# PaddlePaddle/Anakin

Hardware: AMD Instinct MI355X
Metric: ResNet50 INT8 images/sec + p50 latency @ batch 1/8, 1×MI355X (higher is better)
Workload: dtype int8

## Files before the change

### anakin_amd/csrc/api_chain.hip

```cpp
#include "api_internal.h"

enum : unsigned { CK_1X1 = 1, CK_3X3 = 2, CK_HEAD = 4, CK_PAIR = 8, CK_LED = CK_3X3 | CK_HEAD, CK_ANY = 15 };
static unsigned chain_kind(const saber_hip_chain* ch) { return !ch->c3 ? CK_1X1 : (ch->b2 ? CK_PAIR : (ch->b ? CK_3X3 : CK_HEAD)); }
static const struct { int c1; unsigned kinds; ChainForm f; } chain_forms[] = {
    {64, CK_ANY,            {4, 4, 4, 1, 1, CS_BASE, false}},
    {64, CK_ANY,            {2, 2, 4, 1, 1, CS_BASE, false}},
    {128, CK_1X1 | CK_LED,  {2, 2, 4, 1, 1, CS_BASE, false}},
    {128, CK_1X1 | CK_LED,  {1, 1, 4, 1, 1, CS_BASE, false}},
    {128, CK_1X1 | CK_LED,  {6, 2, 8, 1, 1, CS_W8, false}},
    {128, CK_1X1 | CK_LED,  {5, 1, 8, 1, 1, CS_W8, false}},
    {256, CK_1X1 | CK_LED,  {1, 1, 4, 1, 1, CS_BASE, false}},
    {256, CK_1X1,           {9, 1, 4, 2, 1, CS_SPLIT, false}},
    {256, CK_1X1,           {11, 1, 8, 2, 1, CS_SPLIT8, false}},
    {256, CK_LED,           {3, 1, 8, 1, 1, CS_W8, false}},
    {256, CK_3X3,           {7, 1, 8, 1, 2, CS_COOP2, true}},
    {256, CK_3X3,           {15, 2, 8, 1, 4, CS_COOP4, true}},
    {512, CK_1X1,           {1, 1, 4, 1, 1, CS_BASE, false}},
    {512, CK_1X1,           {9, 1, 4, 2, 1, CS_SPLIT, false}},
};
static void for_each_chain_form(const saber_hip_chain* ch, const std::function<void(const ChainForm&)>& fn) {
    for (const auto& r : chain_forms)
        if (r.c1 == ch->c1 && (r.kinds & chain_kind(ch))) fn(r.f);
}
static ChainForm chain_form_where(const saber_hip_chain* ch, const std::function<bool(const ChainForm& row, const ChainForm& found)>& take) {
// ... 45 lines not shown
    const int kw = K / nw, groups = kw / (16 * mfg), ksn = C / 64;
    for (int g = 0; g < groups; ++g)
        for (int ksi = 0; ksi < ksn; ++ksi)
            for (int mf = 0; mf < mfg; ++mf) {
                const int ks = (ks0 + ksi) % ksn;
                for (int lane = 0; lane < 64; ++lane) {
                    const int rho = lane & 15, kq = lane >> 4;
                    const int ch = kbase + wave * kw + g * 16 * mfg + (rho >> 2) * 4 * mfg + mf * 4 + (rho & 3);
                    const int8_t* src = w + (size_t)ch * C + ks * 64 + kq * 16;
                    out.insert(out.end(), (const uint8_t*)src, (const uint8_t*)src + 16);
                }
            }
}
static void pack_chain_weights3(const int8_t* w, int C, int wave, std::vector<uint8_t>& out, int nw = 4, int kbase = 0, int kcount = 0) {
    const int kw = (kcount ? kcount : C) / nw, mf0 = kw / 16, ksn = C / 64;
    for (int tap = 0; tap < 9; ++tap)
        for (int ks = 0; ks < ksn; ++ks)
            for (int mf = 0; mf < mf0; ++mf)
                for (int lane = 0; lane < 64; ++lane) {
                    const int rho = lane & 15, kq = lane >> 4;
                    const int ch = kbase + wave * kw + (rho >> 2) * 4 * mf0 + mf * 4 + (rho & 3);
                    for (int t = 0; t < 16; ++t) {
                        const int c = ks * 64 + kq * 16 + t;
                        out.push_back((uint8_t)w[((size_t)ch * C + c) * 9 + tap]);
                    }
                }
}
static void pack_frag1(const int8_t* w, int C, int ch_base, int mfg, int mf, int ks, std::vector<uint8_t>& out) {
    for (int lane = 0; lane < 64; ++lane) {
        const int rho = lane & 15, kq = lane >> 4;
        const int8_t* src = w + (size_t)(ch_base + (rho >> 2) * 4 * mfg + mf * 4 + (rho & 3)) * C + ks * 64 + kq * 16;
        out.insert(out.end(), (const uint8_t*)src, (const uint8_t*)src + 16);
    }
}
static void pack_frag3(const int8_t* w, int C, int ch_base, int tap, int ks, std::vector<uint8_t>& out) {
    for (int lane = 0; lane < 64; ++lane) {
        const int rho = lane & 15, kq = lane >> 4;
        for (int t = 0; t < 16; ++t) out.push_back((uint8_t)w[((size_t)(ch_base + rho) * C + ks * 64 + kq * 16 + t) * 9 + tap]);
    }
}
static void pack_coop4_stream(const saber_hip_conv* c3, const saber_hip_conv* a, const saber_hip_conv* b, std::vector<uint8_t>& out) {
    const int C = 256, K1 = 1024;
    for (int q = 0; q < 4; ++q)
        for (int w = 0; w < 8; ++w) {
            const int nt = w & 3, kh = w >> 2;
            for (int tap = 0; tap < 9; ++tap)
                for (int kl = 0; kl < 2; ++kl) pack_frag3(c3->wq_oihw.data(), C, q * 64 + nt * 16, tap, kh * 2 + kl, out);
            for (int i = 0; i < 4; ++i)
                for (int mf = 0; mf < 2; ++mf) pack_frag1(a->wq_oihw.data(), C, q * 256 + w * 32, 2, mf, (q + i) & 3, out);
            for (int jj = 0; b && jj < 8; ++jj) {
                const int j = jj < 2 ? kh * 2 + jj : 4 + kh * 6 + (jj - 2);
                pack_frag1(b->wq_oihw.data(), K1, q * 64 + nt * 16, 1, 0, (q * 4 + j) & 15, out);
            }
        }
}
static void pack_stage1_c128_stream(const saber_hip_conv* c3, const saber_hip_conv* a, const saber_hip_conv* b, std::vector<uint8_t>& out) {
    const int C = 128, K1 = 512;
    for (int w = 0; w < 8; ++w) {
        for (int tap = 0; tap < 9; ++tap)
            for (int ks = 0; ks < 2; ++ks) pack_frag3(c3->wq_oihw.data(), C, w * 16, tap, ks, out);
        for (int ks = 0; ks < 2; ++ks)
            for (int mf = 0; mf < 4; ++mf) pack_frag1(a->wq_oihw.data(), C, w * 64, 4, mf, ks, out);
        for (int ks = 0; ks < 8; ++ks) pack_frag1(b->wq_oihw.data(), K1, w * 16, 1, 0, ks, out);
    }
}
int saber_hip_conv2d_stem_pair_create(saber_hip_conv_t* stem, const saber_hip_conv_t* a, const saber_hip_conv_t* b, saber_hip_stem_pair_t** out) {
    if (!stem || !a || !b || !out) return fail(SABER_HIP_INVALID_VALUE, "null argument");
    const saber_hip_conv_desc& ds = stem->d;
    if (!stem->pool_fused || !stem->weights_set || ds.k != 64 || (ds.out_dtype != SABER_HIP_U8 && ds.out_dtype != SABER_HIP_S8))
        return fail(SABER_HIP_INVALID_VALUE, "stem pair: the head must be the fused stem conv + max pooling with 64 output channels (8-bit)");
    auto plain1x1 = [&](const saber_hip_conv* o) {
        const saber_hip_conv_desc& d = o->d;
        return o->is_i8 && o->weights_set && o->algo == ALGO_IGEMM_I8 && o->epi == EPI_I8_CONV && d.res_mode == SABER_HIP_RES_NONE &&
               !o->pair_k2 && !o->pool_fused && !o->pool2 && !o->pre_quant && !o->pre_pad && d.kh == 1 && d.kw == 1 && d.stride_h == 1 &&
               d.stride_w == 1 && d.pad_h == 0 && d.pad_w == 0 && d.group == 1 && d.c == 64 && o->c_eff == 64 && d.k % 32 == 0 &&
               d.in_layout == SABER_HIP_NHWC && d.out_layout == SABER_HIP_NHWC && d.act_negative_slope == 0.f &&
               (d.out_dtype == SABER_HIP_S8 || d.out_dtype == SABER_HIP_U8) && d.n == ds.n && d.h == stem->pool_oh && d.w == stem->pool_ow &&
               (o->x_dtype == DT_U8) == (ds.out_dtype == SABER_HIP_U8) && (int)o->wq_oihw.size() == d.k * 64;
    };
    if (!plain1x1(a) || !plain1x1(b) || a->d.k + b->d.k > 320)
        return fail(SABER_HIP_INVALID_VALUE, "stem pair: two plain 1x1 / stride-1 INT8 convs (64 -> k, k % 32 == 0, k_a + k_b <= 320, 8-bit NHWC outputs) "
                                              "on the pooled tensor");
    auto* sp = new saber_hip_stem_pair();
    sp->stem = stem; sp->a = a; sp->b = b;
    const int K1 = a->d.k, Kt = K1 + b->d.k;
    std::vector<int8_t> wcat((size_t)Kt * 64);
    std::memcpy(wcat.data(), a->wq_oihw.data(), (size_t)K1 * 64);
    std::memcpy(wcat.data() + (size_t)K1 * 64, b->wq_oihw.data(), (size_t)b->d.k * 64);
    std::vector<uint8_t> w, pa, pb, prm(256 * 16, 0);
    w.reserve((size_t)Kt * 64);
    for (int g = 0; g < Kt / 32; ++g)
        for (int mf = 0; mf < 2; ++mf) pack_frag1(wcat.data(), 64, g * 32, 2, mf, 0, w);
    pack_chain_params(a, (size_t)K1 / 4 * 3, pa);
    pack_chain_params(b, (size_t)b->d.k / 4 * 3, pb);
    std::memcpy(prm.data(), pa.data(), pa.size());
    std::memcpy(prm.data() + pa.size(), pb.data(), pb.size());
    hipError_t e = sp->d_w.upload(w);
    if (e == hipSuccess) e = sp->d_prm.upload(prm);
    if (e != hipSuccess) {
        delete sp;
        return hip_fail(e, "stem pair: device copies");
    }
    *out = sp;
    return SABER_HIP_OK;
}
void saber_hip_conv2d_stem_pair_destroy(saber_hip_stem_pair_t* sp) { delete sp; }
int saber_hip_conv2d_stem_pair_run(saber_hip_stem_pair_t* sp, const void* x, void* y_pool, void* y_a, void* y_b, void* workspace,
                                   saber_hip_stream_t stream) {
    if (g_capture) return capture_unsupported("saber_hip_conv2d_stem_pair_run (an executor-level object: saber_hip_net_optimize forms it itself)");
    if (!sp || !x || !y_a || !y_b) return fail(SABER_HIP_INVALID_VALUE, "null argument");
    saber_hip_conv* op = sp->stem;
    if (op->ws_bytes && !workspace) return fail(SABER_HIP_INVALID_VALUE, "workspace required");
    saber_mi355x::StemPairKArgs ka;
    const int rc = stem_pool_args(op, x, y_pool, workspace, (hipStream_t)stream, &ka.c);
    if (rc) return rc;
    ka.t.w = sp->d_w.p; ka.t.prm = sp->d_prm.p; ka.t.y1 = y_a; ka.t.y2 = y_b;
    ka.t.K1 = sp->a->d.k; ka.t.K2 = sp->b->d.k;
    ka.t.relu1 = sp->a->d.act == SABER_HIP_ACT_RELU; ka.t.relu2 = sp->b->d.act == SABER_HIP_ACT_RELU;
    ka.t.u8_1 = sp->a->d.out_dtype == SABER_HIP_U8; ka.t.u8_2 = sp->b->d.out_dtype == SABER_HIP_U8;
    HIP_TRY(saber_mi355x::launch_conv_stem_pool_pair(op->pre_quant ? 1 : 0, ka, (hipStream_t)stream));
    return SABER_HIP_OK;
}
saber_hip_chain::~saber_hip_chain() {
    if (h_coop_err) (void)hipHostFree(h_coop_err);
    delete stage1;
}
static unsigned div_magic(int d) { return d >= 2 ? (unsigned)((0x100000000ull + (unsigned)d - 1) / (unsigned)d) : 0u; }
static int stage_build(saber_hip_chain* const* chains, int n, bool per_image, saber_hip_chain* tail, saber_hip_chain_stage** out) {
    if (!chains || n <= 0 || n > saber_mi355x::STAGE4_LONG || !out) return fail(SABER_HIP_INVALID_VALUE, "stage: 1..24 chains");
    if (tail) {
        if (!chains[0] || chains[0]->c1 != 256 || tail->c1 != 256) return fail(SABER_HIP_INVALID_VALUE, "stage: a tail goes with a C = 256 stage only");
        if (n < 2 || !per_image || n + 1 > saber_mi355x::STAGE4_LONG) return fail(SABER_HIP_INVALID_VALUE, "stage: a tail needs 2..23 blocks, an image per XCD");
        if (!tail->c3 || tail->b || tail->b2 || tail->c3->d.stride_h != 2 || tail->c3->d.stride_w != 2)
            return fail(SABER_HIP_INVALID_VALUE, "stage: the tail must be a conv3x3 / stride 2 + conv1x1 chain without a second 1x1 conv");
        if (tail->a->d.res_stride != 2) return fail(SABER_HIP_INVALID_VALUE, "stage: the tail's shortcut must be sub-sampled by 2");
    }
    if (n > 1 && !per_image) return fail(SABER_HIP_INVALID_VALUE, "stage: several blocks need an image per XCD");
    if (n < 2 && chains[0] && chains[0]->c1 == 128) return fail(SABER_HIP_INVALID_VALUE, "stage: at C = 128 a stage is at least two blocks");
    const saber_hip_chain* c0 = chains[0];
    std::vector<saber_mi355x::StageBlk> blk;
    for (int k = 0; k < n; ++k) {
        const saber_hip_chain* ch = chains[k];
        const uint8_t* stream = !ch ? nullptr : (ch->c1 == 256 ? ch->d_stream[CS_COOP4].p : (ch->c1 == 128 ? ch->d_stream_stage1.p : nullptr));
        if (!ch || ch->c1 != c0->c1 || !ch->c3 || !ch->b || !stream || ch->c3->d.stride_h != 1)
            return fail(SABER_HIP_INVALID_VALUE, "stage: every block must be a conv3x3 (stride 1) + conv1x1 + conv1x1 chain at C = 256 (or all at C = 128)");
        const saber_hip_conv_desc& da = ch->a->d;
        if (da.n != c0->a->d.n || da.h != c0->a->d.h || da.w != c0->a->d.w) return fail(SABER_HIP_INVALID_VALUE, "stage: blocks of one tensor shape");
        if (k && ((ch->c3->x_dtype == DT_U8) != (chains[k - 1]->b->d.out_dtype == SABER_HIP_U8)))
            return fail(SABER_HIP_INVALID_VALUE, "stage: a block's 3x3 conv reads what the previous block's last conv writes");
        saber_mi355x::StageBlk B;
        std::memset(&B, 0, sizeof B);
        B.wstream = stream; B.prm0 = ch->d_prm0.p; B.prm1 = ch->d_prm1.p; B.prm2 = ch->d_prm2.p;
        B.coeff_conv = da.coeff_conv; B.scale_conv = ch->a->out_scale; B.coeff_res = da.coeff_res; B.scale_res = da.scale_res;
        B.in0_u8 = ch->c3->x_dtype == DT_U8; B.relu0 = ch->c3->d.act == SABER_HIP_ACT_RELU;
        B.in_u8 = ch->a->x_dtype == DT_U8; B.relu1 = da.act == SABER_HIP_ACT_RELU; B.res_relu = da.res_act == SABER_HIP_ACT_RELU;
        B.relu2 = ch->b->d.act == SABER_HIP_ACT_RELU; B.out_u8_2 = ch->b->d.out_dtype == SABER_HIP_U8;
        blk.push_back(B);
    }
    const saber_hip_conv_desc& d0 = c0->a->d;
    if (tail) {
        const saber_hip_conv_desc &d3 = tail->c3->d, &da = tail->a->d;
        if (d3.n != d0.n || d3.h != d0.h || d3.w != d0.w || da.res_h != d0.h || da.res_w != d0.w)
            return fail(SABER_HIP_INVALID_VALUE, "stage: the tail's 3x3 conv and shortcut read tensors of the blocks' shape");
        if ((tail->c3->x_dtype == DT_U8) != (chains[n - 1]->b->d.out_dtype == SABER_HIP_U8))
            return fail(SABER_HIP_INVALID_VALUE, "stage: the tail's 3x3 conv reads what the last block's last conv writes");
    }
    saber_hip_chain_stage* st = new saber_hip_chain_stage();
    st->chains.assign(chains, chains + n);
    st->c1 = c0->c1;
    st->n = d0.n; st->h = d0.h; st->w = d0.w;
    st->tiles_x = (d0.w + 15) / 16;
    st->tiles_per_img = st->tiles_x * ((d0.h + 1) / 2);
    st->per_image = per_image;
    const int wg_per_tile = st->c1 == 256 ? 4 : 1;
    const bool fits = d0.n <= 8 && st->tiles_per_img * wg_per_tile <= 32 &&
                      (st->c1 == 256 ? st->tiles_x == 1 : (st->tiles_x == 1 || st->tiles_x == 2 || st->tiles_x == 4));
    if ((per_image && !fits) || (st->c1 == 128 && !per_image)) {
        delete st;
        return fail(SABER_HIP_INVALID_VALUE, "stage: an image per XCD needs batch <= 8 and <= 32 workgroups per image (C = 256: width <= 16, <= 8 tiles "
                    "of 2 x 16 pixels; C = 128: width <= 64, <= 32 tiles)");
    }
    const size_t tiles = (size_t)d0.n * st->tiles_per_img;
    hipError_t e = hipSuccess;
    if (tail) {
        std::vector<uint8_t> ts;
        pack_coop4_stream(tail->c3, tail->a, nullptr, ts);
        e = st->d_tail_stream.upload(ts);
        const saber_hip_conv_desc& da = tail->a->d;
        saber_mi355x::StageBlk B;
        std::memset(&B, 0, sizeof B);
        B.wstream = st->d_tail_stream.p; B.prm0 = tail->d_prm0.p; B.prm1 = tail->d_prm1.p; B.prm2 = tail->d_prm0.p;
        B.coeff_conv = da.coeff_conv; B.scale_conv = tail->a->out_scale; B.coeff_res = da.coeff_res; B.scale_res = da.scale_res;
        B.in0_u8 = tail->c3->x_dtype == DT_U8; B.relu0 = tail->c3->d.act == SABER_HIP_ACT_RELU;
        B.in_u8 = tail->a->x_dtype == DT_U8; B.relu1 = da.act == SABER_HIP_ACT_RELU; B.res_relu = da.res_act == SABER_HIP_ACT_RELU;
        blk.push_back(B);
        st->tail = tail;
    }
    if (e == hipSuccess) e = st->d_blk.upload(blk);
    if (e == hipSuccess && st->c1 == 256) e = st->d_grp_ctr.alloc_zero(tiles * 32);
    if (e == hipSuccess) e = st->d_img_ctr.alloc_zero((size_t)d0.n * (st->tiles_per_img + 1) * 16);
    if (e == hipSuccess) e = st->d_xcc.alloc_zero(tiles * 32);
    if (e == hipSuccess && st->c1 == 256) e = st->d_xch.alloc_zero(tiles * 32 * 256);
    if (e == hipSuccess) e = hipHostMalloc((void**)&st->h_err, sizeof(unsigned), hipHostMallocMapped);
    if (e != hipSuccess) {
        delete st;
        return hip_fail(e, "stage: device buffers");
    }
    *st->h_err = 0u;
    *out = st;
    return SABER_HIP_OK;
}
template <int MAXB>
static int stage_launch(saber_hip_chain_stage* st, const void* x, const void* res, void* const* y1, void* const* y2, void* y_tail, hipStream_t s) {
    saber_mi355x::Stage4KArgs<MAXB> k;
    std::memset(&k, 0, sizeof k);
    k.x = x; k.res = res; k.zero = zero_page();
    if (!k.zero) return fail(SABER_HIP_RUNTIME_ERROR, "stage: zero page");
    k.blk = st->d_blk.p; k.grp_ctr = st->d_grp_ctr.p; k.img_ctr = st->d_img_ctr.p; k.xch = st->d_xch.p; k.xcc = st->d_xcc.p; k.err = st->h_err;
    k.nblk = (int)st->chains.size(); k.N = st->n; k.H = st->h; k.W = st->w;
    k.tiles_x = st->tiles_x; k.tiles_per_img = st->tiles_per_img;
    k.mg_tiles_x = div_magic(st->tiles_x); k.mg_tpi = div_magic(st->tiles_per_img); k.mg_wpi = div_magic(st->tiles_per_img * 4);
    k.per_image = st->per_image;
    for (int i = 0; i < k.nblk; ++i) { k.y1[i] = y1[i]; k.y2[i] = y2[i]; }
    if (y_tail) k.y1[k.nblk] = y_tail;
    HIP_TRY(st->c1 == 256 ? saber_mi355x::launch_conv_stage4(k, y_tail != nullptr, s) : saber_mi355x::launch_conv_stage1_c128(k, s));
    return SABER_HIP_OK;
}
int stage_run(saber_hip_chain_stage* st, const void* x, const void* res, void* const* y1, void* const* y2, hipStream_t s, void* y_tail) {
    if (y_tail && !st->tail) return fail(SABER_HIP_INVALID_VALUE, "stage: created without a tail");
    if (*(volatile unsigned*)st->h_err) {
        *(volatile unsigned*)st->h_err = 0u;
        return fail(SABER_HIP_RUNTIME_ERROR, "cooperative stage: an earlier launch's workgroups did not share an XCD or timed out at a barrier "
                    "(its outputs are not valid)");
    }
    return (int)st->chains.size() + (y_tail ? 1 : 0) <= saber_mi355x::STAGE4_SHORT ? stage_launch<saber_mi355x::STAGE4_SHORT>(st, x, res, y1, y2, y_tail, s)
                                                                                   : stage_launch<saber_mi355x::STAGE4_LONG>(st, x, res, y1, y2, y_tail, s);
}
int saber_hip_conv2d_stage_create(saber_hip_chain_t* const* chains, int n, saber_hip_chain_stage_t** out) {
    if (!xcd_round_robin()) return fail(SABER_HIP_UNIMPL, "stage: this device does not place workgroup b on XCD b % 8");
    return stage_build(chains, n, true, nullptr, out);
}
int saber_hip_conv2d_stage_create_tail(saber_hip_chain_t* const* chains, int n, saber_hip_chain_t* tail, saber_hip_chain_stage_t** out) {
    if (!tail) return fail(SABER_HIP_INVALID_VALUE, "null argument");
    if (!xcd_round_robin()) return fail(SABER_HIP_UNIMPL, "stage: this device does not place workgroup b on XCD b % 8");
    return stage_build(chains, n, true, tail, out);
}
void saber_hip_conv2d_stage_destroy(saber_hip_chain_stage_t* st) { delete st; }
int saber_hip_conv2d_stage_run(saber_hip_chain_stage_t* st, const void* x, const void* res, void* const* y1, void* const* y2, saber_hip_stream_t stream) {
    if (g_capture) return capture_unsupported("saber_hip_conv2d_stage_run (saber_hip_net_optimize forms stages itself)");
    if (!st || !x || !res || !y1 || !y2) return fail(SABER_HIP_INVALID_VALUE, "null argument");
    for (size_t i = 0; i < st->chains.size(); ++i)
        if (!y1[i] || !y2[i]) return fail(SABER_HIP_INVALID_VALUE, "stage: an output pointer per block");
    return stage_run(st, x, res, y1, y2, (hipStream_t)stream);
}
int saber_hip_conv2d_stage_run_tail(saber_hip_chain_stage_t* st, const void* x, const void* res, void* const* y1, void* const* y2, void* y_tail,
                                    saber_hip_stream_t stream) {
    if (g_capture) return capture_unsupported("saber_hip_conv2d_stage_run_tail (saber_hip_net_optimize forms stages itself)");
    if (!st || !x || !res || !y1 || !y2 || !y_tail) return fail(SABER_HIP_INVALID_VALUE, "null argument");
    for (size_t i = 0; i < st->chains.size(); ++i)
        if (!y1[i] || !y2[i]) return fail(SABER_HIP_INVALID_VALUE, "stage: an output pointer per block");
    return stage_run(st, x, res, y1, y2, (hipStream_t)stream, y_tail);
}
static void pack_chain_stream(const saber_hip_chain* ch, ChainStream layout, std::vector<uint8_t>& out) {
    const saber_hip_conv *c3 = ch->c3, *a = ch->a, *b = ch->b;
    const int c = ch->c1, k1 = ch->k1, k2 = ch->k2, c2 = b ? b->d.c : 0, k2w = k2 / 2;
    const int nw = layout == CS_BASE || layout == CS_SPLIT ? 4 : 8;
    const int8_t *w3 = c3 ? c3->wq_oihw.data() : nullptr, *wa = a->wq_oihw.data(), *wb = b ? b->wq_oihw.data() : nullptr;
    std::vector<int8_t> wcat;
    if (ch->b2) {
        wcat.assign(b->wq_oihw.begin(), b->wq_oihw.end());
        wcat.insert(wcat.end(), ch->b2->wq_oihw.begin(), ch->b2->wq_oihw.end());
        wb = wcat.data();
    }
    auto mfg = [&](int k) { return ch->b2 ? 2 : std::min(4, k / nw / 16); };
    switch (layout) {
    case CS_BASE: case CS_W8:
        for (int w = 0; w < nw; ++w) {
            if (c3) pack_chain_weights3(w3, c, w, out, nw);
            pack_chain_weights(wa, k1, c, 4, w, out, 0, nw);
            if (b) pack_chain_weights(wb, k2, c2, mfg(k2), w, out, 0, nw);
        }
        break;
    case CS_SPLIT: case CS_SPLIT8:
        for (int half = 0; half < 2; ++half)
            for (int w = 0; w < nw; ++w) {
                pack_chain_weights(wa, k1, c, 4, w, out, 0, nw);
                pack_chain_weights(wb, k2w, c2, mfg(k2w), w, out, half * k2w, nw);
            }
        break;
    case CS_COOP2:
        for (int half = 0; half < 2; ++half)
            for (int w = 0; w < nw; ++w) {
                pack_chain_weights3(w3, c, w, out, nw, half * (c / 2), c / 2);
                pack_chain_weights(wa, k1 / 2, c, 4, w, out, half * (k1 / 2), nw, half * (c / 128));
                pack_chain_weights(wb, k2w, c2, 1, w, out, half * k2w, nw, half * (c2 / 128));
            }
        break;
    default: pack_coop4_stream(c3, a, b, out);
    }
}
static int chain_build(saber_hip_conv* c3, saber_hip_conv* a, saber_hip_conv* b, saber_hip_chain_t** out, saber_hip_conv* b2 = nullptr) {
    if (!a || !out || (!b && !c3) || (b2 && (!b || !c3))) return fail(SABER_HIP_INVALID_VALUE, "null argument");
    const bool pair2 = b2 != nullptr;
    const bool strided = c3 && (!b || pair2) && c3->d.stride_h == 2 && c3->d.stride_w == 2;
    if (pair2 && !strided) return fail(SABER_HIP_INVALID_VALUE, "chain: a sibling pair follows the strided head (conv3x3 / stride 2 + conv1x1 + eltwise) only");
    if (!chain_1x1(a, strided) || (b && !chain_1x1(b)) || (b2 && !chain_1x1(b2)))
        return fail(SABER_HIP_INVALID_VALUE, "chain: both ops must be plain 1x1 stride-1 INT8 NHWC convs with weights set");
    if (strided != (a->d.res_stride > 1) || (strided && a->d.res_stride != 2))
        return fail(SABER_HIP_INVALID_VALUE, "chain: a stride-2 head goes with a shortcut sub-sampled by 2 (and only with one)");
    const saber_hip_conv_desc& da = a->d;
    if (da.res_mode != SABER_HIP_RES_ELTWISE || da.out_dtype != SABER_HIP_S8 || (da.res_has_dtype && da.res_dtype != SABER_HIP_S8))
        return fail(SABER_HIP_INVALID_VALUE, "chain: the first conv must carry the fused eltwise epilogue with s8 residual and output");
    if (b) {
        const saber_hip_conv_desc& db = b->d;
// ... 168 lines not shown
```

### anakin_amd/csrc/api_internal.h

```cpp
#pragma once
#include "../../include/saber_hip.h"
#include "kernels.h"

#include <cmath>
#include <cstdio>
#include <algorithm>
#include <cstdlib>
#include <cstring>
#include <functional>
#include <memory>
#include <mutex>
#include <string>
#include <utility>
#include <type_traits>
#include <vector>

using namespace saber_mi355x;

namespace saber_api {

extern thread_local std::string g_err;
inline int fail(int code, const std::string& msg) {
    g_err = msg;
    return code;
// ... 142 lines not shown
    unsigned* h_part_err = nullptr;
    DevBuf<uint8_t> d_w3;
    DevBuf<float> d_bias, d_scale;
    DevBuf<int> d_comp;
    DevBuf<unsigned> d_sm_ctr;
    bool has_bias = false, has_comp = false;
    std::string algo_name;
    int pair_k1 = 0, pair_k2 = 0, pair_relu2 = 0, pair_dtype2 = 0;
    const saber_hip_conv* pair_src_a = nullptr;
    const saber_hip_conv* pair_src_b = nullptr;
};

struct saber_hip_stem_pair {
    saber_hip_conv* stem = nullptr;
    const saber_hip_conv* a = nullptr;
    const saber_hip_conv* b = nullptr;
    DevBuf<uint8_t> d_w, d_prm;
};

enum ChainStream { CS_BASE, CS_SPLIT, CS_SPLIT8, CS_W8, CS_COOP2, CS_COOP4, CS_COUNT };
struct ChainForm {
    int code = 0;
    int rows = 0;
    int waves = 4;
    int split = 1;
    int coop = 1;
    ChainStream stream = CS_BASE;
    bool placement = false;
};

struct saber_hip_chain {
    saber_hip_conv* c3 = nullptr;
    saber_hip_conv* a = nullptr;
    saber_hip_conv* b = nullptr;
    saber_hip_conv* b2 = nullptr;
    int c1 = 0, k1 = 0, k2 = 0;
    ChainForm form;
    DevBuf<uint8_t> d_stream[CS_COUNT];
    DevBuf<uint8_t> d_prm0, d_prm1, d_prm2;
    DevBuf<uint8_t> d_coop_xch;
    DevBuf<uint8_t> d_stream_stage1;
    DevBuf<unsigned long long> d_coop_ctr;
    DevBuf<unsigned> d_coop_xcc;
    unsigned* h_coop_err = nullptr;
    int coop_tiles = 0;
    struct saber_hip_chain_stage* stage1 = nullptr;
    ~saber_hip_chain();
};

struct saber_hip_chain_stage {
    std::vector<saber_hip_chain*> chains;
    saber_hip_chain* tail = nullptr;
    DevBuf<uint8_t> d_tail_stream;
    DevBuf<saber_mi355x::StageBlk> d_blk;
    DevBuf<unsigned long long> d_grp_ctr, d_img_ctr;
    DevBuf<uint8_t> d_xch;
    DevBuf<unsigned> d_xcc;
    unsigned* h_err = nullptr;
    int c1 = 0, n = 0, h = 0, w = 0, tiles_x = 0, tiles_per_img = 0;
    bool per_image = false;
    ~saber_hip_chain_stage() {
        if (h_err) (void)hipHostFree(h_err);
    }
};

struct saber_hip_sep {
    saber_hip_conv* dw = nullptr;
    saber_hip_conv* pw = nullptr;
    int form = 0;
    DevBuf<uint8_t> d_wdw, d_wpw, d_prm;
    DevBuf<float> d_dw_bias, d_dw_scale;
    std::string name;
};

struct saber_hip_fc {
    saber_hip_fc_desc d;
    saber_hip_conv* conv = nullptr;
    bool pre_quant = false;
    float in_scale = 1.f;
};

namespace saber_api {
struct EventPair {
    hipEvent_t e0 = nullptr, e1 = nullptr;
    hipError_t init() {
        hipError_t e = hipEventCreate(&e0);
        return e != hipSuccess ? e : hipEventCreate(&e1);
    }
    ~EventPair() {
        if (e0) (void)hipEventDestroy(e0);
        if (e1) (void)hipEventDestroy(e1);
    }
};
struct ColdBench {
    size_t kBytes = (size_t)64 << 20;
    void* buf = nullptr;
    std::vector<hipEvent_t> ev;
    int reps = 0;
    hipError_t init(int r, size_t bytes = 0) {
        if (bytes) kBytes = std::min<size_t>(std::max<size_t>(bytes, (size_t)64 << 20), (size_t)512 << 20) & ~(size_t)0xfffff;
        reps = r < 3 ? 3 : (r > 32 ? 32 : r);
        hipError_t e = hipMalloc(&buf, kBytes + 256);
        if (e != hipSuccess) return e;
        e = hipMemset(buf, 1, kBytes + 256);
        if (e != hipSuccess) return e;
        ev.assign(2 * (size_t)reps, nullptr);
// ... 17 lines not shown
        if (hipEventSynchronize(ev[2 * reps - 1]) != hipSuccess) return -1.f;
        std::vector<float> t(reps);
        for (int r = 0; r < reps; ++r)
            if (hipEventElapsedTime(&t[r], ev[2 * r], ev[2 * r + 1]) != hipSuccess) return -1.f;
        std::sort(t.begin(), t.end());
        return t[reps / 2] * 1000.f;
    }
};

extern thread_local ColdBench* g_cold;
int time_enqueued(hipStream_t s, const std::function<int()>& fn, int warm_iters, float* t);
extern thread_local std::vector<unsigned long long>* g_used_kernels;
constexpr float g_reuse_tol = 0.03f;
struct ColdScope {
    ColdBench local;
    bool owner = false;
    hipError_t enter(int reps, size_t flush_bytes = 0) {
        const char* w = std::getenv("SABER_HIP_AUTOTUNE_WARM");
        if (w && w[0] == '1') return hipSuccess;
        if (g_cold) return hipSuccess;
        hipError_t e = local.init(reps, flush_bytes);
        if (e != hipSuccess) return e;
        g_cold = &local;
        owner = true;
        return hipSuccess;
    }
    ~ColdScope() {
        if (owner) g_cold = nullptr;
    }
};

}

namespace saber_api {
enum OpKind { OP_CONV, OP_CONV_PAIR, OP_FC, OP_QUANT, OP_DEQUANT, OP_TRANSPOSE_IN, OP_ELT_I8, OP_ELT_F32, OP_POOL_I8, OP_POOL_F32, OP_POOL_F32_I8, OP_FC_Q, OP_SOFTMAX, OP_RELU_F32, OP_ACT_F32 };
struct NetOp {
    OpKind kind;
    std::string name;
    saber_hip_conv* conv = nullptr;
    saber_hip_fc* fc = nullptr;
    int in = -1, in2 = -1, out = -1, out2 = -1;
    saber_hip_chain* chain = nullptr;
    int chain_out = -1;
    bool use_chain = false, skip = false;
    saber_hip_chain* chain3 = nullptr;
    int chain3_res = -1, chain3_y1 = -1, chain3_y2 = -1;
    int chain3_y3 = -1;
    bool use_chain3 = false;
    saber_hip_chain_stage* stage = nullptr;
    int stage_n = 0;
    bool use_stage = false;
    bool use_tail = false;
    int tail_of = -1, tail_mode = 0;
    saber_hip_stem_pair* stem_pair = nullptr;
    int stem_y1 = -1, stem_y2 = -1;
    saber_hip_sep* sep = nullptr;
    int sep_out = -1;
    bool use_sep = false;
    int lane = 0;
    bool record = false;
    int p[16] = {0};
    float f[6] = {0};
    size_t count = 0;
};
}

struct saber_hip_net {
    std::vector<size_t> tensor_bytes;
    std::vector<size_t> tensor_off;
    std::vector<void*> tensor_ext;
    std::vector<std::pair<const void*, int>> captured_ptr;
    void* ptr(int id) const {
        if (id < 0) return nullptr;
        if ((size_t)id < tensor_ext.size() && tensor_ext[id]) return tensor_ext[id];
        return (void*)(arena + tensor_off[id]);
    }
    std::vector<NetOp> ops;
    char* arena = nullptr;
    size_t arena_bytes = 0, ws_off = 0, ws_bytes = 0;
    hipGraph_t graph = nullptr;
    hipGraphExec_t exec = nullptr;
    bool finalized = false;
    bool compacted = false;
    bool shared_device = false;
    bool reproducible_fp32 = false;
    bool inplace_external = false;
    int coop_fallbacks = 0;
    hipStream_t side = nullptr;
    hipEvent_t ev_start = nullptr, ev_join = nullptr;
    std::vector<hipEvent_t> ev_op;
    std::vector<int> writer;
    bool lanes_ready = false, has_side = false;
    std::vector<saber_hip_conv*> owned;
    std::vector<saber_hip_chain*> owned_chains;
    std::vector<saber_hip_chain_stage*> owned_stages;
    std::vector<saber_hip_stem_pair*> owned_stem_pairs;
    std::vector<saber_hip_sep*> owned_seps;
};

namespace saber_api {
struct Capture;
extern thread_local Capture* g_capture;
int capture_conv(saber_hip_conv* op, const void* x, void* y, const void* res);
int capture_fc(saber_hip_fc* fc, const void* x, float* y, bool quantised_input);
int capture_unsupported(const char* what);
int capture_stream_op(OpKind kind, const char* name, const int* p, int np, const float* f, int nf, size_t count, const void* in,
                      size_t in_bytes, const void* in2, size_t in2_bytes, void* out, size_t out_bytes, void* out2, size_t out2_bytes);
}

bool sel_valid(const saber_hip_conv* op, const saber_api::ConvSel& s);
int sel_set(saber_hip_conv* op, const saber_api::ConvSel& s);
void sel_release_unused(saber_hip_conv* op);
void sel_name(saber_hip_conv* op);
unsigned long long sel_kernel_key(const saber_hip_conv* op, const saber_api::ConvSel& s);
int sel_launch(saber_hip_conv* op, saber_mi355x::ConvKArgs& a, hipStream_t s);
void for_each_candidate(const saber_hip_conv* op, const saber_api::ConvSel* best, const std::function<void(const saber_api::ConvSel&)>& fn);
bool dw_ok(const saber_hip_conv* op);
bool group_ok(const saber_hip_conv* op);
bool stem_ok(const saber_hip_conv* op);
bool fc_small_ok(const saber_hip_conv* op);
bool b3_tile_ok(const saber_hip_conv* op, int tile, int ks);
int dw_static_form(const saber_hip_conv* op);
int group_static_form(const saber_hip_conv* op);
constexpr long DW_STRIP_MIN_LANES = 150000;
std::string stem_pair_name(const saber_api::NetOp& o);
void conv_fill_args(const saber_hip_conv* op, saber_mi355x::ConvKArgs& a, const void* x, void* y, const void* res);
int stem_pool_args(const saber_hip_conv* op, const void* x, void* y, void* workspace, hipStream_t s, saber_mi355x::ConvKArgs* a);
bool xcd_round_robin();
int split_prepare(saber_hip_conv* op);
bool img_conv_ok(const saber_hip_conv* op);
int img_conv_prepare(saber_hip_conv* op);
int pw_prepare(saber_hip_conv* op);
bool pw_eligible(const saber_hip_conv* op);
int img_conv_run(saber_hip_conv* op, const void* x, void* y, const void* res, void* y_pool, hipStream_t stream);
void img_conv_release(saber_hip_conv* op);
int net_launch(saber_hip_net* net, const NetOp& o, hipStream_t s);
bool fc_softmax_ok(const saber_hip_fc* fc, bool quantised_input = false);
int fc_run_softmax(saber_hip_fc* fc, const void* x, float* y, float* prob, void* workspace, hipStream_t s, bool quantised_input);
int fc_softmax_prepare(saber_hip_fc* fc);
void net_set_chain_mode(saber_hip_net* net, int ia, int mode);
int net_chain_mode(const saber_hip_net* net, int ia);
void net_set_stage(saber_hip_net* net, int i0, bool on);
void net_set_tail(saber_hip_net* net, int i0, bool on);
ChainForm chain_form(const saber_hip_chain* ch, int code);
bool chain_form_valid(const saber_hip_chain* ch, int code);
ChainForm chain_form_default(const saber_hip_chain* ch);
ChainForm chain_form_plain(const saber_hip_chain* ch);
std::string chain_form_name(const saber_hip_chain* ch);
void for_each_chain_candidate(const saber_hip_chain* ch, bool shared_device, const std::function<void(const ChainForm&)>& fn);
bool conv_sep_ok(const saber_hip_conv* dw, const saber_hip_conv* pw, std::string* why);
bool sep_form_valid(const saber_hip_sep* sp, int code);
void for_each_sep_form(const saber_hip_sep* sp, const std::function<void(int code)>& fn);
int sep_static_form(const saber_hip_sep* sp);
void net_set_sep(saber_hip_net* net, int i, int code);
int stage_run(saber_hip_chain_stage* st, const void* x, const void* res, void* const* y1, void* const* y2, hipStream_t s, void* y_tail = nullptr);
```

### anakin_amd/csrc/api_net.hip

```cpp
#include "api_internal.h"

#include <atomic>
static std::atomic<int> g_coop_fallbacks_total{0};

int net_launch(saber_hip_net* net, const NetOp& o, hipStream_t s) {
    auto T = [&](int id) -> void* { return net->ptr(id); };
    void* ws = net->arena + net->ws_off;
    switch (o.kind) {
    case OP_CONV:
        if (o.skip) return SABER_HIP_OK;
        if (o.stage && o.use_stage) {
            void* y1[saber_mi355x::STAGE4_LONG];
            void* y2[saber_mi355x::STAGE4_LONG];
            const NetOp* ops = &o;
            for (int k = 0; k < o.stage_n; ++k) {
                y1[k] = T(ops[3 * k].chain3_y1);
                y2[k] = T(ops[3 * k].chain3_y2);
            }
            const int rc = stage_run(o.stage, T(o.in), T(o.chain3_res), y1, y2, s, o.use_tail ? T(ops[3 * o.stage_n].chain3_y1) : nullptr);
            if (rc == SABER_HIP_RUNTIME_ERROR) {
                ++net->coop_fallbacks;
                ++g_coop_fallbacks_total;
                net_set_stage(net, (int)(&o - net->ops.data()), false);
                if (net->exec) {
                    (void)hipGraphExecDestroy(net->exec);
                    (void)hipGraphDestroy(net->graph);
                    net->exec = nullptr;
                    net->graph = nullptr;
                }
            }
            return rc;
        }
        if (o.stem_pair) return saber_hip_conv2d_stem_pair_run(o.stem_pair, T(o.in), nullptr, T(o.stem_y1), T(o.stem_y2), ws, s);
        if (o.chain3 && o.use_chain3) {
            const int rc = saber_hip_conv2d_chain_run3(o.chain3, T(o.in), T(o.chain3_res), T(o.chain3_y1), T(o.chain3_y2), T(o.chain3_y3), s);
            if (rc == SABER_HIP_RUNTIME_ERROR) {
                ++net->coop_fallbacks;
                ++g_coop_fallbacks_total;
            }
            return rc;
        }
        if (o.chain && o.use_chain) return saber_hip_conv2d_chain_run(o.chain, T(o.in), T(o.in2), T(o.out), T(o.chain_out), s);
        if (o.sep && o.use_sep) return saber_hip_conv2d_sep_run(o.sep, T(o.in), nullptr, T(o.sep_out), s);
        if (o.conv->gpool) return saber_hip_conv2d_run_gpool(o.conv, T(o.in), T(o.out), T(o.in2), T(o.out2), s);
        return saber_hip_conv2d_run(o.conv, T(o.in), T(o.out), T(o.in2), ws, s);
    case OP_CONV_PAIR:
        if (o.skip) return SABER_HIP_OK;
        return saber_hip_conv2d_run_pair(o.conv, T(o.in), T(o.out), T(o.out2), s);
    case OP_FC:
        if (o.out2 >= 0) return fc_run_softmax(o.fc, T(o.in), (float*)T(o.out), (float*)T(o.out2), ws, s, false);
        return saber_hip_fc_run(o.fc, T(o.in), (float*)T(o.out), ws, s);
    case OP_QUANT:
        return saber_hip_quantize_nchw_to_nhwc(o.p[0], o.p[1], o.p[2], o.p[3], o.p[4], o.p[5], o.f[0],
                                               (const float*)T(o.in), T(o.out), s);
    case OP_DEQUANT:
        return saber_hip_dequantize_nhwc_to_nchw(o.p[0], o.p[1], o.p[2], o.p[3], o.p[4], o.f[0], T(o.in),
                                                 (float*)T(o.out), s);
    case OP_TRANSPOSE_IN:
        return saber_hip_transpose_nchw_to_nhwc_f32(o.p[0], o.p[1], o.p[2], o.p[3], o.p[4], (const float*)T(o.in),
                                                    (float*)T(o.out), s);
    case OP_ELT_I8:
        return saber_hip_eltwise_sum_i8(o.count, (const int8_t*)T(o.in), (const int8_t*)T(o.in2), o.f[0], o.f[1],
                                        o.f[2], o.f[3], o.p[0], (int8_t*)T(o.out), s);
    case OP_ELT_F32:
        return saber_hip_eltwise_sum_f32(o.count, (const float*)T(o.in), (const float*)T(o.in2), o.f[0], o.f[1],
                                         o.p[0], (float*)T(o.out), s);
    case OP_POOL_I8:
        return saber_hip_pool2d_i8_nhwc(o.p[0], o.p[1], o.p[2], o.p[3], o.p[4], o.p[5], o.p[6], o.p[7], o.p[8],
                                        o.p[9], o.p[10], o.p[11], o.p[12], o.p[13], o.p[14], T(o.in), T(o.out), s);
    case OP_POOL_F32:
        return saber_hip_pool2d_f32(o.p[0], o.p[1], o.p[2], o.p[3], o.p[4], o.p[5], o.p[6], o.p[7], o.p[8], o.p[9],
                                    o.p[10], o.p[11], o.p[12], o.p[13], (const float*)T(o.in), (float*)T(o.out), s);
// ... 163 lines not shown
int saber_hip_net_add_activation_f32(saber_hip_net_t* net, int active, size_t count, float negative_slope, float coef, int in_id, int out_id) {
    NetOp o;
    o.kind = OP_ACT_F32; o.in = in_id; o.out = out_id; o.count = count; o.name = "activation_f32";
    o.p[0] = active; o.f[0] = negative_slope; o.f[1] = coef;
    return push(net, std::move(o));
}
int saber_hip_net_add_softmax(saber_hip_net_t* net, int rows, int cols, int in_id, int out_id) {
    NetOp o;
    o.kind = OP_SOFTMAX; o.in = in_id; o.out = out_id; o.name = "softmax_f32";
    o.p[0] = rows; o.p[1] = cols;
    return push(net, std::move(o));
}

int saber_hip_net_finalize(saber_hip_net_t* net) {
    if (net->finalized) return SABER_HIP_OK;
    size_t off = 0;
    net->tensor_off.resize(net->tensor_bytes.size());
    for (size_t i = 0; i < net->tensor_bytes.size(); ++i) {
        net->tensor_off[i] = off;
        if (net->tensor_ext[i]) continue;
        off += (net->tensor_bytes[i] + 255) / 256 * 256;
    }
    net->ws_off = off;
    off += (net->ws_bytes + 255) / 256 * 256;
    net->arena_bytes = off ? off : 256;
    HIP_TRY(hipMalloc((void**)&net->arena, net->arena_bytes));
    HIP_TRY(hipMemset(net->arena, 0, net->arena_bytes));
    HIP_TRY(hipStreamSynchronize(nullptr));
    net->finalized = true;
    return SABER_HIP_OK;
}
int saber_hip_net_compact_arena(saber_hip_net_t* net, const int* keep, int n_keep) {
    if (!net || !net->finalized) return fail(SABER_HIP_INVALID_VALUE, "compact_arena: net not finalized");
    const int nt = (int)net->tensor_bytes.size(), nops = (int)net->ops.size();
    for (const NetOp& o : net->ops)
        if (o.lane) return SABER_HIP_OK;
    std::vector<int> first(nt, nops), last(nt, -1), writes(nt, 0), reads(nt, 0);
    std::vector<char> pinned(nt, 0);
    for (int i = 0; i < n_keep; ++i)
        if (keep && keep[i] >= 0 && keep[i] < nt) pinned[keep[i]] = 1;
    std::vector<int> g_lo(nops), g_hi(nops);
    for (int i = 0; i < nops; ++i) g_lo[i] = g_hi[i] = i;
    auto span = [&](int i, int n) {
        const int hi = std::min(nops - 1, i + n - 1);
        int lo = i;
        for (int j = i; j <= hi; ++j) lo = std::min(lo, g_lo[j]);
        int h2 = hi;
        for (int j = i; j <= hi; ++j) h2 = std::max(h2, g_hi[j]);
        for (int j = lo; j <= h2; ++j) { g_lo[j] = std::min(g_lo[j], lo); g_hi[j] = std::max(g_hi[j], h2); }
    };
    for (int i = 0; i < nops; ++i) {
        const NetOp& o = net->ops[i];
        if (o.stage) span(i, 3 * o.stage_n + (o.stage->tail ? 2 : 0));
        if (o.chain3) span(i, 3);
        if (o.chain) span(i, 2);
        if (o.stem_pair) span(i, 2);
        if (o.sep) span(i, 2);
        if ((o.kind == OP_FC || o.kind == OP_FC_Q) && o.out2 >= 0) span(i, 2);
        if (i + 1 < nops && net->ops[i + 1].skip) span(i, 2);
    }
    for (int i = 0; i < nops; ++i) {
        const NetOp& o = net->ops[i];
        const int rd[] = {o.in, o.in2, o.chain3_res};
        const int wr[] = {o.out, o.out2, o.chain_out, o.chain3_y1, o.chain3_y2, o.chain3_y3, o.stem_y1, o.stem_y2, o.sep_out};
        auto touch = [&](int t) {
            if (t < 0 || t >= nt) return;
            first[t] = std::min(first[t], g_lo[i]);
            last[t] = std::max(last[t], g_hi[i]);
        };
        for (int t : rd) { touch(t); if (t >= 0 && t < nt) ++reads[t]; }
        for (int t : wr) { touch(t); if (t >= 0 && t < nt) ++writes[t]; }
    }
    for (int t = 0; t < nt; ++t)
        if (net->tensor_ext[t] || !writes[t] || !reads[t] || last[t] < 0) pinned[t] = 1;
    for (int t = 0; t < nt; ++t)
        if (pinned[t]) { first[t] = -1; last[t] = nops; }
    std::vector<int> order;
    for (int t = 0; t < nt; ++t)
        if (!net->tensor_ext[t]) order.push_back(t);
    auto slot = [&](int t) { return (net->tensor_bytes[t] + 255) / 256 * 256; };
    std::stable_sort(order.begin(), order.end(), [&](int a, int b) { return slot(a) > slot(b); });
    std::vector<size_t> off(nt, 0);
    std::vector<int> placed;
    size_t top = 0;
    for (int t : order) {
        const size_t sz = slot(t);
        if (!sz) { off[t] = 0; continue; }
        std::vector<std::pair<size_t, size_t>> busy;
        for (int u : placed)
            if (first[u] <= last[t] && first[t] <= last[u]) busy.push_back({off[u], off[u] + slot(u)});
        std::sort(busy.begin(), busy.end());
        size_t at = 0;
        for (const auto& b : busy) {
            if (at + sz <= b.first) break;
            at = std::max(at, b.second);
        }
        off[t] = at;
        top = std::max(top, at + sz);
        placed.push_back(t);
    }
    const size_t ws_off = top, total = std::max<size_t>(256, top + (net->ws_bytes + 255) / 256 * 256);
    if (total >= net->arena_bytes) return SABER_HIP_OK;
    char* fresh = nullptr;
    HIP_TRY(hipMalloc((void**)&fresh, total));
    HIP_TRY(hipMemset(fresh, 0, total));
    HIP_TRY(hipDeviceSynchronize());
// ... 247 lines not shown
            float ms = 0;
            HIP_TRY(hipEventElapsedTime(&ms, ev[prev[i]], ev[i + 1]));
            acc[i] += ms;
        }
    }
    for (size_t i = 0; i < n; ++i) out_us[i] = (float)(acc[i] * 1000.0 / iters);
    return SABER_HIP_OK;
}
int saber_hip_net_time_op_in_pass(saber_hip_net_t* net, saber_hip_stream_t stream, int index, int iters, float* out_us) {
    if (!net || !net->finalized || iters <= 0 || !out_us || index < 0 || index >= (int)net->ops.size())
        return fail(SABER_HIP_INVALID_VALUE, "bad argument");
    hipStream_t s = (hipStream_t)stream;
    EventPair evp;
    HIP_TRY(evp.init());
    double acc = 0.0;
    for (int it = 0; it < iters + 1; ++it) {
        for (size_t i = 0; i < net->ops.size(); ++i) {
            if ((int)i == index) HIP_TRY(hipEventRecord(evp.e0, s));
            int rc = net_launch(net, net->ops[i], s);
            if (rc) return rc;
            if ((int)i == index) HIP_TRY(hipEventRecord(evp.e1, s));
        }
        HIP_TRY(hipStreamSynchronize(s));
        float ms = 0;
        HIP_TRY(hipEventElapsedTime(&ms, evp.e0, evp.e1));
        if (it) acc += ms;
    }
    *out_us = (float)(acc * 1000.0 / iters);
    return SABER_HIP_OK;
}
int saber_hip_net_time_ops(saber_hip_net_t* net, saber_hip_stream_t stream, int iters, float* out_us) {
    hipStream_t s = (hipStream_t)stream;
    EventPair evp;
    HIP_TRY(evp.init());
    hipEvent_t e0 = evp.e0, e1 = evp.e1;
    for (size_t i = 0; i < net->ops.size(); ++i) {
        int rc = net_launch(net, net->ops[i], s);
        if (rc) return rc;
        HIP_TRY(hipEventRecord(e0, s));
        for (int it = 0; it < iters; ++it) net_launch(net, net->ops[i], s);
        HIP_TRY(hipEventRecord(e1, s));
        HIP_TRY(hipEventSynchronize(e1));
        float ms = 0;
        HIP_TRY(hipEventElapsedTime(&ms, e0, e1));
        out_us[i] = ms * 1000.f / iters;
    }
    return SABER_HIP_OK;
}
int saber_hip_net_tensor_unwritten(const saber_hip_net_t* net, int id) {
    if (id < 0 || id >= (int)net->tensor_bytes.size()) return 0;
    if (net->tensor_bytes[id] == 0) return 1;
    for (const NetOp& o : net->ops)
        if (((o.chain3 && o.use_chain3) || o.stem_pair || (o.sep && o.use_sep)) && o.out == id) return 1;
    return 0;
}
static void net_drop_graph(saber_hip_net* net) {
    if (!net->exec) return;
    (void)hipGraphExecDestroy(net->exec);
    (void)hipGraphDestroy(net->graph);
    net->exec = nullptr;
    net->graph = nullptr;
}
int saber_hip_net_status(saber_hip_net_t* net) {
    if (!net || !net->finalized) return fail(SABER_HIP_INVALID_VALUE, "net not finalized");
    int bad = 0;
    for (size_t i = 0; i < net->ops.size(); ++i) {
        NetOp& o = net->ops[i];
        if (o.stage && o.stage->h_err && *(volatile unsigned*)o.stage->h_err) {
            *(volatile unsigned*)o.stage->h_err = 0u;
            if (o.use_stage) net_set_stage(net, (int)i, false);
            ++bad;
        }
        saber_hip_chain* ch = o.chain3;
        if (ch) {
            unsigned* words[2] = {ch->h_coop_err, ch->stage1 ? ch->stage1->h_err : nullptr};
            for (unsigned* w : words)
                if (w && *(volatile unsigned*)w) {
                    *(volatile unsigned*)w = 0u;
                    if (ch->form.placement) ch->form = chain_form_plain(ch);
                    ++bad;
                }
        }
    }
    if (!bad) return SABER_HIP_OK;
    net->coop_fallbacks += bad;
    g_coop_fallbacks_total += bad;
    net_drop_graph(net);
    return fail(SABER_HIP_RUNTIME_ERROR, "a cooperative launch of the last pass did not complete (workgroups on different XCDs, or a hand-off "
                "timed out: another kernel held the CUs); its outputs are not valid - those sites now launch block by block: run the pass again");
}
int saber_hip_net_inject_coop_error(saber_hip_net_t* net) {
    if (!net) return fail(SABER_HIP_INVALID_VALUE, "null argument");
    for (NetOp& o : net->ops)
        if (o.stage && o.use_stage && o.stage->h_err) { *(volatile unsigned*)o.stage->h_err = 1u; return SABER_HIP_OK; }
    for (NetOp& o : net->ops) {
        if (o.stage && o.stage->h_err) { *(volatile unsigned*)o.stage->h_err = 1u; return SABER_HIP_OK; }
        if (o.chain3 && o.chain3->h_coop_err) { *(volatile unsigned*)o.chain3->h_coop_err = 1u; return SABER_HIP_OK; }
    }
    return fail(SABER_HIP_INVALID_VALUE, "the net has no cooperative launch site");
}
int saber_hip_net_num_launches(const saber_hip_net_t* net) {
    int n = 0;
    for (const NetOp& o : net->ops) n += o.skip ? 0 : 1;
    return n;
}
void saber_hip_net_destroy(saber_hip_net_t* net) {
// ... 18 lines not shown
```

### anakin_amd/csrc/api_net_autotune.hip

```cpp
#include "api_internal.h"

static saber_hip_conv* net_op_conv(saber_hip_net* net, int index) {
    if (index < 0 || index >= (int)net->ops.size()) return nullptr;
    NetOp& o = net->ops[index];
    if (o.kind == OP_CONV || o.kind == OP_CONV_PAIR) return o.conv;
    if (o.kind == OP_FC || o.kind == OP_FC_Q) return o.fc ? o.fc->conv : nullptr;
    return nullptr;
}
int saber_hip_net_get_choice(saber_hip_net_t* net, int index) {
    saber_hip_conv* c = net_op_conv(net, index);
    int choice = (c && !c->pool_fused && (c->algo <= ALGO_IGEMM_F32 || dw_ok(c) || group_ok(c))) ? saber_hip_conv2d_get_tile(c) : 0;
    if (c && net->ops[index].chain) choice |= (1 << 28) | ((net->ops[index].use_chain ? net->ops[index].chain->form.code : 0) << 24);
    const bool in_tail = c && net->ops[index].tail_of >= 0 && net->ops[net->ops[index].tail_of].use_tail;
    const bool led = net->ops[index].chain3 && (in_tail ? net->ops[index].tail_mode == 2 : net->ops[index].use_chain3);
    if (c && net->ops[index].chain3) choice |= (1 << 29) | ((led ? net->ops[index].chain3->form.code : 0) << 24);
    if (c && net->ops[index].sep) choice |= (3 << 28) | ((net->ops[index].use_sep ? net->ops[index].sep->form : 0) << 24);
    if (c && net->ops[index].stage && net->ops[index].use_stage) choice |= 1 << 30;
    if (c && net->ops[index].stage && net->ops[index].use_tail) choice |= (int)0x80000000u;
    return choice;
}
int saber_hip_net_stage_blocks(const saber_hip_net_t* net, int index) {
    if (!net || index < 0 || index >= (int)net->ops.size()) return 0;
    return net->ops[index].stage ? net->ops[index].stage_n : 0;
}
int saber_hip_net_set_choice(saber_hip_net_t* net, int index, int choice) {
    saber_hip_conv* c = net_op_conv(net, index);
    if (!c || !choice || c->pool_fused || (c->algo > ALGO_IGEMM_F32 && !dw_ok(c) && !group_ok(c))) return SABER_HIP_OK;
    if (net->reproducible_fp32 && !c->is_i8) return SABER_HIP_OK;
    if (net->ops[index].kind == OP_CONV_PAIR && index > 0 && net->ops[index - 1].stem_pair) return SABER_HIP_OK;
    const int chain_bits = (choice >> 24) & 63;
    const bool stage_on = ((choice >> 30) & 1) && !net->shared_device;
    const bool tail_on = stage_on && (((unsigned)choice >> 31) & 1u);
    choice &= 0xffffff;
    if (net->shared_device && ((choice >> 16) & 0xff) == 11) choice &= ~(0xf << 12);
    NetOp& o = net->ops[index];
    saber_hip_chain* ch = index + 1 >= (int)net->ops.size() ? nullptr : ((o.chain3 && (chain_bits & 32)) ? o.chain3 : ((o.chain && (chain_bits & 16)) ? o.chain : nullptr));
    int tn = chain_bits & 15;
    if (ch && net->shared_device && chain_form(ch, tn).placement) tn = chain_form_plain(ch).code;
    if (ch && tn && !chain_form_valid(ch, tn)) return saber_hip_conv2d_chain_set_tile(ch, tn);
    const bool sep_bits = o.sep && (chain_bits & 48) == 48;
    if (sep_bits && tn && !sep_form_valid(o.sep, tn)) return saber_hip_conv2d_sep_set_tile(o.sep, tn);
    int rc = choice ? saber_hip_conv2d_set_tile(c, choice) : SABER_HIP_OK;
    if (rc) return rc;
    const bool in_tail = o.tail_of >= 0 && net->ops[o.tail_of].use_tail;
    if (in_tail) net_set_tail(net, o.tail_of, false);
    o.name = std::string(o.kind == OP_FC || o.kind == OP_FC_Q ? "fc:" : "conv:") + c->algo_name;
    if ((o.kind == OP_FC || o.kind == OP_FC_Q) && o.out2 >= 0) o.name += fc_softmax_ok(o.fc, o.kind == OP_FC_Q) ? "+softmax" : " | softmax_f32";
    if (ch && tn) (void)saber_hip_conv2d_chain_set_tile(ch, tn);
    const bool in_stage = o.chain3 && o.skip && !o.stage;
    if (ch && ch == o.chain3) net_set_chain_mode(net, index + 1, (tn || in_stage) ? 2 : net_chain_mode(net, index + 1) == 2 ? 1 : net_chain_mode(net, index + 1));
    else if (ch) net_set_chain_mode(net, index, net_chain_mode(net, index) == 2 ? 2 : (tn ? 1 : 0));
    if (o.stage) net_set_stage(net, index, stage_on);
    if (o.stage) net_set_tail(net, index, tail_on);
    if (in_tail) net_set_tail(net, o.tail_of, true);
    if (o.skip) o.name = (o.chain3 && o.use_chain3) ? "conv:(in the stage launch)" : "conv:(in the chain launch)";
    if (o.skip && index > 0 && net->ops[index - 1].tail_of >= 0 && net->ops[net->ops[index - 1].tail_of].use_tail) o.name = "conv:(in the stage launch)";
    if (o.skip && o.kind == OP_CONV_PAIR) o.name = (index > 0 && net->ops[index - 1].stem_pair) ? "conv:(in the stem launch)" : "conv:(in the chain launch)";
    if (o.stem_pair) o.name = stem_pair_name(o);
    if (o.sep) net_set_sep(net, index, sep_bits ? tn : (o.use_sep ? o.sep->form : 0));
    if (o.skip && index > 0 && net->ops[index - 1].sep && net->ops[index - 1].use_sep) o.name = "conv:(in the separable launch)";
    if (net->exec) {
        (void)hipGraphExecDestroy(net->exec);
        (void)hipGraphDestroy(net->graph);
        net->exec = nullptr;
        net->graph = nullptr;
    }
    return SABER_HIP_OK;
}

static int net_consolidate_kernels(saber_hip_net* net, hipStream_t s) {
    if (net->has_side) return SABER_HIP_OK;
    if (const char* e = std::getenv("SABER_HIP_NO_CONSOLIDATE"))
        if (e[0] == '1') return SABER_HIP_OK;
    struct Site { int op; unsigned long long key; ConvSel choice; };
    auto conv_of = [&](const NetOp& o) -> saber_hip_conv* {
        if (o.skip || (o.chain && o.use_chain) || (o.chain3 && o.use_chain3) || (o.stage && o.use_stage) || (o.sep && o.use_sep)) return nullptr;
        if (o.kind != OP_CONV && o.kind != OP_CONV_PAIR) return nullptr;
        if (net->reproducible_fp32 && o.conv && !o.conv->is_i8) return nullptr;
        return (o.conv && !o.conv->pool_fused && o.conv->algo <= ALGO_IGEMM_F32) ? o.conv : nullptr;
    };
    auto collect = [&]() {
        std::vector<Site> v;
        for (int i = 0; i < (int)net->ops.size(); ++i)
            if (saber_hip_conv* c = conv_of(net->ops[i])) v.push_back({i, sel_kernel_key(c, c->sel), c->sel});
        return v;
    };
    EventPair ev;
    HIP_TRY(ev.init());
    auto forward_ms = [&](float* ms) -> int {
        int rc = 0;
        for (int i = 0; i < 3 && !rc; ++i) rc = saber_hip_net_run(net, s);
        if (rc) return rc;
        HIP_TRY(hipEventRecord(ev.e0, s));
        for (int i = 0; i < 30 && !rc; ++i) rc = saber_hip_net_run(net, s);
        HIP_TRY(hipEventRecord(ev.e1, s));
        HIP_TRY(hipEventSynchronize(ev.e1));
        HIP_TRY(hipEventElapsedTime(ms, ev.e0, ev.e1));
        return rc;
    };
    std::vector<Site> sites = collect();
    for (size_t si = 0; si < sites.size(); ++si) {
        const Site cur = sites[si];
        if ((cur.key >> 8 & 0xff) != 5) continue;
        int uses = 0;
        for (const Site& t : sites) uses += t.key == cur.key;
        if (uses != 1) continue;
        saber_hip_conv* c = conv_of(net->ops[cur.op]);
        std::vector<Site> alts;
        for (const Site& t : sites) {
            if (t.op == cur.op || (t.key & 0xff) != (cur.key & 0xff) || (t.key >> 8 & 0xff) != 5 || t.key == cur.key) continue;
// ... 68 lines not shown
        int rc = saber_hip_conv2d_autotune(c, xin, T(o.out), T(o.in2), net->arena + net->ws_off, stream, iters);
        if (rc) return rc;
        o.name = std::string(o.kind == OP_CONV ? "conv:" : "fc:") + c->algo_name;
        if ((o.kind == OP_FC || o.kind == OP_FC_Q) && o.out2 >= 0) o.name += fc_softmax_ok(o.fc, o.kind == OP_FC_Q) ? "+softmax" : " | softmax_f32";
        if (o.stem_pair) o.name = stem_pair_name(o);
    }
    const char* log_env = std::getenv("SABER_HIP_AUTOTUNE_LOG");
    const bool log_cands = g_cold && log_env && log_env[0] == '1';
    auto log_cand = [&](const saber_hip_conv* c, const std::string& name, float t) {
        if (log_cands) std::fprintf(stderr, "autotune [%dx%dx%d c%d k%d %dx%d] %-40s %8.2f us\n", c->d.n, c->d.h, c->d.w, c->d.c, c->d.k, c->d.kh, c->d.kw, name.c_str(), t);
    };
    for (size_t i = 0; i < net->ops.size(); ++i)
        if (net->ops[i].stage) net_set_stage(net, (int)i, false);
    for (size_t i = 0; i < net->ops.size(); ++i) {
        NetOp& A = net->ops[i];
        const int ia = (int)i;
        NetOp* H = (ia > 0 && net->ops[ia - 1].chain3) ? &net->ops[ia - 1] : nullptr;
        if (!A.chain && !H) continue;
        const int first = H ? ia - 1 : ia;
        const int last = (A.chain || (H && H->chain3->b2)) ? ia + 1 : ia;
        hipStream_t s = (hipStream_t)stream;
        auto run_all = [&]() -> int {
            int rc = 0;
            for (int k = first; k <= last; ++k) rc |= net_launch(net, net->ops[k], s);
            return rc;
        };
        auto timed = [&](float* t) { return time_enqueued(s, run_all, 20, t); };
        float best = 0.f;
        int best_mode = 0, best_tn = 0;
        net_set_chain_mode(net, ia, 0);
        int rc = timed(&best);
        if (rc) return rc;
        log_cand(A.conv, "separate", best);
        for (int mode = A.chain ? 1 : 2; mode <= (H ? 2 : 1); ++mode) {
            saber_hip_chain* ch = mode == 2 ? H->chain3 : A.chain;
            for_each_chain_candidate(ch, net->shared_device, [&](const ChainForm& f) {
                float ms = -1.f;
                if (saber_hip_conv2d_chain_set_tile(ch, f.code) != SABER_HIP_OK) return;
                net_set_chain_mode(net, ia, mode);
                const int rt = timed(&ms);
                log_cand(A.conv, (mode == 2 ? H->name : A.name).substr(5), ms);
                if (rt == SABER_HIP_OK && ms < best) { best = ms; best_mode = mode; best_tn = f.code; }
            });
        }
        if (best_mode) (void)saber_hip_conv2d_chain_set_tile(best_mode == 2 ? H->chain3 : A.chain, best_tn);
        net_set_chain_mode(net, ia, best_mode);
        rc = run_all();
        if (rc) return rc;
    }
    for (size_t i = 0; i < net->ops.size(); ++i) {
        NetOp& H0 = net->ops[i];
        if (!H0.stage || net->shared_device) continue;
        const bool has_tail = H0.stage->tail != nullptr;
        const int first = (int)i, last = first + 3 * H0.stage_n - 1 + (has_tail ? 2 : 0);
        hipStream_t s = (hipStream_t)stream;
        auto run_all = [&]() -> int {
            int rc = 0;
            for (int k = first; k <= last; ++k) rc |= net_launch(net, net->ops[k], s);
            return rc;
        };
        auto timed = [&](float* t) { return time_enqueued(s, run_all, 20, t); };
        std::vector<int> modes(H0.stage_n), tns(H0.stage_n);
        for (int k = 0; k < H0.stage_n; ++k) {
            modes[k] = net_chain_mode(net, first + 3 * k + 1);
            tns[k] = net->ops[first + 3 * k].chain3->form.code;
        }
        float sep = 0.f, one = 0.f;
        int rc = timed(&sep);
        if (rc) return rc;
        log_cand(H0.conv, "separate", sep);
        net_set_stage(net, first, true);
        net_set_tail(net, first, false);
        bool ok = timed(&one) == SABER_HIP_OK && hipStreamSynchronize(s) == hipSuccess && !*(volatile unsigned*)H0.stage->h_err;
        log_cand(H0.conv, H0.name.substr(5), ok ? one : -1.f);
        if (ok && has_tail) {
            float wt = 0.f;
            net_set_tail(net, first, true);
            const bool ok_t = timed(&wt) == SABER_HIP_OK && hipStreamSynchronize(s) == hipSuccess && !*(volatile unsigned*)H0.stage->h_err;
            log_cand(H0.conv, H0.name.substr(5), ok_t ? wt : -1.f);
            if (*(volatile unsigned*)H0.stage->h_err) ok = false;
            else if (ok_t && wt < one) one = wt;
            else net_set_tail(net, first, false);
        }
        if (!ok || one >= sep) {
            *(volatile unsigned*)H0.stage->h_err = 0u;
            net_set_stage(net, first, false);
            for (int k = 0; k < H0.stage_n; ++k) {
                (void)saber_hip_conv2d_chain_set_tile(net->ops[first + 3 * k].chain3, tns[k]);
                net_set_chain_mode(net, first + 3 * k + 1, modes[k]);
            }
        }
        rc = run_all();
        if (rc) return rc;
    }
    for (size_t i = 0; i + 1 < net->ops.size(); ++i) {
        NetOp& D = net->ops[i];
        if (!D.sep) continue;
        hipStream_t s = (hipStream_t)stream;
        auto run_all = [&]() -> int { return net_launch(net, net->ops[i], s) | net_launch(net, net->ops[i + 1], s); };
        auto timed = [&](float* t) { return time_enqueued(s, run_all, 20, t); };
        float best = 0.f;
        int best_code = 0;
        net_set_sep(net, (int)i, 0);
        int rc = timed(&best);
        if (rc) return rc;
        log_cand(D.conv, "separate", best);
        for_each_sep_form(D.sep, [&](int code) {
            float us = -1.f;
            net_set_sep(net, (int)i, code);
            const int rt = timed(&us);
            log_cand(D.conv, D.name.substr(5), us);
            if (rt == SABER_HIP_OK && us < best) { best = us; best_code = code; }
        });
        net_set_sep(net, (int)i, best_code);
        rc = run_all();
        if (rc) return rc;
    }
    return g_cold ? net_consolidate_kernels(net, (hipStream_t)stream) : SABER_HIP_OK;
}
```

### anakin_amd/csrc/api_net_optimize.hip

```cpp
#include "api_internal.h"

static void net_name_chain(NetOp& A, NetOp& B) {
    if (A.skip) {
        A.name = B.name = "conv:(in the chain launch)";
    } else if (A.use_chain) {
        A.name = "conv:" + chain_form_name(A.chain);
        B.name = "conv:(in the chain launch)";
    } else {
        A.name = std::string("conv:") + A.conv->algo_name;
        B.name = std::string("conv:") + B.conv->algo_name;
    }
}
static std::string stage_name(const NetOp& H0) {
    return "conv:stage_c" + std::to_string(H0.stage->c1) + "_" + std::to_string(H0.stage_n) + "x[conv3x3+chain1x1]_2x16" + (H0.stage->c1 == 256 ? "_coop4" : "") +
           (H0.use_tail ? "+[conv3x3/2+conv1x1]" : "");
}
void net_set_chain_mode(saber_hip_net* net, int ia, int mode) {
    NetOp& A = net->ops[ia];
    NetOp* H = (ia > 0 && net->ops[ia - 1].chain3) ? &net->ops[ia - 1] : nullptr;
    if (mode == 2 && !H) mode = 1;
    if (mode == 1 && !A.chain) mode = 0;
    NetOp* B = A.chain ? &net->ops[ia + 1] : nullptr;
    A.use_chain = mode == 1 || (mode == 2 && H->chain3->b && !H->chain3->b2);
    if (B) B->skip = mode == 1 || (mode == 2 && H->chain3->b);
    A.skip = mode == 2;
    if (H && H->chain3->b2) {
        NetOp& P = net->ops[ia + 1];
        P.skip = mode == 2;
        P.name = mode == 2 ? "conv:(in the chain launch)" : std::string("conv:") + P.conv->algo_name;
    }
    if (H) {
        H->use_chain3 = mode == 2;
        H->name = "conv:" + (mode == 2 ? chain_form_name(H->chain3) : std::string(H->conv->algo_name));
    }
    if (B) net_name_chain(A, *B);
    else A.name = A.skip ? "conv:(in the chain launch)" : std::string("conv:") + A.conv->algo_name;
    if (H && H->stage && H->use_stage) H->name = stage_name(*H);
    else if (H && H->skip) H->name = "conv:(in the stage launch)";
}
std::string stem_pair_name(const NetOp& o) {
    return std::string("conv:") + o.conv->algo_name + "+pair1x1_" + std::to_string(o.stem_pair->a->d.k) + "+" + std::to_string(o.stem_pair->b->d.k);
}
void net_set_tail(saber_hip_net* net, int i0, bool on) {
    NetOp& H0 = net->ops[i0];
    if (!H0.stage || !H0.stage->tail) return;
    const int it = i0 + 3 * H0.stage_n;
    NetOp& Ht = net->ops[it];
    on = on && H0.use_stage;
    if (on == H0.use_tail) return;
    if (on) Ht.tail_mode = net_chain_mode(net, it + 1);
    H0.use_tail = on;
    Ht.skip = on;
    net_set_chain_mode(net, it + 1, on ? 2 : Ht.tail_mode);
    if (on) net->ops[it + 1].name = "conv:(in the stage launch)";
    if (H0.use_stage) H0.name = stage_name(H0);
}
void net_set_stage(saber_hip_net* net, int i0, bool on) {
    NetOp& H0 = net->ops[i0];
    if (!H0.stage) return;
    if (!on) net_set_tail(net, i0, false);
    for (int k = 0; k < H0.stage_n; ++k) {
        if (on || H0.use_stage) net_set_chain_mode(net, i0 + 3 * k + 1, 2);
        NetOp& Hk = net->ops[i0 + 3 * k];
        if (k) {
            Hk.skip = on;
            if (on) Hk.name = "conv:(in the stage launch)";
        }
    }
    H0.use_stage = on;
    if (on) net_set_tail(net, i0, true);
    if (on) H0.name = stage_name(H0);
}
int net_chain_mode(const saber_hip_net* net, int ia) {
    const NetOp& A = net->ops[ia];
    return A.skip ? 2 : (A.use_chain ? 1 : 0);
}
void net_set_sep(saber_hip_net* net, int i, int code) {
    NetOp& D = net->ops[i];
    if (!D.sep || i + 1 >= (int)net->ops.size()) return;
    NetOp& P = net->ops[i + 1];
    if (code && saber_hip_conv2d_sep_set_tile(D.sep, code) != SABER_HIP_OK) code = 0;
    D.use_sep = code != 0;
    P.skip = D.use_sep;
    D.name = std::string("conv:") + (D.use_sep ? saber_hip_conv2d_sep_algo(D.sep) : D.conv->algo_name.c_str());
    P.name = D.use_sep ? std::string("conv:(in the separable launch)") : std::string("conv:") + P.conv->algo_name;
}
static int clone_conv_i8(const saber_hip_conv* src, const saber_hip_conv_desc& d, saber_hip_conv** out) {
    int rc = saber_hip_conv2d_create(&d, out);
    if (rc) return rc;
    rc = saber_hip_conv2d_set_weights(*out, src->wq_oihw.data(), SABER_HIP_S8, src->w_scale.data(),
                                      src->has_bias ? src->bias_host.data() : nullptr, src->in_scale, src->out_scale);
    if (rc) {
        saber_hip_conv2d_destroy(*out);
        *out = nullptr;
    }
    return rc;
}

int saber_hip_net_optimize(saber_hip_net_t* net, int flags) {
    if (!net) return fail(SABER_HIP_INVALID_VALUE, "null argument");
    if (net->finalized) return fail(SABER_HIP_INVALID_VALUE, "optimize must run before finalize");
    if (flags & 2048) {
        net->shared_device = true;
        flags &= ~256;
    }
    if (net->shared_device) flags &= ~256;
    if (flags & SABER_HIP_NET_REPRODUCIBLE_FP32) net->reproducible_fp32 = true;
    std::vector<NetOp>& ops = net->ops;
    const int nt = (int)net->tensor_bytes.size();
    std::vector<char> dead(ops.size(), 0);
    int removed = 0;
    auto consumers = [&](int t) {
// ... 279 lines not shown
            Hd.chain3_res = A.in2; Hd.chain3_y1 = A.out; Hd.chain3_y2 = B.out;
            const bool was = A.use_chain;
            net_set_chain_mode(net, (int)i + 1, ch->c1 <= 128 ? 2 : (was ? 1 : 0));
            if (Hd.use_chain3) removed += was ? 1 : 2;
        }
        for (size_t i = 0; i + 1 < ops.size(); ++i) {
            NetOp& Hd = ops[i];
            NetOp& A = ops[i + 1];
            if (A.chain || A.skip || A.kind != OP_CONV || !A.conv || A.conv->d.res_mode != SABER_HIP_RES_ELTWISE || A.in2 < 0 || A.lane ||
                Hd.kind != OP_CONV || !Hd.conv || Hd.chain3 || Hd.chain || Hd.skip || Hd.lane || Hd.in2 >= 0 || A.in != Hd.out)
                continue;
            int readers = 0;
            for (const NetOp& o : ops) readers += (o.in == Hd.out) + (o.in2 == Hd.out);
            if (readers != 1) continue;
            saber_hip_chain* ch = nullptr;
            NetOp* P = (flags & 1024) && i + 2 < ops.size() ? &ops[i + 2] : nullptr;
            if (P && (P->kind != OP_CONV_PAIR || P->lane || P->skip || P->in != A.out || !P->conv || !P->conv->pair_src_a || !P->conv->pair_src_b)) P = nullptr;
            if (P) {
                int rd = 0;
                for (const NetOp& o : ops) rd += (o.in == A.out) + (o.in2 == A.out);
                if (rd != 1 || saber_hip_conv2d_chain_create3_pair(Hd.conv, A.conv, const_cast<saber_hip_conv*>(P->conv->pair_src_a),
                                                                   const_cast<saber_hip_conv*>(P->conv->pair_src_b), &ch) != SABER_HIP_OK)
                    P = nullptr;
            }
            if (!P && saber_hip_conv2d_chain_create3(Hd.conv, A.conv, nullptr, &ch) != SABER_HIP_OK) continue;
            net->owned_chains.push_back(ch);
            Hd.chain3 = ch;
            Hd.chain3_res = A.in2; Hd.chain3_y1 = A.out; Hd.chain3_y2 = P ? P->out : -1; Hd.chain3_y3 = P ? P->out2 : -1;
            net_set_chain_mode(net, (int)i + 1, ch->c1 <= 128 ? 2 : 0);
            if (Hd.use_chain3) removed += P ? 2 : 1;
        }
    }
    if ((flags & 256) && (flags & 32) && !two_lanes) {
        for (size_t i = 0; i + 2 < ops.size();) {
            auto block_ok = [&](size_t j) {
                return j + 2 < ops.size() && ops[j].chain3 && ops[j].chain3->b && !ops[j].stage && ops[j].chain3_y2 >= 0 &&
                       ((ops[j].chain3->c1 == 256 && ops[j].chain3->stage1) || (ops[j].chain3->c1 == 128 && ops[j].chain3->d_stream_stage1.p));
            };
            if (!block_ok(i)) { ++i; continue; }
            std::vector<saber_hip_chain*> run{ops[i].chain3};
            while ((int)run.size() < saber_mi355x::STAGE4_LONG) {
                const size_t p = i + 3 * (run.size() - 1), j = p + 3;
                if (!block_ok(j) || ops[j].chain3->c1 != run[0]->c1 || ops[j].in != ops[p].chain3_y2 || ops[j].chain3_res != ops[p].chain3_y1) break;
                run.push_back(ops[j].chain3);
            }
            if (run.size() >= 2) {
                saber_hip_chain_stage* st = nullptr;
                const size_t pl = i + 3 * (run.size() - 1), jt = pl + 3;
                saber_hip_chain* tail = nullptr;
                if (jt + 1 < ops.size() && run[0]->c1 == 256 && ops[jt].chain3 && !ops[jt].chain3->b && !ops[jt].chain3->b2 && !ops[jt].stage &&
                    ops[jt].chain3->c1 == 256 && ops[jt].chain3->c3->d.stride_h == 2 && ops[jt].in == ops[pl].chain3_y2 &&
                    ops[jt].chain3_res == ops[pl].chain3_y1 && ops[jt].chain3_y1 >= 0)
                    tail = ops[jt].chain3;
                if (tail && saber_hip_conv2d_stage_create_tail(run.data(), (int)run.size(), tail, &st) != SABER_HIP_OK) tail = nullptr;
                if (tail || saber_hip_conv2d_stage_create(run.data(), (int)run.size(), &st) == SABER_HIP_OK) {
                    net->owned_stages.push_back(st);
                    ops[i].stage = st;
                    ops[i].stage_n = (int)run.size();
                    if (tail) ops[jt].tail_of = (int)i;
                    int before = 0;
                    for (size_t k = 0; k < run.size(); ++k) before += 3 - (ops[i + 3 * k].skip + ops[i + 3 * k + 1].skip + ops[i + 3 * k + 2].skip);
                    if (tail) before += 2 - (ops[jt].skip + ops[jt + 1].skip);
                    const bool on = run[0]->a->d.n >= 4 && run[0]->c1 == 256;
                    net_set_stage(net, (int)i, on);
                    if (on) removed += before - 1;
                }
            }
            i += 3 * run.size();
        }
    }
    if (flags & 4096) {
        for (size_t i = 0; i + 1 < ops.size(); ++i) {
            NetOp& F = ops[i];
            if (dead[i] || (F.kind != OP_FC && F.kind != OP_FC_Q) || !F.fc || F.out2 >= 0 || F.lane) continue;
            size_t j = i + 1;
            while (j < ops.size() && dead[j]) ++j;
            if (j >= ops.size()) break;
            NetOp& S = ops[j];
            if (S.kind != OP_SOFTMAX || S.in != F.out || S.skip || S.lane || S.p[0] != F.fc->d.m || S.p[1] != F.fc->d.n) continue;
            if (F.kind == OP_FC && F.fc->pre_quant) continue;
            if (!fc_softmax_ok(F.fc, F.kind == OP_FC_Q) || fc_softmax_prepare(F.fc) != SABER_HIP_OK) continue;
            F.out2 = S.out;
            F.name = std::string("fc:") + F.fc->conv->algo_name + "+softmax";
            S.skip = true;
            S.name = "softmax_f32 (in the fc launch)";
            ++removed;
        }
    }
    if (net->shared_device) {
        for (NetOp& o : ops) {
            saber_hip_conv* c = (o.kind == OP_FC || o.kind == OP_FC_Q) ? (o.fc ? o.fc->conv : nullptr) : o.conv;
            if (c) {
                c->no_placement = true;
                if (c->sel.fam == FAM_B3 && c->sel.ksplit) (void)sel_set(c, sel_b3(c->sel, c->sel.tile, c->sel.ks, 0));
            }
            for (saber_hip_chain* ch : {o.chain, o.chain3})
                if (ch && ch->form.placement) ch->form = chain_form_plain(ch);
        }
    }
    net->ws_bytes = 0;
    for (const NetOp& o : ops) {
        size_t w = 0;
        if ((o.kind == OP_CONV) && o.conv) w = o.conv->ws_bytes;
        if (o.kind == OP_FC && o.fc) w = saber_hip_fc_workspace_bytes(o.fc);
        if (w > net->ws_bytes) net->ws_bytes = w;
    }
    return removed;
}
```

### anakin_amd/csrc/conv_stage_coop.hip

```cpp
#include "coop_sync.h"

namespace saber_mi355x {

template <int MAXB, bool TAIL>
__global__ __launch_bounds__(512) void conv_stage4_c256_kernel(const Stage4KArgs<MAXB> ka) {
    constexpr int C1 = 256, K1 = 1024, K2 = 256, NW = 8;
    constexpr int F0 = 18, F1 = 8, F2 = 8;
    constexpr int FB = F0 + F1 + F2, FT = F0 + F1;
    constexpr int K0Q = C1 / 4, K1Q = K1 / 4, K2Q = K2 / 4;
    constexpr int CH1 = C1 / 16, PCH = CH1 + 1, HW = 18, HP = 4 * HW;
    constexpr int HCH = (HP * PCH + 63) / 64 * 64;
    constexpr int CPRW = K1Q / 16;
    constexpr int P0C = (K0Q / 4 * 3 + 63) / 64 * 64, P1C = K1Q / 4 * 3, P2C = (K2Q / 4 * 3 + 63) / 64 * 64;
    constexpr int MPC = K0Q / 16 + 1;
    constexpr int YPC = (K1 - K1Q) / 16 + 1;
    constexpr int YCH = (32 * YPC + 63) / 64 * 64;
    static_assert(P1C % 64 == 0 && (32 * CPRW) == 64 * NW, "DMA granularity");
    __shared__ v4i halo[HCH];
    __shared__ v4i tile[32 * CPRW];
    __shared__ v4i ptile[YCH];
    __shared__ v4i mid_own[32 * MPC];
    __shared__ v4i red[4 * 2 * 64];
    __shared__ v4i prm0[P0C];
    __shared__ v4i prm1[P1C];
    __shared__ v4i prm2[P2C];
    __shared__ int dma_off[((HCH / 64 + NW - 1) / NW + (YCH / 64 + NW - 1) / NW) * 512];
    SABER_TL_DECL;
    SABER_TL(0);
    const int tid = threadIdx.x, lane = tid & 63;
    const int wave = __builtin_amdgcn_readfirstlane(tid >> 6);
    const int nt = wave & 3, kh = wave >> 2;
    const int frow = lane & 15, fq = lane >> 4;
    const int b = blockIdx.x;
    int n, rem, q;
    if (ka.per_image) {
        const int slot = b >> 3;
        const int il = ka.mg_wpi ? (int)__umulhi((unsigned)slot, ka.mg_wpi) : slot;
        const int widx = slot - il * ka.tiles_per_img * 4;
        n = il * 8 + (b & 7);
        rem = widx >> 2;
        q = widx & 3;
        if (n >= ka.N) return;
    } else {
        const int t = (b >> 5) * 8 + (b & 7);
        q = (b >> 3) & 3;
        if (t >= ka.N * ka.tiles_per_img) return;
        n = ka.mg_tpi ? (int)__umulhi((unsigned)t, ka.mg_tpi) : t;
        rem = t - n * ka.tiles_per_img;
    }
    const int t = n * ka.tiles_per_img + rem;
    const int ty = ka.mg_tiles_x ? (int)__umulhi((unsigned)rem, ka.mg_tiles_x) : rem;
    const int x0 = (rem - ty * ka.tiles_x) * 16, y0 = ty * 2;
    const int H = ka.H, W = ka.W;
    auto pix = [&](int m, bool& ok) -> int {
        int x = x0 + (m & 15), y = y0 + (m >> 4);
        ok = x < W && y < H;
        x = x < W ? x : W - 1;
        y = y < H ? y : H - 1;
        return (n * H + y) * W + x;
    };
    unsigned long long* const ctr = ka.grp_ctr + (size_t)t * 32;
    unsigned long long* const e_up = ka.img_ctr + ((size_t)n * (ka.tiles_per_img + 1) + ty) * 16;
    bool ok0, ok1, okt;
    const int p0 = pix(frow, ok0), p1 = pix(16 + frow, ok1);
    const int tpx = tid / CPRW, tc = (tid % CPRW) ^ (tpx & 15);
    const int pt = pix(tpx, okt);

    constexpr int HIT = (HCH / 64 + NW - 1) / NW, YIT = (YCH / 64 + NW - 1) / NW;
    int* const halo_off = dma_off + tid;
    int* const pt_off = dma_off + HIT * 512 + tid;
#pragma unroll
    for (int it = 0; it < HIT; ++it) {
        const int L = (wave + it * NW) * 64 + lane;
        const int hp = L / PCH, cc = L - hp * PCH;
        const int hy = hp / HW, hx = hp - hy * HW;
        const int gy = y0 - 1 + hy, gx = x0 - 1 + hx;
        const bool in = hp < HP && cc < CH1 && (unsigned)gy < (unsigned)H && (unsigned)gx < (unsigned)W;
        halo_off[it * 512] = in ? ((n * H + gy) * W + gx) * C1 + cc * 16 : -1;
    }
#pragma unroll
    for (int it = 0; it < YIT; ++it) {
        const int L = (wave + it * NW) * 64 + lane;
        const int px = L / YPC, j = L - px * YPC;
        bool okp;
        const int pp_ = pix(px & 31, okp);
        const int pc = j < q * 16 ? j : j + 16;
        pt_off[it * 512] = (px < 32 && j < YPC - 1) ? pp_ * K1 + pc * 16 : -1;
    }
    auto dma_halo = [&](const void* x, bool l2) {
        const char* xg = (const char*)x;
#pragma unroll
        for (int it = 0; it < HIT; ++it) {
            const int i = wave + it * NW;
            if (i >= HCH / 64) break;
            const int off = halo_off[it * 512];
            if (off < 0) lds_dma16(ka.zero, halo + i * 64);
            else if (l2) lds_dma16_l2(xg + off, halo + i * 64);
            else lds_dma16(xg + off, halo + i * 64);
        }
    };
    auto dma_prm = [&](const StageBlk& B) {
        if (wave < P0C / 64) lds_dma16((const v4i*)B.prm0 + q * (K0Q / 4 * 3) + wave * 64 + lane, prm0 + wave * 64);
        for (int i = wave; i < P1C / 64; i += NW) lds_dma16((const v4i*)B.prm1 + q * P1C + i * 64 + lane, prm1 + i * 64);
        if (wave < P2C / 64) lds_dma16((const v4i*)B.prm2 + q * (K2Q / 4 * 3) + wave * 64 + lane, prm2 + wave * 64);
    };
    auto stream_of = [&](const StageBlk& B, int nf) -> const v4i* {
        return (const v4i*)B.wstream + (size_t)(q * NW + wave) * (nf * 64) + lane;
    };
    const int nall = ka.nblk + (TAIL ? 1 : 0);

    dma_halo(ka.x, false);
    lds_dma16((const char*)ka.res + (size_t)pt * K1 + q * K1Q + tc * 16, tile + wave * 64);
    dma_prm(ka.blk[0]);
    asm volatile("" ::: "memory");
    v4i fr[F0 + 2];
    {
        const v4i* wsb = stream_of(ka.blk[0], FB);
#pragma unroll
        for (int r = 0; r < F0 + 2; ++r) {
            fr[r] = wsb[r * 64];
            asm volatile("" ::: "memory");
        }
    }
    wait_vm_older_than<F0 + 2>();
    __builtin_amdgcn_s_barrier();
    SABER_TL(1);

    StageBlk B = ka.blk[0];
    for (int k = 0; k < ka.nblk; ++k) {
        const v4i z = {0, 0, 0, 0};
        {
            const int xm0 = B.in0_u8 ? (int)0x80808080u : 0;
            const int c0 = nt * 16 + fq * 4;
            const v4i* pp = prm0 + (c0 / 4) * 3;
            v4i acc0 = kh ? z : pp[2], acc1 = acc0;
            const v4i* hb = halo + frow * PCH + fq + kh * 8;
#pragma unroll
            for (int s = 0; s < F0; ++s) {
                const int kl = s % 2, tap = s / 2;
                const int dy = tap / 3, dx = tap % 3;
                v4i b0 = hb[(dy * HW + dx) * PCH + kl * 4];
                v4i b1 = hb[((dy + 1) * HW + dx) * PCH + kl * 4];
                b0.x ^= xm0; b0.y ^= xm0; b0.z ^= xm0; b0.w ^= xm0;
                b1.x ^= xm0; b1.y ^= xm0; b1.z ^= xm0; b1.w ^= xm0;
                acc0 = mma_step(fr[s], b0, acc0);
                acc1 = mma_step(fr[s], b1, acc1);
            }
            if (kh) {
                red[(nt * 2 + 0) * 64 + lane] = acc0;
                red[(nt * 2 + 1) * 64 + lane] = acc1;
            }
            asm volatile("s_waitcnt lgkmcnt(0)" ::: "memory");
            __builtin_amdgcn_s_barrier();
            if (!kh) {
                const v4i r0 = red[(nt * 2 + 0) * 64 + lane], r1 = red[(nt * 2 + 1) * 64 + lane];
                acc0.x += r0.x; acc0.y += r0.y; acc0.z += r0.z; acc0.w += r0.w;
                acc1.x += r1.x; acc1.y += r1.y; acc1.z += r1.z; acc1.w += r1.w;
                const float lo0 = B.relu0 ? 0.f : -3.0e38f;
                const float off0 = B.in_u8 ? 0.f : 128.f;
                const unsigned xo0 = B.in_u8 ? 0u : 0x80808080u;
                const unsigned o0 = chain_out_pack(acc0, z, __builtin_bit_cast(v4f, pp[1]), __builtin_bit_cast(v4f, pp[0]), lo0, off0, xo0);
                const unsigned o1 = chain_out_pack(acc1, z, __builtin_bit_cast(v4f, pp[1]), __builtin_bit_cast(v4f, pp[0]), lo0, off0, xo0);
                char* xg = (char*)ka.xch + ((size_t)t * 32 + frow) * C1 + q * K0Q + c0;
                *(unsigned*)xg = o0;
                *(unsigned*)(xg + 16 * C1) = o1;
                *(unsigned*)((char*)mid_own + frow * (MPC * 16) + c0) = o0;
                *(unsigned*)((char*)mid_own + (16 + frow) * (MPC * 16) + c0) = o1;
            }
        }
        if (k == 0 && tid == 0) {
            unsigned xcc;
            asm volatile("s_getreg_b32 %0, hwreg(HW_REG_XCC_ID)" : "=s"(xcc));
            ka.xcc[t * 32 + q] = xcc & 7u;
            if (rem == 0 && q == 0) ka.xcc[t * 32 + 4] = (xcc & 7u) + 1u;
        }
        coop_arrive(ctr);
        v4i fs[F1 - 2 + F2];
        {
            const v4i* wsb = stream_of(B, FB);
// ... 431 lines not shown
                const int ch = (ks * 4 + fq) ^ frow;
                acc0 = mma_step(fs[F1 - 2 + ks], tile[frow * CPRW + ch], acc0);
                acc1 = mma_step(fs[F1 - 2 + ks], tile[(16 + frow) * CPRW + ch], acc1);
            }
            const float lo2 = B.relu2 ? 0.f : -3.0e38f;
            const float off2 = B.out_u8_2 ? 0.f : 128.f;
            const unsigned xm2 = B.out_u8_2 ? 0u : 0x80808080u;
            const unsigned o0 = chain_out_pack(acc0, z, __builtin_bit_cast(v4f, pp[1]), __builtin_bit_cast(v4f, pp[0]), lo2, off2, xm2);
            const unsigned o1 = chain_out_pack(acc1, z, __builtin_bit_cast(v4f, pp[1]), __builtin_bit_cast(v4f, pp[0]), lo2, off2, xm2);
            if (ok0) *(unsigned*)((char*)ka.y2[k] + (size_t)p0 * K2 + c2) = o0;
            if (ok1) *(unsigned*)((char*)ka.y2[k] + (size_t)p1 * K2 + c2) = o1;
        }
        SABER_TL(6);
        if (k + 1 < ka.nblk) {
            asm volatile("s_waitcnt vmcnt(0)" ::: "memory");
            __builtin_amdgcn_s_barrier();
            unsigned long long* const e_k = e_up + (k & 1);
            if (wave == 0 && lane == 0) {
                (void)__hip_atomic_fetch_add(e_k, 1ull, __ATOMIC_RELAXED, __HIP_MEMORY_SCOPE_WORKGROUP);
                (void)__hip_atomic_fetch_add(e_k + 16, 1ull, __ATOMIC_RELAXED, __HIP_MEMORY_SCOPE_WORKGROUP);
            }
            dma_prm(Bn);
            if (wave == 0) {
                const unsigned long long one = (unsigned long long)ka.tiles_x;
                coop_wait_mask2(e_k, (ty > 0 ? 2 * one : one) - 1, e_k + 16, (ty + 1 < tile_rows ? 2 * one : one) - 1, ka.err);
            }
            __builtin_amdgcn_s_barrier();
            dma_halo(ka.y2[k], true);
            wait_vm_older_than<0>();
            __builtin_amdgcn_s_barrier();
            B = Bn;
            SABER_TL(7);
        }
    }
    if (tid == 0 && ka.err) {
        const unsigned first = (unsigned)L2Reader(ka.xcc).load16((unsigned)(n * ka.tiles_per_img) * 128u + 16u).x;
        if (first && first != my_xcc) __hip_atomic_fetch_add(ka.err, 1u, __ATOMIC_RELAXED, __HIP_MEMORY_SCOPE_SYSTEM);
    }
    SABER_TL_FLUSH();
}

template <int MAXB>
static hipError_t launch_stage1(const Stage4KArgs<MAXB>& ka, hipStream_t s) {
    if (ka.nblk <= 1 || ka.nblk > MAXB || ka.N <= 0 || !ka.blk || !ka.xcc || !ka.per_image || !ka.img_ctr ||
        (ka.tiles_x != 1 && ka.tiles_x != 2 && ka.tiles_x != 4))
        return hipErrorInvalidValue;
    const dim3 grid((ka.N + 7) / 8 * ka.tiles_per_img * 8), block(512);
    hipLaunchKernelGGL(conv_stage1_c128_kernel<MAXB>, grid, block, 0, s, ka);
    return hipGetLastError();
}
hipError_t launch_conv_stage1_c128(const Stage4KArgs<STAGE4_SHORT>& a, hipStream_t s) { return launch_stage1(a, s); }
hipError_t launch_conv_stage1_c128(const Stage4KArgs<STAGE4_LONG>& a, hipStream_t s) { return launch_stage1(a, s); }
template <int MAXB>
static hipError_t launch_stage4(const Stage4KArgs<MAXB>& ka, bool tail, hipStream_t s) {
    if (tail && (ka.nblk < 2 || ka.nblk + 1 > MAXB || !ka.y1[ka.nblk])) return hipErrorInvalidValue;
    if (ka.nblk <= 0 || ka.nblk > MAXB || ka.N <= 0 || !ka.blk || !ka.grp_ctr || !ka.xch || !ka.xcc ||
        (ka.nblk > 1 && (!ka.per_image || !ka.img_ctr || ka.tiles_x != 1)))
        return hipErrorInvalidValue;
    const int tiles = ka.N * ka.tiles_per_img;
    const dim3 grid(ka.per_image ? (ka.N + 7) / 8 * ka.tiles_per_img * 4 * 8 : (tiles + 7) / 8 * 32), block(512);
    if (tail) hipLaunchKernelGGL((conv_stage4_c256_kernel<MAXB, true>), grid, block, 0, s, ka);
    else hipLaunchKernelGGL((conv_stage4_c256_kernel<MAXB, false>), grid, block, 0, s, ka);
    return hipGetLastError();
}
hipError_t launch_conv_stage4(const Stage4KArgs<STAGE4_SHORT>& a, bool tail, hipStream_t s) { return launch_stage4(a, tail, s); }
hipError_t launch_conv_stage4(const Stage4KArgs<STAGE4_LONG>& a, bool tail, hipStream_t s) { return launch_stage4(a, tail, s); }

}
```

### anakin_amd/csrc/kernels.h

```cpp
#pragma once
#include <hip/hip_runtime.h>
#include <stddef.h>
#include <stdint.h>

#ifdef SABER_TIMELINE
extern __device__ unsigned long long* saber_tl_buf;
#define SABER_TL_DECL unsigned long long tl_[16] = {0, 0, 0, 0, 0, 0, 0, 0, 0, 0, 0, 0, 0, 0, 0, 0}
#define SABER_TL(i) tl_[i] = wall_clock64()
#define SABER_TL_FLUSH()                                                                   \
    do {                                                                                   \
        if (threadIdx.x == 0 && saber_tl_buf)                                              \
            for (int i_ = 0; i_ < 16; ++i_) saber_tl_buf[(size_t)blockIdx.x * 16 + i_] = tl_[i_]; \
    } while (0)
#else
#define SABER_TL_DECL do { } while (0)
#define SABER_TL(i) do { } while (0)
#define SABER_TL_FLUSH() do { } while (0)
#endif

namespace saber_mi355x {

enum { DT_F32 = 0, DT_S8 = 1, DT_U8 = 2 };

enum {
// ... 80 lines not shown
    void* y2;
    int M, in_u8;
    int relu1, res_relu;
    float coeff_conv, scale_conv, coeff_res, scale_res;
    int relu2, out_u8_2;
    const void* prm0;
    const void* zero;
    int N, H, W;
    int tiles_x, tiles_per_img;
    unsigned mg_tiles_x, mg_tpi;
    int in0_u8, relu0;
    int s0, H0, W0;
    int res_sub, res_H, res_W;
    void* y2b;
    int k2_split, relu2b, out_u8_2b;
};
struct CoopKArgs {
    ChainKArgs c;
    unsigned long long* coop_ctr;
    void* coop_xch;
    unsigned* coop_xcc;
    unsigned* coop_err;
    int n_tiles;
};
bool conv1x1_chain_ok(int c1, int k1, int k2);
hipError_t launch_conv1x1_chain(const ChainKArgs& a, int c1, int k1, int k2, int rows, int waves, int split, int with3x3, hipStream_t s);
hipError_t launch_conv_chain_coop(const CoopKArgs& a, hipStream_t s);

struct StageBlk {
    const void* wstream;
    const void* prm0;
    const void* prm1;
    const void* prm2;
    float coeff_conv, scale_conv, coeff_res, scale_res;
    int in0_u8, relu0, in_u8, relu1, res_relu, relu2, out_u8_2, pad_;
};
template <int MAXB>
struct Stage4KArgs {
    const void* x;
    const void* res;
    const void* zero;
    const StageBlk* blk;
    unsigned long long* grp_ctr;
    unsigned long long* img_ctr;
    void* xch;
    unsigned* xcc;
    unsigned* err;
    int nblk, N, H, W;
    int tiles_x, tiles_per_img;
    unsigned mg_tiles_x, mg_tpi, mg_wpi;
    int per_image;
    void* y1[MAXB];
    void* y2[MAXB];
};
constexpr int STAGE4_SHORT = 8, STAGE4_LONG = 24;
hipError_t launch_conv_stage4(const Stage4KArgs<STAGE4_SHORT>& a, bool tail, hipStream_t s);
hipError_t launch_conv_stage4(const Stage4KArgs<STAGE4_LONG>& a, bool tail, hipStream_t s);
hipError_t launch_conv_stage1_c128(const Stage4KArgs<STAGE4_SHORT>& a, hipStream_t s);
hipError_t launch_conv_stage1_c128(const Stage4KArgs<STAGE4_LONG>& a, hipStream_t s);

struct StagePhase {
    int type;
    int cin, cout;
    int in_t, out_t, res_t;
    int in_u8, relu, out_u8;
    int elt, res_relu;
    float coeff_conv, scale_conv, coeff_res, scale_res;
    unsigned w_chunk, prm_chunk;
    int barrier;
    int reload;
    unsigned pch, mg_pch;
    int red_chunk;
    int pool_t;
    float pool_idiv;
};
static_assert(sizeof(StagePhase) == 96, "StagePhase layout");
struct StageKArgs {
    const StagePhase* phases;
    const void* weights;
    const void* prm;
    const void* zero;
    unsigned long long* sync;
    int n_phases, n_barriers;
    int n_img, H, W;
    unsigned long long* trace;
    void* t[STAGE_MAX_TENSORS];
};
bool stage_xcd_type(int tiles_per_cu, int ksteps_per_wave, int is3x3, int* type);
hipError_t launch_stage_xcd(const StageKArgs& a, size_t lds_bytes, hipStream_t s);
hipError_t launch_img_conv(const StageKArgs& a, size_t lds_bytes, hipStream_t s);

__device__ __forceinline__ void pin_hot_args(const ConvKArgs& a) {
    asm volatile("" ::"s"(a.x), "s"(a.w), "s"(a.zero), "s"(a.npx), "s"(a.nky), "s"(a.mg_npx), "s"(a.Kg_pad), "s"(a.M), "s"(a.OH),
                 "s"(a.OW), "s"(a.inv_ohw), "s"(a.inv_ow), "s"(a.H), "s"(a.W), "s"(a.C), "s"(a.stride_h), "s"(a.stride_w),
                 "s"(a.pad_h), "s"(a.pad_w), "s"(a.dil_h), "s"(a.dil_w), "s"(a.kh), "s"(a.kw), "s"(a.steps), "s"(a.in_u8));
}

enum { TILE_32x32 = 0, TILE_64x32 = 1, TILE_64x64 = 2, TILE_128x64 = 3, TILE_64x128 = 4, TILE_128x128 = 5,
       TILE_COUNT = 6,
       TILE_W8_64x64 = 6, TILE_W8_128x64 = 7, TILE_W8_128x128 = 8, TILE_W8_256x128 = 9, TILE_COUNT_B3 = 10 };
void tile_dims(int tile, int* bm_k, int* bn_pix);

hipError_t launch_conv_igemm(int mode, int tile, int ks, const ConvKArgs& a, hipStream_t s);
hipError_t launch_conv_igemm_dma(int mode, int tile, int ks, int wg, const ConvKArgs& a, hipStream_t s);
hipError_t launch_conv3x3_halo(int th, const ConvKArgs& a, hipStream_t s);
hipError_t launch_conv3x3_img(const ConvKArgs& a, int nw, int ib, int rb, hipStream_t s);
bool conv3x3_img_feasible(int C, int OW, int OH, int N, int nw, int ib, int rb);
bool conv3x3_b3h_variant(int variant, int* bmk, int* th, int* tm, int* threads);
bool conv1x1_pw_ok(int c, int k);
hipError_t launch_conv1x1_pw(const ConvKArgs& a, hipStream_t s);
// ... 99 lines not shown
```

### anakin_amd/lib.py

```python
import ctypes as C
import os

HERE = os.path.dirname(os.path.abspath(__file__))
LIB_PATH = os.environ.get("SABER_MI355X_LIB") or os.path.join(HERE, "libsaber_mi355x.so")

F32, S8, U8, S32 = 0, 1, 2, 3
NHWC, NCHW = 0, 1
ACT_NONE, ACT_RELU = 0, 1
POOL_MAX, POOL_AVG_INCL, POOL_AVG_EXCL = 0, 1, 2
RES_NONE, RES_SUM_INPLACE, RES_ELTWISE = 0, 1, 2
TILES = ["32x32", "64x32", "64x64", "128x64", "64x128", "128x128"]

SYMBOLS = [
    "saber_hip_last_error", "saber_hip_device_ok",
    "saber_hip_conv2d_create", "saber_hip_conv2d_set_weights", "saber_hip_conv2d_workspace_bytes",
    "saber_hip_conv2d_out_shape", "saber_hip_conv2d_run", "saber_hip_conv2d_destroy",
    "saber_hip_conv2d_get_quantized_weights", "saber_hip_conv2d_algo", "saber_hip_conv2d_set_tile",
    "saber_hip_conv2d_get_tile", "saber_hip_conv2d_autotune", "saber_hip_conv2d_set_pooling",
    "saber_hip_conv2d_create_pair", "saber_hip_conv2d_run_pair", "saber_hip_conv2d_autotune_pair",
    "saber_hip_net_add_conv_pair",
    "saber_hip_conv2d_chain_create", "saber_hip_conv2d_chain_create3", "saber_hip_conv2d_chain_create3_pair", "saber_hip_conv2d_chain_destroy", "saber_hip_conv2d_chain_run",
    "saber_hip_conv2d_chain_run3",
    "saber_hip_conv2d_chain_set_tile", "saber_hip_conv2d_chain_get_tile",
    "saber_hip_conv2d_stage_create", "saber_hip_conv2d_stage_destroy", "saber_hip_conv2d_stage_run", "saber_hip_conv2d_stage_create_tail", "saber_hip_conv2d_stage_run_tail",
    "saber_hip_conv2d_stem_pair_create", "saber_hip_conv2d_stem_pair_destroy", "saber_hip_conv2d_stem_pair_run",
    "saber_hip_conv2d_sep_create", "saber_hip_conv2d_sep_run", "saber_hip_conv2d_sep_set_tile", "saber_hip_conv2d_sep_get_tile",
    "saber_hip_conv2d_sep_algo", "saber_hip_conv2d_sep_destroy",
    "saber_hip_conv2d_set_global_pooling", "saber_hip_conv2d_run_gpool",
    "saber_hip_stage_create", "saber_hip_stage_num_tensors", "saber_hip_stage_run", "saber_hip_stage_status", "saber_hip_stage_trace", "saber_hip_stage_destroy",
    "saber_hip_fc_create", "saber_hip_fc_set_weights", "saber_hip_fc_workspace_bytes", "saber_hip_fc_run",
    "saber_hip_fc_destroy", "saber_hip_fc_algo", "saber_hip_fc_set_tile", "saber_hip_gemm_f32", "saber_hip_gemm_f32_release_plans",
    "saber_hip_gemm_i8_create", "saber_hip_gemm_i8_workspace_bytes", "saber_hip_gemm_i8_run", "saber_hip_gemm_i8_destroy",
    "saber_hip_quantize_nchw_to_nhwc", "saber_hip_dequantize_nhwc_to_nchw",
    "saber_hip_transpose_nchw_to_nhwc_f32", "saber_hip_transpose_nhwc_to_nchw_f32",
    "saber_hip_quantize_flat_s8", "saber_hip_eltwise_sum_i8", "saber_hip_eltwise_sum_f32", "saber_hip_relu_f32", "saber_hip_activation_f32", "saber_hip_prelu_f32",
    "saber_hip_pool_out_dim", "saber_hip_pool_out_dim2", "saber_hip_pool2d_i8_nhwc", "saber_hip_pool2d_f32", "saber_hip_pool2d_f32_from_i8", "saber_hip_pool2d_f32_from_i8_q", "saber_hip_fc_run_q", "saber_hip_fc_run_softmax", "saber_hip_softmax_f32",
    "saber_hip_net_add_pool_f32_from_i8_q", "saber_hip_net_add_fc_q", "saber_hip_net_optimize", "saber_hip_net_num_launches", "saber_hip_net_tensor_unwritten", "saber_hip_net_get_choice", "saber_hip_net_set_choice", "saber_hip_net_stage_blocks", "saber_hip_net_time_op_in_pass", "saber_hip_net_status", "saber_hip_net_inject_coop_error", "saber_hip_net_coop_fallbacks", "saber_hip_coop_fallbacks_total",
    "saber_hip_net_create", "saber_hip_net_add_tensor", "saber_hip_net_add_conv", "saber_hip_net_add_fc",
    "saber_hip_net_add_quantize", "saber_hip_net_add_dequantize", "saber_hip_net_add_transpose_in_f32", "saber_hip_net_add_eltwise_i8",
    "saber_hip_net_add_eltwise_f32", "saber_hip_net_add_pool_i8", "saber_hip_net_add_pool_f32",
    "saber_hip_net_add_pool_f32_from_i8", "saber_hip_net_add_softmax", "saber_hip_net_set_lane", "saber_hip_net_finalize", "saber_hip_net_tensor_ptr",
    "saber_hip_net_arena_bytes", "saber_hip_net_num_ops", "saber_hip_net_run", "saber_hip_net_run_op",
    "saber_hip_net_capture", "saber_hip_net_replay", "saber_hip_net_time_ops", "saber_hip_net_time_pass", "saber_hip_net_op_work", "saber_hip_net_op_name",
    "saber_hip_net_autotune", "saber_hip_net_destroy",
    "saber_hip_net_add_relu_f32", "saber_hip_net_add_activation_f32", "saber_hip_net_bind_tensor", "saber_hip_net_num_tensors", "saber_hip_net_tensor_bytes",
    "saber_hip_capture_begin", "saber_hip_capture_end", "saber_hip_capture_active", "saber_hip_net_tensor_of_ptr",
    "saber_hip_net_compact_arena", "saber_hip_net_arena_compacted", "saber_hip_serving_streams",
]


class StagePhase(C.Structure):
    _fields_ = [("conv", C.c_void_p), ("in_", C.c_int), ("out", C.c_int), ("res", C.c_int)]


class ConvDesc(C.Structure):
    _fields_ = [(n, C.c_int) for n in
                ("n", "h", "w", "c", "k", "kh", "kw", "pad_h", "pad_w", "stride_h", "stride_w", "dil_h", "dil_w",
                 "group", "in_dtype", "out_dtype", "in_layout", "out_layout", "act", "res_mode", "res_act")] + \
               [("sum_scale", C.c_float), ("coeff_conv", C.c_float), ("coeff_res", C.c_float),
                ("scale_res", C.c_float), ("int8_weights", C.c_int), ("act_negative_slope", C.c_float),
                ("res_has_dtype", C.c_int), ("res_dtype", C.c_int), ("res_stride", C.c_int), ("res_h", C.c_int),
                ("res_w", C.c_int)]


class FcDesc(C.Structure):
    _fields_ = [(n, C.c_int) for n in ("m", "n", "k", "in_dtype", "int8_weights", "w_is_kn")]


class SaberHipError(RuntimeError):
    pass


_lib = None


def load():
    global _lib
    if _lib is not None:
        return _lib
    try:
        import torch
    except ImportError:
        pass
    if not os.path.exists(LIB_PATH):
        raise SaberHipError(
            "anakin_amd/libsaber_mi355x.so is missing - build it with `python anakin_amd/build.py` "
            "(there is no CPU fallback for the MI355X Saber target)")
    lib = C.CDLL(LIB_PATH)
    P, I, F, Z = C.c_void_p, C.c_int, C.c_float, C.c_size_t
    lib.saber_hip_last_error.restype = C.c_char_p
    lib.saber_hip_conv2d_create.argtypes = [C.POINTER(ConvDesc), C.POINTER(P)]
    lib.saber_hip_conv2d_set_weights.argtypes = [P, P, I, P, P, F, F]
    lib.saber_hip_conv2d_workspace_bytes.argtypes = [P]
    lib.saber_hip_conv2d_workspace_bytes.restype = Z
    lib.saber_hip_conv2d_out_shape.argtypes = [P, C.POINTER(I), C.POINTER(I)]
    lib.saber_hip_conv2d_out_shape.restype = None
    lib.saber_hip_conv2d_run.argtypes = [P, P, P, P, P, P]
    lib.saber_hip_conv2d_destroy.argtypes = [P]
    lib.saber_hip_conv2d_destroy.restype = None
    lib.saber_hip_conv2d_get_quantized_weights.argtypes = [P, P, P]
    lib.saber_hip_conv2d_algo.argtypes = [P]
    lib.saber_hip_conv2d_algo.restype = C.c_char_p
    lib.saber_hip_conv2d_set_tile.argtypes = [P, I]
    lib.saber_hip_conv2d_get_tile.argtypes = [P]
    lib.saber_hip_conv2d_set_pooling.argtypes = [P] + [I] * 8
    lib.saber_hip_conv2d_autotune.argtypes = [P, P, P, P, P, P, I]
    lib.saber_hip_conv2d_create_pair.argtypes = [P, P, C.POINTER(P)]
    lib.saber_hip_conv2d_run_pair.argtypes = [P, P, P, P, P]
    lib.saber_hip_conv2d_autotune_pair.argtypes = [P, P, P, P, P, I]
    lib.saber_hip_net_add_conv_pair.argtypes = [P, P, I, I, I]
    lib.saber_hip_conv2d_chain_create.argtypes = [P, P, C.POINTER(P)]
    lib.saber_hip_conv2d_chain_create3.argtypes = [P, P, P, C.POINTER(P)]
    lib.saber_hip_net_tensor_unwritten.argtypes = [P, I]
    lib.saber_hip_net_num_launches.argtypes = [P]
    lib.saber_hip_conv2d_chain_destroy.argtypes = [P]
    lib.saber_hip_conv2d_chain_destroy.restype = None
    lib.saber_hip_conv2d_chain_run.argtypes = [P, P, P, P, P, P]
    lib.saber_hip_conv2d_chain_create3_pair.argtypes = [P, P, P, P, C.POINTER(P)]
    lib.saber_hip_conv2d_chain_run3.argtypes = [P, P, P, P, P, P, P]
    lib.saber_hip_conv2d_chain_set_tile.argtypes = [P, I]
    lib.saber_hip_conv2d_chain_get_tile.argtypes = [P]
    lib.saber_hip_conv2d_stage_create.argtypes = [C.POINTER(P), I, C.POINTER(P)]
    lib.saber_hip_conv2d_stage_destroy.argtypes = [P]
    lib.saber_hip_conv2d_stage_destroy.restype = None
    lib.saber_hip_conv2d_stage_run.argtypes = [P, P, P, C.POINTER(P), C.POINTER(P), P]
    lib.saber_hip_conv2d_stage_create_tail.argtypes = [C.POINTER(P), I, P, C.POINTER(P)]
    lib.saber_hip_conv2d_stage_run_tail.argtypes = [P, P, P, C.POINTER(P), C.POINTER(P), P, P]
    lib.saber_hip_conv2d_stem_pair_create.argtypes = [P, P, P, C.POINTER(P)]
    lib.saber_hip_conv2d_stem_pair_destroy.argtypes = [P]
    lib.saber_hip_conv2d_stem_pair_destroy.restype = None
    lib.saber_hip_conv2d_stem_pair_run.argtypes = [P, P, P, P, P, P, P]
    lib.saber_hip_conv2d_sep_create.argtypes = [P, P, C.POINTER(P)]
    lib.saber_hip_conv2d_sep_run.argtypes = [P, P, P, P, P]
    lib.saber_hip_conv2d_sep_set_tile.argtypes = [P, I]
    lib.saber_hip_conv2d_sep_get_tile.argtypes = [P]
    lib.saber_hip_conv2d_sep_algo.argtypes = [P]
    lib.saber_hip_conv2d_sep_algo.restype = C.c_char_p
    lib.saber_hip_conv2d_sep_destroy.argtypes = [P]
    lib.saber_hip_conv2d_sep_destroy.restype = None
    lib.saber_hip_conv2d_set_global_pooling.argtypes = [P]
    lib.saber_hip_conv2d_run_gpool.argtypes = [P, P, P, P, P, P]
    lib.saber_hip_stage_create.argtypes = [C.POINTER(StagePhase), I, C.POINTER(P)]
    lib.saber_hip_stage_num_tensors.argtypes = [P]
    lib.saber_hip_stage_run.argtypes = [P, C.POINTER(P), I, P]
    lib.saber_hip_stage_status.argtypes = [P]
    lib.saber_hip_stage_trace.argtypes = [P, P, C.c_size_t]
    lib.saber_hip_stage_destroy.argtypes = [P]
    lib.saber_hip_stage_destroy.restype = None
    lib.saber_hip_fc_create.argtypes = [C.POINTER(FcDesc), C.POINTER(P)]
    lib.saber_hip_fc_set_weights.argtypes = [P, P, I, P, P, F, F]
    lib.saber_hip_fc_workspace_bytes.argtypes = [P]
    lib.saber_hip_fc_workspace_bytes.restype = Z
    lib.saber_hip_fc_run.argtypes = [P, P, P, P, P]
    lib.saber_hip_fc_destroy.argtypes = [P]
    lib.saber_hip_net_optimize.argtypes = [P, I]
    lib.saber_hip_net_stage_blocks.argtypes = [P, I]
    lib.saber_hip_net_status.argtypes = [P]
    lib.saber_hip_net_inject_coop_error.argtypes = [P]
    lib.saber_hip_net_coop_fallbacks.argtypes = [P]
    lib.saber_hip_coop_fallbacks_total.argtypes = []
    lib.saber_hip_net_time_op_in_pass.argtypes = [P, P, I, I, C.POINTER(C.c_float)]
    lib.saber_hip_net_get_choice.argtypes = [P, I]
    lib.saber_hip_net_set_choice.argtypes = [P, I, I]
    lib.saber_hip_fc_algo.argtypes = [P]
    lib.saber_hip_fc_algo.restype = C.c_char_p
    lib.saber_hip_fc_set_tile.argtypes = [P, I]
    lib.saber_hip_fc_destroy.restype = None
    lib.saber_hip_gemm_f32.argtypes = [I, I, I, I, I, F, P, P, F, P, P]
    lib.saber_hip_gemm_f32_release_plans.argtypes = []
    lib.saber_hip_gemm_f32_release_plans.restype = I
    lib.saber_hip_gemm_i8_create.argtypes = [I, I, I, I, I, I, P, C.POINTER(P)]
    lib.saber_hip_gemm_i8_workspace_bytes.argtypes = [P]
    lib.saber_hip_gemm_i8_workspace_bytes.restype = Z
    lib.saber_hip_gemm_i8_run.argtypes = [P, P, P, P, P]
    lib.saber_hip_gemm_i8_destroy.argtypes = [P]
    lib.saber_hip_gemm_i8_destroy.restype = None
    lib.saber_hip_quantize_nchw_to_nhwc.argtypes = [I, I, I, I, I, I, F, P, P, P]
    lib.saber_hip_dequantize_nhwc_to_nchw.argtypes = [I, I, I, I, I, F, P, P, P]
    lib.saber_hip_transpose_nchw_to_nhwc_f32.argtypes = [I, I, I, I, I, P, P, P]
    lib.saber_hip_transpose_nhwc_to_nchw_f32.argtypes = [I, I, I, I, I, P, P, P]
    lib.saber_hip_quantize_flat_s8.argtypes = [Z, F, P, P, P]
    lib.saber_hip_eltwise_sum_i8.argtypes = [Z, P, P, F, F, F, F, I, P, P]
    lib.saber_hip_eltwise_sum_f32.argtypes = [Z, P, P, F, F, I, P, P]
    lib.saber_hip_pool_out_dim.argtypes = [I, I, I, I, I]
    lib.saber_hip_pool_out_dim2.argtypes = [I, I, I, I, I, I]
    lib.saber_hip_pool2d_i8_nhwc.argtypes = [I] * 15 + [P, P, P]
    lib.saber_hip_pool2d_f32.argtypes = [I] * 14 + [P, P, P]
    lib.saber_hip_pool2d_f32_from_i8.argtypes = [I] * 14 + [F, P, P, P]
    lib.saber_hip_pool2d_f32_from_i8_q.argtypes = [I] * 14 + [F, P, P, F, P, P]
    lib.saber_hip_fc_run_q.argtypes = [P, P, P, P]
    lib.saber_hip_net_add_pool_f32_from_i8_q.argtypes = [P] + [I] * 14 + [F, I, I, F, I]
    lib.saber_hip_net_add_fc_q.argtypes = [P, P, I, I]
    lib.saber_hip_softmax_f32.argtypes = [I, I, P, P, P]
    lib.saber_hip_relu_f32.argtypes = [Z, P, P, P]
    lib.saber_hip_activation_f32.argtypes = [I, Z, F, F, P, P, P]
    lib.saber_hip_prelu_f32.argtypes = [Z, I, I, I, P, P, P, P]
    lib.saber_hip_net_create.argtypes = [C.POINTER(P)]
    lib.saber_hip_net_add_tensor.argtypes = [P, Z]
    lib.saber_hip_net_add_conv.argtypes = [P, P, I, I, I]
    lib.saber_hip_net_add_fc.argtypes = [P, P, I, I]
    lib.saber_hip_net_add_quantize.argtypes = [P, I, I, I, I, I, I, F, I, I]
    lib.saber_hip_net_add_dequantize.argtypes = [P, I, I, I, I, I, F, I, I]
    lib.saber_hip_net_add_transpose_in_f32.argtypes = [P, I, I, I, I, I, I, I]
    lib.saber_hip_net_add_eltwise_i8.argtypes = [P, Z, F, F, F, F, I, I, I, I]
    lib.saber_hip_net_add_eltwise_f32.argtypes = [P, Z, F, F, I, I, I, I]
    lib.saber_hip_net_add_pool_i8.argtypes = [P] + [I] * 17
    lib.saber_hip_net_add_pool_f32.argtypes = [P] + [I] * 16
    lib.saber_hip_net_add_pool_f32_from_i8.argtypes = [P] + [I] * 14 + [F, I, I]
    lib.saber_hip_net_add_softmax.argtypes = [P, I, I, I, I]
# ... 67 lines not shown
```

### anakin_amd/saber.py

```python
import ctypes as C

import numpy as np
import torch

from . import lib as L

_TORCH_DT = {L.F32: torch.float32, L.S8: torch.int8, L.U8: torch.uint8}


def _stream():
    return C.c_void_p(torch.cuda.current_stream().cuda_stream)


def _p(t):
    return None if t is None else C.c_void_p(t.data_ptr())


def _np_ptr(a):
    return None if a is None else a.ctypes.data_as(C.c_void_p)


def dtype_code(t):
    return {torch.float32: L.F32, torch.int8: L.S8, torch.uint8: L.U8}[t.dtype]

# ... 219 lines not shown

ACTIVE_SIGMOID, ACTIVE_RELU, ACTIVE_TANH, ACTIVE_CLIPPED_RELU, ACTIVE_ELU, ACTIVE_STANH, ACTIVE_PRELU, ACTIVE_GELU, ACTIVE_SWISH = \
    1, 2, 3, 4, 5, 9, 10, 11, 12


def activation(active, x, y=None, negative_slope=0.0, coef=1.0):
    import torch
    if y is None:
        y = torch.empty_like(x)
    L.check(L.load().saber_hip_activation_f32(int(active), x.numel(), float(negative_slope), float(coef), _p(x), _p(y), _stream()))
    return y


def prelu(x, slope, channels, inner, channel_shared=False, y=None):
    import torch
    if y is None:
        y = torch.empty_like(x)
    L.check(L.load().saber_hip_prelu_f32(x.numel(), int(channels), int(inner), int(bool(channel_shared)), _p(slope), _p(x), _p(y), _stream()))
    return y


class SaberConvChain:

    def __init__(self, a, b, conv3x3=None, pair_b=None):
        self.a, self.b, self.c3, self.b2 = a, b, conv3x3, pair_b
        self.h = C.c_void_p()
        if pair_b is not None:
            L.check(L.load().saber_hip_conv2d_chain_create3_pair(conv3x3.h, a.h, b.h, pair_b.h, C.byref(self.h)))
        elif conv3x3 is None:
            L.check(L.load().saber_hip_conv2d_chain_create(a.h, b.h, C.byref(self.h)))
        else:
            L.check(L.load().saber_hip_conv2d_chain_create3(conv3x3.h, a.h, None if b is None else b.h, C.byref(self.h)))

    def dispatch(self, x, res, ya, yb=None, yc=None):
        L.check(L.load().saber_hip_conv2d_chain_run3(self.h, _p(x), _p(res), _p(ya), _p(yb), _p(yc), _stream()))
        return ya, yb

    def set_tile(self, tn):
        L.check(L.load().saber_hip_conv2d_chain_set_tile(self.h, tn))

    def tile(self):
        return L.load().saber_hip_conv2d_chain_get_tile(self.h)

    def __del__(self):
        try:
            if self.h:
                L.load().saber_hip_conv2d_chain_destroy(self.h)
        except Exception:
            pass


class SaberChainStage:

    def __init__(self, chains, tail=None):
        self.chains = list(chains)
        self.tail = tail
        arr = (C.c_void_p * len(chains))(*[c.h for c in chains])
        self.h = C.c_void_p()
        if tail is None:
            L.check(L.load().saber_hip_conv2d_stage_create(arr, len(chains), C.byref(self.h)))
        else:
            L.check(L.load().saber_hip_conv2d_stage_create_tail(arr, len(chains), tail.h, C.byref(self.h)))

    def dispatch(self, x, res, y1s, y2s, y_tail=None):
        n = len(self.chains)
        a = (C.c_void_p * n)(*[t.data_ptr() for t in y1s])
        b = (C.c_void_p * n)(*[t.data_ptr() for t in y2s])
        if y_tail is None:
            L.check(L.load().saber_hip_conv2d_stage_run(self.h, _p(x), _p(res), a, b, _stream()))
        else:
            L.check(L.load().saber_hip_conv2d_stage_run_tail(self.h, _p(x), _p(res), a, b, _p(y_tail), _stream()))

    def __del__(self):
        try:
            if self.h:
                L.load().saber_hip_conv2d_stage_destroy(self.h)
        except Exception:
            pass


class SaberStemPair:

    def __init__(self, stem, a, b):
        self.ops = (stem, a, b)
        self.h = C.c_void_p()
        L.check(L.load().saber_hip_conv2d_stem_pair_create(stem.h, a.h, b.h, C.byref(self.h)))

    def dispatch(self, x, y_a, y_b, y_pool=None):
        stem = self.ops[0]
        ws = stem.ws if hasattr(stem, "ws") else stem.conv.ws
        L.check(L.load().saber_hip_conv2d_stem_pair_run(self.h, _p(x), _p(y_pool), _p(y_a), _p(y_b), _p(ws), _stream()))

    def __del__(self):
        try:
            if self.h:
                L.load().saber_hip_conv2d_stem_pair_destroy(self.h)
        except Exception:
            pass


class SaberConvSep:

    def __init__(self, dw, pw):
        self.ops = (dw, pw)
        self.h = C.c_void_p()
        L.check(L.load().saber_hip_conv2d_sep_create(dw.h, pw.h, C.byref(self.h)))

    def dispatch(self, x, y_pw, y_dw=None):
        L.check(L.load().saber_hip_conv2d_sep_run(self.h, _p(x), _p(y_dw), _p(y_pw), _stream()))
        return y_pw

    def set_tile(self, code):
        L.check(L.load().saber_hip_conv2d_sep_set_tile(self.h, code))

    def tile(self):
        return L.load().saber_hip_conv2d_sep_get_tile(self.h)

    def algo(self):
        return L.load().saber_hip_conv2d_sep_algo(self.h).decode()

    def __del__(self):
        try:
            if self.h:
                L.load().saber_hip_conv2d_sep_destroy(self.h)
# ... 379 lines not shown
            cur.wait_stream(side)
        else:
            L.check(L.load().saber_hip_net_capture(self.h, _stream()))

    def replay(self):
        L.check(L.load().saber_hip_net_replay(self.h, _stream()))

    def autotune(self, iters=5):
        L.check(L.load().saber_hip_net_autotune(self.h, _stream(), iters))

    def choices(self):
        lib = L.load()
        return [int(lib.saber_hip_net_get_choice(self.h, i)) for i in range(self.num_ops())]

    def set_choices(self, choices):
        lib = L.load()
        assert len(choices) == self.num_ops()
        for i, c in enumerate(choices):
            L.check(lib.saber_hip_net_set_choice(self.h, i, int(c)))

    def status(self):
        L.check(L.load().saber_hip_net_status(self.h))

    def coop_fallbacks(self):
        return L.load().saber_hip_net_coop_fallbacks(self.h)

    def stages(self):
        lib = L.load()
        out = []
        for i in range(self.num_ops()):
            n = int(lib.saber_hip_net_stage_blocks(self.h, i))
            if n:
                out.append((i, n, bool(int(lib.saber_hip_net_get_choice(self.h, i)) >> 30 & 1)))
        return out

    def select_stages(self, on):
        ch = self.choices()
        for i, _, _ in self.stages():
            ch[i] = (ch[i] | (1 << 30)) if on else (ch[i] & ~(1 << 30))
        self.set_choices(ch)

    def tails(self):
        ch = self.choices()
        return [(i, n) for i, n, on in self.stages() if on and (ch[i] >> 31) & 1]

    def select_tails(self, on):
        ch = self.choices()
        for i, _, sel in self.stages():
            if sel:
                v = ((ch[i] | (1 << 31)) if on else (ch[i] & ~(1 << 31))) & 0xffffffff
                ch[i] = v - (1 << 32) if v >> 31 else v
        self.set_choices(ch)

    def time_ops(self, iters=20):
        out = (C.c_float * self.num_ops())()
        L.check(L.load().saber_hip_net_time_ops(self.h, _stream(), iters, out))
        return list(out)

    def time_op_in_pass(self, index, iters=20):
        out = C.c_float()
        L.check(L.load().saber_hip_net_time_op_in_pass(self.h, _stream(), int(index), int(iters), C.byref(out)))
        return float(out.value)

    def time_pass(self, iters=20):
        out = (C.c_float * self.num_ops())()
        L.check(L.load().saber_hip_net_time_pass(self.h, _stream(), iters, out))
        return list(out)

    def op_work(self, index):
        b, f = C.c_double(), C.c_double()
        L.check(L.load().saber_hip_net_op_work(self.h, int(index), C.byref(b), C.byref(f)))
        return b.value, f.value

    def arena_bytes(self):
        return L.load().saber_hip_net_arena_bytes(self.h)

    def compact(self, keep=()):
        ids = (C.c_int * max(1, len(keep)))(*[self.tensors[k][0] for k in keep])
        L.check(L.load().saber_hip_net_compact_arena(self.h, ids, len(keep)))
        return self.arena_bytes()

    def compacted(self):
        return bool(L.load().saber_hip_net_arena_compacted(self.h))

    def tensor_of_ptr(self, t):
        return int(L.load().saber_hip_net_tensor_of_ptr(self.h, t.data_ptr()))

    def bind(self, tid, t):
        self.keep.append(t)
        L.check(L.load().saber_hip_net_bind_tensor(self.h, int(tid), t.data_ptr()))

    def num_tensors(self):
        return int(L.load().saber_hip_net_num_tensors(self.h))


class Capture:

    def __init__(self, keep=()):
        self.net = None
        self._keep = list(keep)

    def __enter__(self):
        L.check(L.load().saber_hip_capture_begin())
        return self

    def __exit__(self, et, ev, tb):
# ... 24 lines not shown
```

### include/saber_hip.h

```cpp
#ifndef SABER_HIP_H
#define SABER_HIP_H

#include <stddef.h>
#include <stdint.h>

#ifdef __cplusplus
extern "C" {
#endif

typedef void* saber_hip_stream_t;

typedef enum {
    SABER_HIP_OK = 0,
    SABER_HIP_INVALID_VALUE = -2,
    SABER_HIP_UNIMPL = -3,
    SABER_HIP_OUT_OF_MEM = -4,
    SABER_HIP_RUNTIME_ERROR = -5
} saber_hip_status;

typedef enum { SABER_HIP_F32 = 0, SABER_HIP_S8 = 1, SABER_HIP_U8 = 2, SABER_HIP_S32 = 3 } saber_hip_dtype;
typedef enum { SABER_HIP_NHWC = 0, SABER_HIP_NCHW = 1 } saber_hip_layout;
typedef enum { SABER_HIP_ACT_NONE = 0, SABER_HIP_ACT_RELU = 1 } saber_hip_act;
typedef enum { SABER_HIP_POOL_MAX = 0, SABER_HIP_POOL_AVG_INCL = 1, SABER_HIP_POOL_AVG_EXCL = 2 } saber_hip_pool_type;

// ... 25 lines not shown
    int res_dtype;
    int res_stride;
    int res_h, res_w;
} saber_hip_conv_desc;

typedef struct saber_hip_conv saber_hip_conv_t;

int saber_hip_conv2d_create(const saber_hip_conv_desc* desc, saber_hip_conv_t** out);
int saber_hip_conv2d_set_weights(saber_hip_conv_t* op, const void* w, int w_dtype, const float* w_scale,
                                 const float* bias, float in_scale, float out_scale);
size_t saber_hip_conv2d_workspace_bytes(const saber_hip_conv_t* op);
void saber_hip_conv2d_out_shape(const saber_hip_conv_t* op, int* oh, int* ow);
int saber_hip_conv2d_run(saber_hip_conv_t* op, const void* x, void* y, const void* res, void* workspace,
                         saber_hip_stream_t stream);
void saber_hip_conv2d_destroy(saber_hip_conv_t* op);
int saber_hip_conv2d_set_pooling(saber_hip_conv_t* op, int pool_type, int kh, int kw, int stride_h, int stride_w,
                                 int pad_h, int pad_w, int floor_mode);
int saber_hip_conv2d_get_quantized_weights(const saber_hip_conv_t* op, int8_t* wq_oihw, float* w_scale);
const char* saber_hip_conv2d_algo(const saber_hip_conv_t* op);
int saber_hip_conv2d_set_tile(saber_hip_conv_t* op, int tile);
int saber_hip_conv2d_get_tile(const saber_hip_conv_t* op);
int saber_hip_conv2d_autotune(saber_hip_conv_t* op, const void* x, void* y, const void* res, void* workspace,
                              saber_hip_stream_t stream, int iters);

int saber_hip_conv2d_set_global_pooling(saber_hip_conv_t* op);
int saber_hip_conv2d_run_gpool(saber_hip_conv_t* op, const void* x, void* y, const void* res, void* y_pool,
                               saber_hip_stream_t stream);

int saber_hip_conv2d_create_pair(const saber_hip_conv_t* a, const saber_hip_conv_t* b, saber_hip_conv_t** out);
int saber_hip_conv2d_run_pair(saber_hip_conv_t* pair, const void* x, void* y_a, void* y_b, saber_hip_stream_t stream);
int saber_hip_conv2d_autotune_pair(saber_hip_conv_t* pair, const void* x, void* y_a, void* y_b,
                                   saber_hip_stream_t stream, int iters);

typedef struct saber_hip_chain saber_hip_chain_t;
int saber_hip_conv2d_chain_create(saber_hip_conv_t* a, saber_hip_conv_t* b, saber_hip_chain_t** out);
int saber_hip_conv2d_chain_create3(saber_hip_conv_t* conv3x3, saber_hip_conv_t* a, saber_hip_conv_t* b, saber_hip_chain_t** out);
int saber_hip_conv2d_chain_create3_pair(saber_hip_conv_t* conv3x3, saber_hip_conv_t* a, saber_hip_conv_t* pair_a, saber_hip_conv_t* pair_b,
                                        saber_hip_chain_t** out);
void saber_hip_conv2d_chain_destroy(saber_hip_chain_t* chain);
int saber_hip_conv2d_chain_run(saber_hip_chain_t* chain, const void* x, const void* res, void* y_a, void* y_b,
                               saber_hip_stream_t stream);
int saber_hip_conv2d_chain_run3(saber_hip_chain_t* chain, const void* x, const void* res, void* y_a, void* y_b, void* y_c,
                                saber_hip_stream_t stream);
int saber_hip_conv2d_chain_set_tile(saber_hip_chain_t* chain, int tn);
int saber_hip_conv2d_chain_get_tile(const saber_hip_chain_t* chain);

typedef struct saber_hip_chain_stage saber_hip_chain_stage_t;
int saber_hip_conv2d_stage_create(saber_hip_chain_t* const* chains, int n, saber_hip_chain_stage_t** out);
void saber_hip_conv2d_stage_destroy(saber_hip_chain_stage_t* stage);
int saber_hip_conv2d_stage_run(saber_hip_chain_stage_t* stage, const void* x, const void* res, void* const* y1, void* const* y2,
                               saber_hip_stream_t stream);
int saber_hip_conv2d_stage_create_tail(saber_hip_chain_t* const* chains, int n, saber_hip_chain_t* tail, saber_hip_chain_stage_t** out);
int saber_hip_conv2d_stage_run_tail(saber_hip_chain_stage_t* stage, const void* x, const void* res, void* const* y1, void* const* y2,
                                    void* y_tail, saber_hip_stream_t stream);

typedef struct saber_hip_stem_pair saber_hip_stem_pair_t;
int saber_hip_conv2d_stem_pair_create(saber_hip_conv_t* stem, const saber_hip_conv_t* a, const saber_hip_conv_t* b, saber_hip_stem_pair_t** out);
void saber_hip_conv2d_stem_pair_destroy(saber_hip_stem_pair_t* sp);
int saber_hip_conv2d_stem_pair_run(saber_hip_stem_pair_t* sp, const void* x, void* y_pool, void* y_a, void* y_b, void* workspace,
                                   saber_hip_stream_t stream);

typedef struct saber_hip_sep saber_hip_sep_t;
int saber_hip_conv2d_sep_create(saber_hip_conv_t* dw, saber_hip_conv_t* pw, saber_hip_sep_t** out);
int saber_hip_conv2d_sep_run(saber_hip_sep_t* sep, const void* x, void* y_dw , void* y_pw, saber_hip_stream_t stream);
int saber_hip_conv2d_sep_set_tile(saber_hip_sep_t* sep, int code);
int saber_hip_conv2d_sep_get_tile(const saber_hip_sep_t* sep);
const char* saber_hip_conv2d_sep_algo(const saber_hip_sep_t* sep);
void saber_hip_conv2d_sep_destroy(saber_hip_sep_t* sep);

typedef struct saber_hip_stage saber_hip_stage_t;
typedef struct {
    saber_hip_conv_t* conv;
    int in, out, res;
} saber_hip_stage_phase;
int saber_hip_stage_create(const saber_hip_stage_phase* phases, int n_phases, saber_hip_stage_t** out);
int saber_hip_stage_num_tensors(const saber_hip_stage_t* stage);
int saber_hip_stage_run(saber_hip_stage_t* stage, void* const* tensors, int n_tensors, saber_hip_stream_t stream);
int saber_hip_stage_status(saber_hip_stage_t* stage);
int saber_hip_stage_trace(saber_hip_stage_t* stage, unsigned long long* out, size_t cap);
void saber_hip_stage_destroy(saber_hip_stage_t* stage);

typedef struct {
    int m, n, k;
    int in_dtype;
    int int8_weights;
    int w_is_kn;
} saber_hip_fc_desc;
typedef struct saber_hip_fc saber_hip_fc_t;
int saber_hip_fc_create(const saber_hip_fc_desc* desc, saber_hip_fc_t** out);
int saber_hip_fc_set_weights(saber_hip_fc_t* op, const void* w, int w_dtype, const float* w_scale,
                             const float* bias, float in_scale, float out_scale);
size_t saber_hip_fc_workspace_bytes(const saber_hip_fc_t* op);
int saber_hip_fc_run(saber_hip_fc_t* op, const void* x, float* y, void* workspace, saber_hip_stream_t stream);
int saber_hip_fc_run_q(saber_hip_fc_t* op, const int8_t* xq, float* y, saber_hip_stream_t stream);
int saber_hip_fc_run_softmax(saber_hip_fc_t* op, const void* x, float* y, float* prob, void* workspace, saber_hip_stream_t stream);
const char* saber_hip_fc_algo(const saber_hip_fc_t* op);
int saber_hip_fc_set_tile(saber_hip_fc_t* op, int tile);
void saber_hip_fc_destroy(saber_hip_fc_t* op);

int saber_hip_gemm_f32(int trans_a, int trans_b, int m, int n, int k, float alpha, const float* a,
                       const float* b, float beta, float* c, saber_hip_stream_t stream);
int saber_hip_gemm_f32_release_plans(void);

typedef struct saber_hip_gemm_i8 saber_hip_gemm_i8_t;
int saber_hip_gemm_i8_create(int trans_a, int trans_b, int m, int n, int k, int a_dtype, const int8_t* b_host,
                             saber_hip_gemm_i8_t** out);
// ... 24 lines not shown
int saber_hip_pool_out_dim2(int in, int pad, int window, int stride, int floor_mode, int any_pad);
int saber_hip_pool2d_i8_nhwc(int n, int h, int w, int c, int oh, int ow, int kh, int kw, int stride_h,
                             int stride_w, int pad_h, int pad_w, int pool_type, int in_dtype, int out_dtype,
                             const void* x, void* y, saber_hip_stream_t stream);
int saber_hip_pool2d_f32(int n, int h, int w, int c, int oh, int ow, int kh, int kw, int stride_h,
                         int stride_w, int pad_h, int pad_w, int pool_type, int layout, const float* x,
                         float* y, saber_hip_stream_t stream);
int saber_hip_pool2d_f32_from_i8(int n, int h, int w, int c, int oh, int ow, int kh, int kw, int stride_h,
                                 int stride_w, int pad_h, int pad_w, int pool_type, int in_dtype, float scale,
                                 const void* x, float* y, saber_hip_stream_t stream);
int saber_hip_pool2d_f32_from_i8_q(int n, int h, int w, int c, int oh, int ow, int kh, int kw, int stride_h,
                                   int stride_w, int pad_h, int pad_w, int pool_type, int in_dtype, float scale,
                                   const void* x, float* y, float q_scale, int8_t* yq, saber_hip_stream_t stream);
int saber_hip_softmax_f32(int rows, int cols, const float* x, float* y, saber_hip_stream_t stream);

typedef struct saber_hip_net saber_hip_net_t;
int saber_hip_net_create(saber_hip_net_t** out);
int saber_hip_net_add_tensor(saber_hip_net_t* net, size_t bytes);
int saber_hip_net_add_conv(saber_hip_net_t* net, saber_hip_conv_t* op, int in_id, int out_id, int res_id);
int saber_hip_net_add_conv_pair(saber_hip_net_t* net, saber_hip_conv_t* pair, int in_id, int out_a_id, int out_b_id);
int saber_hip_net_add_fc(saber_hip_net_t* net, saber_hip_fc_t* op, int in_id, int out_id);
int saber_hip_net_add_quantize(saber_hip_net_t* net, int n, int c, int h, int w, int c_pad, int out_dtype,
                               float scale, int in_id, int out_id);
int saber_hip_net_add_dequantize(saber_hip_net_t* net, int n, int c, int h, int w, int in_dtype, float scale,
                                 int in_id, int out_id);
int saber_hip_net_add_transpose_in_f32(saber_hip_net_t* net, int n, int c, int h, int w, int c_pad, int in_id,
                                       int out_id);
int saber_hip_net_add_eltwise_i8(saber_hip_net_t* net, size_t count, float scale_a, float scale_b,
                                 float coeff_a, float coeff_b, int relu, int a_id, int b_id, int out_id);
int saber_hip_net_add_eltwise_f32(saber_hip_net_t* net, size_t count, float coeff_a, float coeff_b, int relu,
                                  int a_id, int b_id, int out_id);
int saber_hip_net_add_pool_i8(saber_hip_net_t* net, int n, int h, int w, int c, int oh, int ow, int kh, int kw,
                              int stride_h, int stride_w, int pad_h, int pad_w, int pool_type, int in_dtype,
                              int out_dtype, int in_id, int out_id);
int saber_hip_net_add_pool_f32(saber_hip_net_t* net, int n, int h, int w, int c, int oh, int ow, int kh, int kw,
                               int stride_h, int stride_w, int pad_h, int pad_w, int pool_type, int layout,
                               int in_id, int out_id);
int saber_hip_net_add_pool_f32_from_i8(saber_hip_net_t* net, int n, int h, int w, int c, int oh, int ow, int kh,
                                       int kw, int stride_h, int stride_w, int pad_h, int pad_w, int pool_type,
                                       int in_dtype, float scale, int in_id, int out_id);
int saber_hip_net_add_pool_f32_from_i8_q(saber_hip_net_t* net, int n, int h, int w, int c, int oh, int ow, int kh, int kw,
                                         int stride_h, int stride_w, int pad_h, int pad_w, int pool_type, int in_dtype,
                                         float scale, int in_id, int out_id, float q_scale, int q_out_id);
int saber_hip_net_add_fc_q(saber_hip_net_t* net, saber_hip_fc_t* op, int in_q_id, int out_id);
#define SABER_HIP_NET_SHARED_DEVICE 2048
#define SABER_HIP_NET_REPRODUCIBLE_FP32 8192
#define SABER_HIP_NET_SEPARABLE 16384
int saber_hip_net_optimize(saber_hip_net_t* net, int flags);
int saber_hip_net_coop_fallbacks(const saber_hip_net_t* net);
int saber_hip_coop_fallbacks_total(void);
int saber_hip_net_status(saber_hip_net_t* net);
int saber_hip_net_inject_coop_error(saber_hip_net_t* net);
int saber_hip_net_stage_blocks(const saber_hip_net_t* net, int index);
int saber_hip_net_num_launches(const saber_hip_net_t* net);
int saber_hip_net_tensor_unwritten(const saber_hip_net_t* net, int id);
int saber_hip_net_add_softmax(saber_hip_net_t* net, int rows, int cols, int in_id, int out_id);
int saber_hip_net_set_lane(saber_hip_net_t* net, int op_index, int lane);
int saber_hip_net_finalize(saber_hip_net_t* net);
void* saber_hip_net_tensor_ptr(saber_hip_net_t* net, int id);
size_t saber_hip_net_arena_bytes(const saber_hip_net_t* net);
int saber_hip_net_compact_arena(saber_hip_net_t* net, const int* keep, int n_keep);
int saber_hip_net_arena_compacted(const saber_hip_net_t* net);
int saber_hip_net_num_ops(const saber_hip_net_t* net);
int saber_hip_net_run(saber_hip_net_t* net, saber_hip_stream_t stream);
int saber_hip_net_run_op(saber_hip_net_t* net, int index, saber_hip_stream_t stream);
int saber_hip_net_capture(saber_hip_net_t* net, saber_hip_stream_t stream);
int saber_hip_net_replay(saber_hip_net_t* net, saber_hip_stream_t stream);
int saber_hip_net_time_ops(saber_hip_net_t* net, saber_hip_stream_t stream, int iters, float* out_us);
int saber_hip_net_time_pass(saber_hip_net_t* net, saber_hip_stream_t stream, int iters, float* out_us);
int saber_hip_net_time_op_in_pass(saber_hip_net_t* net, saber_hip_stream_t stream, int index, int iters, float* out_us);
int saber_hip_net_op_work(const saber_hip_net_t* net, int index, double* bytes, double* flops);
const char* saber_hip_net_op_name(const saber_hip_net_t* net, int index);
int saber_hip_net_get_choice(saber_hip_net_t* net, int index);
int saber_hip_net_set_choice(saber_hip_net_t* net, int index, int choice);
int saber_hip_net_autotune(saber_hip_net_t* net, saber_hip_stream_t stream, int iters);
void saber_hip_net_destroy(saber_hip_net_t* net);
int saber_hip_net_add_relu_f32(saber_hip_net_t* net, size_t count, int in_id, int out_id);
int saber_hip_net_add_activation_f32(saber_hip_net_t* net, int active, size_t count, float negative_slope, float coef, int in_id,
                                     int out_id);
int saber_hip_net_bind_tensor(saber_hip_net_t* net, int id, void* ptr);
int saber_hip_net_num_tensors(const saber_hip_net_t* net);
size_t saber_hip_net_tensor_bytes(const saber_hip_net_t* net, int id);

int saber_hip_capture_begin(void);
int saber_hip_capture_end(saber_hip_net_t** out);
int saber_hip_capture_active(void);
int saber_hip_net_tensor_of_ptr(const saber_hip_net_t* net, const void* ptr);

int saber_hip_serving_streams(int n, saber_hip_stream_t* out, int* distinct);

#ifdef __cplusplus
}
#endif
#endif
```

Before: 37890.

## Fuse the stage-3 head 1x1 conv pair into the cooperative stage launch

Adds an optional head to the C=256 cooperative stage kernel. The two 1x1 convs that read the 512-channel stage input (the 1024-channel shortcut projection and the 256-channel reduce) are packed into a weight stream and run inside the same stage launch instead of as a separate conv-pair launch. This removes one kernel launch and a round trip of the intermediate tensors through memory. In exchange it adds validation, packing, net-graph wiring, and an autotune choice bit. It is gated by autotune (chain bit 32, not on shared devices), so whether it is used by default depends on the tuner picking it.

Measured after the change: 38410, median of 6. +1.4%, better.

```diff
diff --git a/anakin_amd/csrc/api_chain.hip b/anakin_amd/csrc/api_chain.hip
--- a/anakin_amd/csrc/api_chain.hip
+++ b/anakin_amd/csrc/api_chain.hip
@@ -121,6 +121,16 @@
                 const int j = jj < 2 ? kh * 2 + jj : 4 + kh * 6 + (jj - 2);
                 pack_frag1(b->wq_oihw.data(), K1, q * 64 + nt * 16, 1, 0, (q * 4 + j) & 15, out);
             }
+        }
+}
+static void pack_stage_head_stream(const saber_hip_conv* a, const saber_hip_conv* b, std::vector<uint8_t>& out) {
+    const int C0 = 512;
+    for (int q = 0; q < 4; ++q)
+        for (int w = 0; w < 8; ++w) {
+            const int nt = w & 3, kh = w >> 2;
+            for (int ks = 0; ks < 8; ++ks)
+                for (int mf = 0; mf < 2; ++mf) pack_frag1(a->wq_oihw.data(), C0, q * 256 + w * 32, 2, mf, ks, out);
+            for (int j = 0; j < 4; ++j) pack_frag1(b->wq_oihw.data(), C0, q * 64 + nt * 16, 1, 0, kh * 4 + j, out);
         }
 }
 static void pack_stage1_c128_stream(const saber_hip_conv* c3, const saber_hip_conv* a, const saber_hip_conv* b, std::vector<uint8_t>& out) {
@@ -195,8 +205,30 @@
     delete stage1;
 }
 static unsigned div_magic(int d) { return d >= 2 ? (unsigned)((0x100000000ull + (unsigned)d - 1) / (unsigned)d) : 0u; }
-static int stage_build(saber_hip_chain* const* chains, int n, bool per_image, saber_hip_chain* tail, saber_hip_chain_stage** out) {
+static int stage_build(saber_hip_chain* const* chains, int n, bool per_image, saber_hip_chain* tail, saber_hip_chain_stage** out,
+                       const saber_hip_conv* head_a = nullptr, const saber_hip_conv* head_b = nullptr) {
     if (!chains || n <= 0 || n > saber_mi355x::STAGE4_LONG || !out) return fail(SABER_HIP_INVALID_VALUE, "stage: 1..24 chains");
+    if (head_a || head_b) {
+        if (!head_a || !head_b) return fail(SABER_HIP_INVALID_VALUE, "null argument");
+        if (!chains[0] || chains[0]->c1 != 256) return fail(SABER_HIP_INVALID_VALUE, "stage: a head goes with a C = 256 stage only");
+        if (!per_image) return fail(SABER_HIP_INVALID_VALUE, "stage: a head needs an image per XCD");
+        for (const saber_hip_conv* o : {head_a, head_b})
+            if (o->d.res_mode != SABER_HIP_RES_NONE) return fail(SABER_HIP_INVALID_VALUE, "stage: the head's convs carry no residual");
+        for (const saber_hip_conv* o : {head_a, head_b}) {
+            const saber_hip_conv_desc& d = o->d;
+            if (!o->is_i8 || !o->weights_set || o->algo != ALGO_IGEMM_I8 || o->epi != EPI_I8_CONV || o->pair_k2 || o->pool_fused || o->pool2 || o->gpool ||
+                o->pre_quant || o->pre_pad || d.kh != 1 || d.kw != 1 || d.stride_h != 1 || d.stride_w != 1 || d.pad_h != 0 || d.pad_w != 0 || d.group != 1 ||
+                o->c_eff != d.c || d.act_negative_slope != 0.f || d.in_layout != SABER_HIP_NHWC || d.out_layout != SABER_HIP_NHWC ||
+                (d.out_dtype != SABER_HIP_S8 && d.out_dtype != SABER_HIP_U8))
+                return fail(SABER_HIP_INVALID_VALUE, "stage: the head must be two plain 1x1 / stride 1 / pad 0 INT8 NHWC convs with weights set");
+        }
+        if (head_a->d.c != 512 || head_b->d.c != 512) return fail(SABER_HIP_INVALID_VALUE, "stage: the head's convs read 512 channels");
+        if (head_a->d.k != 1024 || head_b->d.k != 256) return fail(SABER_HIP_INVALID_VALUE, "stage: the head's convs write 1024 and 256 channels");
+        const saber_hip_conv_desc &d0 = chains[0]->a->d, &da = head_a->d, &db = head_b->d;
+        if (!chains[0]->c3 || da.n != d0.n || da.h != d0.h || da.w != d0.w || db.n != d0.n || db.h != d0.h || db.w != d0.w || head_a->x_dtype != head_b->x_dtype ||
+            da.out_dtype != SABER_HIP_S8 || (db.out_dtype == SABER_HIP_U8) != (chains[0]->c3->x_dtype == DT_U8))
+            return fail(SABER_HIP_INVALID_VALUE, "stage: the head's outputs must be the first block's shortcut (s8) and 3x3 input (its dtype), one input tensor");
+    }
     if (tail) {
         if (!chains[0] || chains[0]->c1 != 256 || tail->c1 != 256) return fail(SABER_HIP_INVALID_VALUE, "stage: a tail goes with a C = 256 stage only");
         if (n < 2 || !per_image || n + 1 > saber_mi355x::STAGE4_LONG) return fail(SABER_HIP_INVALID_VALUE, "stage: a tail needs 2..23 blocks, an image per XCD");
@@ -265,6 +297,22 @@
         blk.push_back(B);
         st->tail = tail;
     }
+    if (head_a) {
+        std::vector<uint8_t> hs, p1, p2;
+        pack_stage_head_stream(head_a, head_b, hs);
+        pack_chain_params(head_a, (size_t)head_a->d.k / 4 * 3, p1);
+        pack_chain_params(head_b, ((size_t)head_b->d.k / 4 * 3 + 63) / 64 * 64 + 64, p2);
+        if (e == hipSuccess) e = st->d_head_stream.upload(hs);
+        if (e == hipSuccess) e = st->d_head_prm1.upload(p1);
+        if (e == hipSuccess) e = st->d_head_prm2.upload(p2);
+        saber_mi355x::StageBlk B;
+        std::memset(&B, 0, sizeof B);
+        B.wstream = st->d_head_stream.p; B.prm0 = st->d_head_prm2.p; B.prm1 = st->d_head_prm1.p; B.prm2 = st->d_head_prm2.p;
+        B.in_u8 = head_a->x_dtype == DT_U8; B.relu1 = head_a->d.act == SABER_HIP_ACT_RELU;
+        B.relu2 = head_b->d.act == SABER_HIP_ACT_RELU; B.out_u8_2 = head_b->d.out_dtype == SABER_HIP_U8;
+        blk.insert(blk.begin(), B);
+        st->head_a = head_a; st->head_b = head_b;
+    }
     if (e == hipSuccess) e = st->d_blk.upload(blk);
     if (e == hipSuccess && st->c1 == 256) e = st->d_grp_ctr.alloc_zero(tiles * 32);
     if (e == hipSuccess) e = st->d_img_ctr.alloc_zero((size_t)d0.n * (st->tiles_per_img + 1) * 16);
@@ -280,30 +328,32 @@
     return SABER_HIP_OK;
 }
 template <int MAXB>
-static int stage_launch(saber_hip_chain_stage* st, const void* x, const void* res, void* const* y1, void* const* y2, void* y_tail, hipStream_t s) {
+static int stage_launch(saber_hip_chain_stage* st, const void* x, const void* res, void* const* y1, void* const* y2, void* y_tail, void* y_head, hipStream_t s) {
     saber_mi355x::Stage4KArgs<MAXB> k;
     std::memset(&k, 0, sizeof k);
     k.x = x; k.res = res; k.zero = zero_page();
     if (!k.zero) return fail(SABER_HIP_RUNTIME_ERROR, "stage: zero page");
-    k.blk = st->d_blk.p; k.grp_ctr = st->d_grp_ctr.p; k.img_ctr = st->d_img_ctr.p; k.xch = st->d_xch.p; k.xcc = st->d_xcc.p; k.err = st->h_err;
+    k.blk = st->d_blk.p + (st->head_a ? 1 : 0); k.grp_ctr = st->d_grp_ctr.p; k.img_ctr = st->d_img_ctr.p; k.xch = st->d_xch.p; k.xcc = st->d_xcc.p; k.err = st->h_err;
     k.nblk = (int)st->chains.size(); k.N = st->n; k.H = st->h; k.W = st->w;
     k.tiles_x = st->tiles_x; k.tiles_per_img = st->tiles_per_img;
     k.mg_tiles_x = div_magic(st->tiles_x); k.mg_tpi = div_magic(st->tiles_per_img); k.mg_wpi = div_magic(st->tiles_per_img * 4);
     k.per_image = st->per_image;
     for (int i = 0; i < k.nblk; ++i) { k.y1[i] = y1[i]; k.y2[i] = y2[i]; }
     if (y_tail) k.y1[k.nblk] = y_tail;
-    HIP_TRY(st->c1 == 256 ? saber_mi355x::launch_conv_stage4(k, y_tail != nullptr, s) : saber_mi355x::launch_conv_stage1_c128(k, s));
+    k.head_y = y_head;
+    HIP_TRY(st->c1 == 256 ? saber_mi355x::launch_conv_stage4(k, y_tail != nullptr, y_head != nullptr, s) : saber_mi355x::launch_conv_stage1_c128(k, s));
     return SABER_HIP_OK;
 }
-int stage_run(saber_hip_chain_stage* st, const void* x, const void* res, void* const* y1, void* const* y2, hipStream_t s, void* y_tail) {
+int stage_run(saber_hip_chain_stage* st, const void* x, const void* res, void* const* y1, void* const* y2, hipStream_t s, void* y_tail, void* y_head) {
     if (y_tail && !st->tail) return fail(SABER_HIP_INVALID_VALUE, "stage: created without a tail");
+    if (y_head && !st->head_a) return fail(SABER_HIP_INVALID_VALUE, "stage: created without a head");
     if (*(volatile unsigned*)st->h_err) {
         *(volatile unsigned*)st->h_err = 0u;
         return fail(SABER_HIP_RUNTIME_ERROR, "cooperative stage: an earlier launch's workgroups did not share an XCD or timed out at a barrier "
                     "(its outputs are not valid)");
     }
-    return (int)st->chains.size() + (y_tail ? 1 : 0) <= saber_mi355x::STAGE4_SHORT ? stage_launch<saber_mi355x::STAGE4_SHORT>(st, x, res, y1, y2, y_tail, s)
-                                                                                   : stage_launch<saber_mi355x::STAGE4_LONG>(st, x, res, y1, y2, y_tail, s);
+    return (int)st->chains.size() + (y_tail ? 1 : 0) <= saber_mi355x::STAGE4_SHORT ? stage_launch<saber_mi355x::STAGE4_SHORT>(st, x, res, y1, y2, y_tail, y_head, s)
+                                                                                   : stage_launch<saber_mi355x::STAGE4_LONG>(st, x, res, y1, y2, y_tail, y_head, s);
 }
 int saber_hip_conv2d_stage_create(saber_hip_chain_t* const* chains, int n, saber_hip_chain_stage_t** out) {
     if (!xcd_round_robin()) return fail(SABER_HIP_UNIMPL, "stage: this device does not place workgroup b on XCD b % 8");
@@ -313,6 +363,12 @@
     if (!tail) return fail(SABER_HIP_INVALID_VALUE, "null argument");
     if (!xcd_round_robin()) return fail(SABER_HIP_UNIMPL, "stage: this device does not place workgroup b on XCD b % 8");
     return stage_build(chains, n, true, tail, out);
+}
+int saber_hip_conv2d_stage_create_head(saber_hip_chain_t* const* chains, int n, saber_hip_chain_t* tail, const saber_hip_conv_t* head_a,
+                                       const saber_hip_conv_t* head_b, saber_hip_chain_stage_t** out) {
+    if (!head_a || !head_b) return fail(SABER_HIP_INVALID_VALUE, "null argument");
+    if (!xcd_round_robin()) return fail(SABER_HIP_UNIMPL, "stage: this device does not place workgroup b on XCD b % 8");
+    return stage_build(chains, n, true, tail, out, head_a, head_b);
 }
 void saber_hip_conv2d_stage_destroy(saber_hip_chain_stage_t* st) { delete st; }
 int saber_hip_conv2d_stage_run(saber_hip_chain_stage_t* st, const void* x, const void* res, void* const* y1, void* const* y2, saber_hip_stream_t stream) {
@@ -329,6 +385,14 @@
     for (size_t i = 0; i < st->chains.size(); ++i)
         if (!y1[i] || !y2[i]) return fail(SABER_HIP_INVALID_VALUE, "stage: an output pointer per block");
     return stage_run(st, x, res, y1, y2, (hipStream_t)stream, y_tail);
+}
+int saber_hip_conv2d_stage_run_head(saber_hip_chain_stage_t* st, const void* x_head, void* y_head_b, void* const* y1, void* const* y2, void* y_tail,
+                                    saber_hip_stream_t stream) {
+    if (g_capture) return capture_unsupported("saber_hip_conv2d_stage_run_head (saber_hip_net_optimize forms stages itself)");
+    if (!st || !x_head || !y_head_b || !y1 || !y2) return fail(SABER_HIP_INVALID_VALUE, "null argument");
+    for (size_t i = 0; i < st->chains.size(); ++i)
+        if (!y1[i] || !y2[i]) return fail(SABER_HIP_INVALID_VALUE, "stage: an output pointer per block");
+    return stage_run(st, x_head, nullptr, y1, y2, (hipStream_t)stream, y_tail, y_head_b);
 }
 static void pack_chain_stream(const saber_hip_chain* ch, ChainStream layout, std::vector<uint8_t>& out) {
     const saber_hip_conv *c3 = ch->c3, *a = ch->a, *b = ch->b;
diff --git a/anakin_amd/csrc/api_internal.h b/anakin_amd/csrc/api_internal.h
--- a/anakin_amd/csrc/api_internal.h
+++ b/anakin_amd/csrc/api_internal.h
@@ -218,6 +218,9 @@
     std::vector<saber_hip_chain*> chains;
     saber_hip_chain* tail = nullptr;
     DevBuf<uint8_t> d_tail_stream;
+    const saber_hip_conv* head_a = nullptr;
+    const saber_hip_conv* head_b = nullptr;
+    DevBuf<uint8_t> d_head_stream, d_head_prm1, d_head_prm2;
     DevBuf<saber_mi355x::StageBlk> d_blk;
     DevBuf<unsigned long long> d_grp_ctr, d_img_ctr;
     DevBuf<uint8_t> d_xch;
@@ -341,6 +344,8 @@
     bool use_stage = false;
     bool use_tail = false;
     int tail_of = -1, tail_mode = 0;
+    bool use_head = false, head_req = false;
+    int head_of = -1;
     saber_hip_stem_pair* stem_pair = nullptr;
     int stem_y1 = -1, stem_y2 = -1;
     saber_hip_sep* sep = nullptr;
@@ -430,6 +435,7 @@
 void net_set_chain_mode(saber_hip_net* net, int ia, int mode);
 int net_chain_mode(const saber_hip_net* net, int ia);
 void net_set_stage(saber_hip_net* net, int i0, bool on);
+void net_set_head(saber_hip_net* net, int i0, bool on);
 void net_set_tail(saber_hip_net* net, int i0, bool on);
 ChainForm chain_form(const saber_hip_chain* ch, int code);
 bool chain_form_valid(const saber_hip_chain* ch, int code);
@@ -442,4 +448,5 @@
 void for_each_sep_form(const saber_hip_sep* sp, const std::function<void(int code)>& fn);
 int sep_static_form(const saber_hip_sep* sp);
 void net_set_sep(saber_hip_net* net, int i, int code);
-int stage_run(saber_hip_chain_stage* st, const void* x, const void* res, void* const* y1, void* const* y2, hipStream_t s, void* y_tail = nullptr);
+int stage_run(saber_hip_chain_stage* st, const void* x, const void* res, void* const* y1, void* const* y2, hipStream_t s, void* y_tail = nullptr,
+              void* y_head = nullptr);
diff --git a/anakin_amd/csrc/api_net.hip b/anakin_amd/csrc/api_net.hip
--- a/anakin_amd/csrc/api_net.hip
+++ b/anakin_amd/csrc/api_net.hip
@@ -17,7 +17,9 @@
                 y1[k] = T(ops[3 * k].chain3_y1);
                 y2[k] = T(ops[3 * k].chain3_y2);
             }
-            const int rc = stage_run(o.stage, T(o.in), T(o.chain3_res), y1, y2, s, o.use_tail ? T(ops[3 * o.stage_n].chain3_y1) : nullptr);
+            void* const y_tail = o.use_tail ? T(ops[3 * o.stage_n].chain3_y1) : nullptr;
+            const int rc = o.use_head ? stage_run(o.stage, T(ops[-1].in), nullptr, y1, y2, s, y_tail, T(o.in))
+                                      : stage_run(o.stage, T(o.in), T(o.chain3_res), y1, y2, s, y_tail);
             if (rc == SABER_HIP_RUNTIME_ERROR) {
                 ++net->coop_fallbacks;
                 ++g_coop_fallbacks_total;
@@ -287,6 +289,7 @@
     for (int i = 0; i < nops; ++i) {
         const NetOp& o = net->ops[i];
         if (o.stage) span(i, 3 * o.stage_n + (o.stage->tail ? 2 : 0));
+        if (o.stage && o.stage->head_a && i > 0) span(i - 1, 2);
         if (o.chain3) span(i, 3);
         if (o.chain) span(i, 2);
         if (o.stem_pair) span(i, 2);
@@ -640,6 +643,8 @@
     if (net->tensor_bytes[id] == 0) return 1;
     for (const NetOp& o : net->ops)
         if (((o.chain3 && o.use_chain3) || o.stem_pair || (o.sep && o.use_sep)) && o.out == id) return 1;
+    for (const NetOp& o : net->ops)
+        if (o.stage && o.use_head && o.chain3_res == id) return 1;
     return 0;
 }
 static void net_drop_graph(saber_hip_net* net) {
diff --git a/anakin_amd/csrc/api_net_autotune.hip b/anakin_amd/csrc/api_net_autotune.hip
--- a/anakin_amd/csrc/api_net_autotune.hip
+++ b/anakin_amd/csrc/api_net_autotune.hip
@@ -17,11 +17,16 @@
     if (c && net->ops[index].sep) choice |= (3 << 28) | ((net->ops[index].use_sep ? net->ops[index].sep->form : 0) << 24);
     if (c && net->ops[index].stage && net->ops[index].use_stage) choice |= 1 << 30;
     if (c && net->ops[index].stage && net->ops[index].use_tail) choice |= (int)0x80000000u;
+    if (c && net->ops[index].head_of >= 0 && net->ops[net->ops[index].head_of].use_head) choice |= 1 << 29;
     return choice;
 }
 int saber_hip_net_stage_blocks(const saber_hip_net_t* net, int index) {
     if (!net || index < 0 || index >= (int)net->ops.size()) return 0;
     return net->ops[index].stage ? net->ops[index].stage_n : 0;
+}
+int saber_hip_net_stage_head(const saber_hip_net_t* net, int index) {
+    if (!net || index < 1 || index >= (int)net->ops.size() || !net->ops[index].stage) return -1;
+    return net->ops[index - 1].head_of == index ? index - 1 : -1;
 }
 int saber_hip_net_set_choice(saber_hip_net_t* net, int index, int choice) {
     saber_hip_conv* c = net_op_conv(net, index);
@@ -50,12 +55,21 @@
     const bool in_stage = o.chain3 && o.skip && !o.stage;
     if (ch && ch == o.chain3) net_set_chain_mode(net, index + 1, (tn || in_stage) ? 2 : net_chain_mode(net, index + 1) == 2 ? 1 : net_chain_mode(net, index + 1));
     else if (ch) net_set_chain_mode(net, index, net_chain_mode(net, index) == 2 ? 2 : (tn ? 1 : 0));
+    const bool stage_was = o.stage && o.use_stage;
     if (o.stage) net_set_stage(net, index, stage_on);
     if (o.stage) net_set_tail(net, index, tail_on);
+    if (o.stage && stage_on && !stage_was) net_set_head(net, index, o.head_req);
+    if (o.stage) o.head_req = false;
+    if (o.head_of >= 0) {
+        const bool head_on = (chain_bits & 32) && !net->shared_device;
+        net->ops[o.head_of].head_req = head_on;
+        net_set_head(net, o.head_of, head_on);
+    }
     if (in_tail) net_set_tail(net, o.tail_of, true);
     if (o.skip) o.name = (o.chain3 && o.use_chain3) ? "conv:(in the stage launch)" : "conv:(in the chain launch)";
     if (o.skip && index > 0 && net->ops[index - 1].tail_of >= 0 && net->ops[net->ops[index - 1].tail_of].use_tail) o.name = "conv:(in the stage launch)";
     if (o.skip && o.kind == OP_CONV_PAIR) o.name = (index > 0 && net->ops[index - 1].stem_pair) ? "conv:(in the stem launch)" : "conv:(in the chain launch)";
+    if (o.skip && o.head_of >= 0 && net->ops[o.head_of].use_head) o.name = "conv:(in the stage launch)";
     if (o.stem_pair) o.name = stem_pair_name(o);
     if (o.sep) net_set_sep(net, index, sep_bits ? tn : (o.use_sep ? o.sep->form : 0));
     if (o.skip && index > 0 && net->ops[index - 1].sep && net->ops[index - 1].use_sep) o.name = "conv:(in the separable launch)";
@@ -230,11 +244,12 @@
         NetOp& H0 = net->ops[i];
         if (!H0.stage || net->shared_device) continue;
         const bool has_tail = H0.stage->tail != nullptr;
+        const bool has_head = saber_hip_net_stage_head(net, (int)i) >= 0;
         const int first = (int)i, last = first + 3 * H0.stage_n - 1 + (has_tail ? 2 : 0);
         hipStream_t s = (hipStream_t)stream;
         auto run_all = [&]() -> int {
             int rc = 0;
-            for (int k = first; k <= last; ++k) rc |= net_launch(net, net->ops[k], s);
+            for (int k = first - (has_head ? 1 : 0); k <= last; ++k) rc |= net_launch(net, net->ops[k], s);
             return rc;
         };
         auto timed = [&](float* t) { return time_enqueued(s, run_all, 20, t); };
@@ -260,6 +275,15 @@
             else if (ok_t && wt < one) one = wt;
             else net_set_tail(net, first, false);
         }
+        if (ok && one < sep && has_head) {
+            float wh = 0.f;
+            net_set_head(net, first, true);
+            const bool ok_h = timed(&wh) == SABER_HIP_OK && hipStreamSynchronize(s) == hipSuccess && !*(volatile unsigned*)H0.stage->h_err;
+            log_cand(H0.conv, H0.name.substr(5), ok_h ? wh : -1.f);
+            if (*(volatile unsigned*)H0.stage->h_err) ok = false;
+            else if (ok_h && wh < one * 0.99f) one = wh;
+            else net_set_head(net, first, false);
+        }
         if (!ok || one >= sep) {
             *(volatile unsigned*)H0.stage->h_err = 0u;
             net_set_stage(net, first, false);
diff --git a/anakin_amd/csrc/api_net_optimize.hip b/anakin_amd/csrc/api_net_optimize.hip
--- a/anakin_amd/csrc/api_net_optimize.hip
+++ b/anakin_amd/csrc/api_net_optimize.hip
@@ -12,7 +12,7 @@
     }
 }
 static std::string stage_name(const NetOp& H0) {
-    return "conv:stage_c" + std::to_string(H0.stage->c1) + "_" + std::to_string(H0.stage_n) + "x[conv3x3+chain1x1]_2x16" + (H0.stage->c1 == 256 ? "_coop4" : "") +
+    return std::string(H0.use_head ? "conv:[pair1x1]+stage_c" : "conv:stage_c") + std::to_string(H0.stage->c1) + "_" + std::to_string(H0.stage_n) + "x[conv3x3+chain1x1]_2x16" + (H0.stage->c1 == 256 ? "_coop4" : "") +
            (H0.use_tail ? "+[conv3x3/2+conv1x1]" : "");
 }
 void net_set_chain_mode(saber_hip_net* net, int ia, int mode) {
@@ -55,9 +55,21 @@
     if (on) net->ops[it + 1].name = "conv:(in the stage launch)";
     if (H0.use_stage) H0.name = stage_name(H0);
 }
+void net_set_head(saber_hip_net* net, int i0, bool on) {
+    NetOp& H0 = net->ops[i0];
+    if (!H0.stage || !H0.stage->head_a || i0 < 1 || net->ops[i0 - 1].head_of != i0) return;
+    NetOp& P = net->ops[i0 - 1];
+    on = on && H0.use_stage;
+    if (on == H0.use_head) return;
+    H0.use_head = on;
+    P.skip = on;
+    P.name = on ? std::string("conv:(in the stage launch)") : std::string("conv:") + P.conv->algo_name;
+    if (H0.use_stage) H0.name = stage_name(H0);
+}
 void net_set_stage(saber_hip_net* net, int i0, bool on) {
     NetOp& H0 = net->ops[i0];
     if (!H0.stage) return;
+    if (!on) net_set_head(net, i0, false);
     if (!on) net_set_tail(net, i0, false);
     for (int k = 0; k < H0.stage_n; ++k) {
         if (on || H0.use_stage) net_set_chain_mode(net, i0 + 3 * k + 1, 2);
@@ -443,12 +455,30 @@
                     ops[jt].chain3->c1 == 256 && ops[jt].chain3->c3->d.stride_h == 2 && ops[jt].in == ops[pl].chain3_y2 &&
                     ops[jt].chain3_res == ops[pl].chain3_y1 && ops[jt].chain3_y1 >= 0)
                     tail = ops[jt].chain3;
-                if (tail && saber_hip_conv2d_stage_create_tail(run.data(), (int)run.size(), tail, &st) != SABER_HIP_OK) tail = nullptr;
-                if (tail || saber_hip_conv2d_stage_create(run.data(), (int)run.size(), &st) == SABER_HIP_OK) {
+                const saber_hip_conv *head_a = nullptr, *head_b = nullptr;
+                if (i >= 1 && run[0]->c1 == 256 && ops[i - 1].kind == OP_CONV_PAIR && !ops[i - 1].skip && !ops[i - 1].lane && ops[i - 1].conv &&
+                    ops[i - 1].conv->pair_src_a && ops[i - 1].conv->pair_src_b && !(i >= 3 && ops[i - 3].chain3 && ops[i - 3].chain3->b2)) {
+                    const NetOp& P = ops[i - 1];
+                    const int t_res = ops[i].chain3_res, t_x = ops[i].in;
+                    auto readers = [&](int t) {
+                        int r = 0;
+                        for (const NetOp& o : ops) r += (o.in == t) + (o.in2 == t);
+                        return r;
+                    };
+                    const bool fwd = P.out == t_res && P.out2 == t_x, rev = P.out == t_x && P.out2 == t_res;
+                    if ((fwd || rev) && t_res != t_x && readers(t_res) == 1 && readers(t_x) == 1) {
+                        head_a = fwd ? P.conv->pair_src_a : P.conv->pair_src_b;
+                        head_b = fwd ? P.conv->pair_src_b : P.conv->pair_src_a;
+                    }
+                }
+                if (head_a && saber_hip_conv2d_stage_create_head(run.data(), (int)run.size(), tail, head_a, head_b, &st) != SABER_HIP_OK) head_a = head_b = nullptr;
+                if (!head_a && tail && saber_hip_conv2d_stage_create_tail(run.data(), (int)run.size(), tail, &st) != SABER_HIP_OK) tail = nullptr;
+                if (head_a || tail || saber_hip_conv2d_stage_create(run.data(), (int)run.size(), &st) == SABER_HIP_OK) {
                     net->owned_stages.push_back(st);
                     ops[i].stage = st;
                     ops[i].stage_n = (int)run.size();
                     if (tail) ops[jt].tail_of = (int)i;
+                    if (head_a) ops[i - 1].head_of = (int)i;
                     int before = 0;
                     for (size_t k = 0; k < run.size(); ++k) before += 3 - (ops[i + 3 * k].skip + ops[i + 3 * k + 1].skip + ops[i + 3 * k + 2].skip);
                     if (tail) before += 2 - (ops[jt].skip + ops[jt + 1].skip);
diff --git a/anakin_amd/csrc/conv_stage_coop.hip b/anakin_amd/csrc/conv_stage_coop.hip
--- a/anakin_amd/csrc/conv_stage_coop.hip
+++ b/anakin_amd/csrc/conv_stage_coop.hip
@@ -2,7 +2,7 @@
 
 namespace saber_mi355x {
 
-template <int MAXB, bool TAIL>
+template <int MAXB, bool TAIL, bool HEAD>
 __global__ __launch_bounds__(512) void conv_stage4_c256_kernel(const Stage4KArgs<MAXB> ka) {
     constexpr int C1 = 256, K1 = 1024, K2 = 256, NW = 8;
     constexpr int F0 = 18, F1 = 8, F2 = 8;
@@ -109,11 +109,12 @@
     };
     const int nall = ka.nblk + (TAIL ? 1 : 0);
 
+    v4i fr[F0 + 2];
+    if constexpr (!HEAD) {
     dma_halo(ka.x, false);
     lds_dma16((const char*)ka.res + (size_t)pt * K1 + q * K1Q + tc * 16, tile + wave * 64);
     dma_prm(ka.blk[0]);
     asm volatile("" ::: "memory");
-    v4i fr[F0 + 2];
     {
         const v4i* wsb = stream_of(ka.blk[0], FB);
 #pragma unroll
@@ -125,6 +126,122 @@
     wait_vm_older_than<F0 + 2>();
     __builtin_amdgcn_s_barrier();
     SABER_TL(1);
+    } else {
+        constexpr int C0 = 512, CH0 = C0 / 16, XPC = CH0 + 1;
+        constexpr int XCH = (32 * XPC + 63) / 64 * 64;
+        constexpr int FA = 2 * (C0 / 64), FH = (C0 / 64) / 2;
+        static_assert(XCH <= YCH && FA + FH == F0 + 2, "the head's tile fits ptile, its fragments the entry registers");
+        const StageBlk Bh = ka.blk[-1];
+        v4i* const xt = ptile;
+        for (int i = wave; i < XCH / 64; i += NW) {
+            const int L = i * 64 + lane;
+            const int px = L / XPC, cc = L - px * XPC;
+            bool okp;
+            const int pp_ = pix(px & 31, okp);
+            const char* src = (px < 32 && cc < CH0) ? (const char*)ka.x + ((size_t)pp_ * C0 + cc * 16) : (const char*)ka.zero;
+            lds_dma16(src, xt + i * 64);
+        }
+        dma_prm(Bh);
+        asm volatile("" ::: "memory");
+        {
+            const v4i* wsb = stream_of(Bh, FA + FH);
+#pragma unroll
+            for (int r = 0; r < FA + FH; ++r) {
+                fr[r] = wsb[r * 64];
+                asm volatile("" ::: "memory");
+            }
+        }
+        wait_vm_older_than<FA + FH>();
+        __builtin_amdgcn_s_barrier();
+        SABER_TL(12);
+        const v4i z = {0, 0, 0, 0};
+        const int xmask = Bh.in_u8 ? (int)0x80808080u : 0;
+        {
+            const int cg = wave * 32 + fq * 8;
+            const v4i* pp = prm1 + (cg / 4) * 3;
+            v4i acc[2][2];
+#pragma unroll
+            for (int m = 0; m < 2; ++m)
+#pragma unroll
+                for (int mf = 0; mf < 2; ++mf) acc[m][mf] = pp[mf * 3 + 2];
+#pragma unroll
+            for (int ks = 0; ks < C0 / 64; ++ks)
+#pragma unroll
+                for (int m = 0; m < 2; ++m) {
+                    v4i bo = xt[(m * 16 + frow) * XPC + ks * 4 + fq];
+                    bo.x ^= xmask; bo.y ^= xmask; bo.z ^= xmask; bo.w ^= xmask;
+                    acc[m][0] = mma_step(fr[ks * 2], bo, acc[m][0]);
+                    acc[m][1] = mma_step(fr[ks * 2 + 1], bo, acc[m][1]);
+                }
+            const float lo1 = Bh.relu1 ? 0.f : -3.0e38f;
+#pragma unroll
+            for (int m = 0; m < 2; ++m) {
+                c2i o;
+                o.x = (int)chain_out_pack(acc[m][0], z, __builtin_bit_cast(v4f, pp[1]), __builtin_bit_cast(v4f, pp[0]), lo1, 128.f, 0x80808080u);
+                o.y = (int)chain_out_pack(acc[m][1], z, __builtin_bit_cast(v4f, pp[4]), __builtin_bit_cast(v4f, pp[3]), lo1, 128.f, 0x80808080u);
+                *(c2i*)((char*)tile + ((m * 16 + frow) * CPRW + ((cg / 16) ^ frow)) * 16 + (fq & 1) * 8) = o;
+            }
+        }
+        SABER_TL(13);
+        const v4i* const ws0 = stream_of(ka.blk[0], FB);
+#pragma unroll
+        for (int r = 0; r < FA; ++r) {
+            fr[r] = ws0[r * 64];
+            asm volatile("" ::: "memory");
+        }
+        {
+            const int c2 = nt * 16 + fq * 4;
+            const v4i* pp = prm2 + (c2 / 4) * 3;
+            v4i acc0 = kh ? z : pp[2], acc1 = acc0;
+#pragma unroll
+            for (int j = 0; j < FH; ++j) {
+                v4i b0 = xt[frow * XPC + (kh * FH + j) * 4 + fq];
+                v4i b1 = xt[(16 + frow) * XPC + (kh * FH + j) * 4 + fq];
+                b0.x ^= xmask; b0.y ^= xmask; b0.z ^= xmask; b0.w ^= xmask;
+                b1.x ^= xmask; b1.y ^= xmask; b1.z ^= xmask; b1.w ^= xmask;
+                acc0 = mma_step(fr[FA + j], b0, acc0);
+                acc1 = mma_step(fr[FA + j], b1, acc1);
+            }
+#pragma unroll
+            for (int r = FA; r < FA + FH; ++r) {
+                fr[r] = ws0[r * 64];
+                asm volatile("" ::: "memory");
+            }
+            if (kh) {
+                red[(nt * 2 + 0) * 64 + lane] = acc0;
+                red[(nt * 2 + 1) * 64 + lane] = acc1;
+            }
+            asm volatile("s_waitcnt lgkmcnt(0)" ::: "memory");
+            __builtin_amdgcn_s_barrier();
+            if (!kh) {
+                const v4i r0 = red[(nt * 2 + 0) * 64 + lane], r1 = red[(nt * 2 + 1) * 64 + lane];
+                acc0.x += r0.x; acc0.y += r0.y; acc0.z += r0.z; acc0.w += r0.w;
+                acc1.x += r1.x; acc1.y += r1.y; acc1.z += r1.z; acc1.w += r1.w;
+                const float lo2 = Bh.relu2 ? 0.f : -3.0e38f;
+                const float off2 = Bh.out_u8_2 ? 0.f : 128.f;
+                const unsigned xm2 = Bh.out_u8_2 ? 0u : 0x80808080u;
+                const unsigned o0 = chain_out_pack(acc0, z, __builtin_bit_cast(v4f, pp[1]), __builtin_bit_cast(v4f, pp[0]), lo2, off2, xm2);
+                const unsigned o1 = chain_out_pack(acc1, z, __builtin_bit_cast(v4f, pp[1]), __builtin_bit_cast(v4f, pp[0]), lo2, off2, xm2);
+                if (ok0) *(unsigned*)((char*)ka.head_y + (size_t)p0 * K2 + q * K2Q + c2) = o0;
+                if (ok1) *(unsigned*)((char*)ka.head_y + (size_t)p1 * K2 + q * K2Q + c2) = o1;
+            }
+        }
+        SABER_TL(14);
+        asm volatile("s_waitcnt vmcnt(0)" ::: "memory");
+        __builtin_amdgcn_s_barrier();
+        unsigned long long* const e_h = e_up + 1;
+        if (wave == 0 && lane == 0) {
+            (void)__hip_atomic_fetch_add(e_h, 1ull, __ATOMIC_RELAXED, __HIP_MEMORY_SCOPE_WORKGROUP);
+            (void)__hip_atomic_fetch_add(e_h + 16, 1ull, __ATOMIC_RELAXED, __HIP_MEMORY_SCOPE_WORKGROUP);
+        }
+        dma_prm(ka.blk[0]);
+        if (wave == 0) coop_wait_mask2(e_h, ty > 0 ? 7ull : 3ull, e_h + 16, ty + 1 < ka.tiles_per_img ? 7ull : 3ull, ka.err);
+        __builtin_amdgcn_s_barrier();
+        dma_halo(ka.head_y, true);
+        wait_vm_older_than<0>();
+        __builtin_amdgcn_s_barrier();
+        SABER_TL(1);
+    }
 
     StageBlk B = ka.blk[0];
     for (int k = 0; k < ka.nblk; ++k) {
@@ -662,18 +779,21 @@
 hipError_t launch_conv_stage1_c128(const Stage4KArgs<STAGE4_SHORT>& a, hipStream_t s) { return launch_stage1(a, s); }
 hipError_t launch_conv_stage1_c128(const Stage4KArgs<STAGE4_LONG>& a, hipStream_t s) { return launch_stage1(a, s); }
 template <int MAXB>
-static hipError_t launch_stage4(const Stage4KArgs<MAXB>& ka, bool tail, hipStream_t s) {
+static hipError_t launch_stage4(const Stage4KArgs<MAXB>& ka, bool tail, bool head, hipStream_t s) {
     if (tail && (ka.nblk < 2 || ka.nblk + 1 > MAXB || !ka.y1[ka.nblk])) return hipErrorInvalidValue;
+    if (head && (!ka.per_image || !ka.img_ctr || ka.tiles_x != 1 || !ka.head_y)) return hipErrorInvalidValue;
     if (ka.nblk <= 0 || ka.nblk > MAXB || ka.N <= 0 || !ka.blk || !ka.grp_ctr || !ka.xch || !ka.xcc ||
         (ka.nblk > 1 && (!ka.per_image || !ka.img_ctr || ka.tiles_x != 1)))
         return hipErrorInvalidValue;
     const int tiles = ka.N * ka.tiles_per_img;
     const dim3 grid(ka.per_image ? (ka.N + 7) / 8 * ka.tiles_per_img * 4 * 8 : (tiles + 7) / 8 * 32), block(512);
-    if (tail) hipLaunchKernelGGL((conv_stage4_c256_kernel<MAXB, true>), grid, block, 0, s, ka);
-    else hipLaunchKernelGGL((conv_stage4_c256_kernel<MAXB, false>), grid, block, 0, s, ka);
+    if (head && tail) hipLaunchKernelGGL((conv_stage4_c256_kernel<MAXB, true, true>), grid, block, 0, s, ka);
+    else if (head) hipLaunchKernelGGL((conv_stage4_c256_kernel<MAXB, false, true>), grid, block, 0, s, ka);
+    else if (tail) hipLaunchKernelGGL((conv_stage4_c256_kernel<MAXB, true, false>), grid, block, 0, s, ka);
+    else hipLaunchKernelGGL((conv_stage4_c256_kernel<MAXB, false, false>), grid, block, 0, s, ka);
     return hipGetLastError();
 }
-hipError_t launch_conv_stage4(const Stage4KArgs<STAGE4_SHORT>& a, bool tail, hipStream_t s) { return launch_stage4(a, tail, s); }
-hipError_t launch_conv_stage4(const Stage4KArgs<STAGE4_LONG>& a, bool tail, hipStream_t s) { return launch_stage4(a, tail, s); }
+hipError_t launch_conv_stage4(const Stage4KArgs<STAGE4_SHORT>& a, bool tail, bool head, hipStream_t s) { return launch_stage4(a, tail, head, s); }
+hipError_t launch_conv_stage4(const Stage4KArgs<STAGE4_LONG>& a, bool tail, bool head, hipStream_t s) { return launch_stage4(a, tail, head, s); }
 
 }
diff --git a/anakin_amd/csrc/kernels.h b/anakin_amd/csrc/kernels.h
--- a/anakin_amd/csrc/kernels.h
+++ b/anakin_amd/csrc/kernels.h
@@ -156,10 +156,11 @@
     int per_image;
     void* y1[MAXB];
     void* y2[MAXB];
+    void* head_y;
 };
 constexpr int STAGE4_SHORT = 8, STAGE4_LONG = 24;
-hipError_t launch_conv_stage4(const Stage4KArgs<STAGE4_SHORT>& a, bool tail, hipStream_t s);
-hipError_t launch_conv_stage4(const Stage4KArgs<STAGE4_LONG>& a, bool tail, hipStream_t s);
+hipError_t launch_conv_stage4(const Stage4KArgs<STAGE4_SHORT>& a, bool tail, bool head, hipStream_t s);
+hipError_t launch_conv_stage4(const Stage4KArgs<STAGE4_LONG>& a, bool tail, bool head, hipStream_t s);
 hipError_t launch_conv_stage1_c128(const Stage4KArgs<STAGE4_SHORT>& a, hipStream_t s);
 hipError_t launch_conv_stage1_c128(const Stage4KArgs<STAGE4_LONG>& a, hipStream_t s);
 
diff --git a/anakin_amd/lib.py b/anakin_amd/lib.py
--- a/anakin_amd/lib.py
+++ b/anakin_amd/lib.py
@@ -23,6 +23,7 @@
     "saber_hip_conv2d_chain_run3",
     "saber_hip_conv2d_chain_set_tile", "saber_hip_conv2d_chain_get_tile",
     "saber_hip_conv2d_stage_create", "saber_hip_conv2d_stage_destroy", "saber_hip_conv2d_stage_run", "saber_hip_conv2d_stage_create_tail", "saber_hip_conv2d_stage_run_tail",
+    "saber_hip_conv2d_stage_create_head", "saber_hip_conv2d_stage_run_head",
     "saber_hip_conv2d_stem_pair_create", "saber_hip_conv2d_stem_pair_destroy", "saber_hip_conv2d_stem_pair_run",
     "saber_hip_conv2d_sep_create", "saber_hip_conv2d_sep_run", "saber_hip_conv2d_sep_set_tile", "saber_hip_conv2d_sep_get_tile",
     "saber_hip_conv2d_sep_algo", "saber_hip_conv2d_sep_destroy",
@@ -35,7 +36,7 @@
     "saber_hip_transpose_nchw_to_nhwc_f32", "saber_hip_transpose_nhwc_to_nchw_f32",
     "saber_hip_quantize_flat_s8", "saber_hip_eltwise_sum_i8", "saber_hip_eltwise_sum_f32", "saber_hip_relu_f32", "saber_hip_activation_f32", "saber_hip_prelu_f32",
     "saber_hip_pool_out_dim", "saber_hip_pool_out_dim2", "saber_hip_pool2d_i8_nhwc", "saber_hip_pool2d_f32", "saber_hip_pool2d_f32_from_i8", "saber_hip_pool2d_f32_from_i8_q", "saber_hip_fc_run_q", "saber_hip_fc_run_softmax", "saber_hip_softmax_f32",
-    "saber_hip_net_add_pool_f32_from_i8_q", "saber_hip_net_add_fc_q", "saber_hip_net_optimize", "saber_hip_net_num_launches", "saber_hip_net_tensor_unwritten", "saber_hip_net_get_choice", "saber_hip_net_set_choice", "saber_hip_net_stage_blocks", "saber_hip_net_time_op_in_pass", "saber_hip_net_status", "saber_hip_net_inject_coop_error", "saber_hip_net_coop_fallbacks", "saber_hip_coop_fallbacks_total",
+    "saber_hip_net_add_pool_f32_from_i8_q", "saber_hip_net_add_fc_q", "saber_hip_net_optimize", "saber_hip_net_num_launches", "saber_hip_net_tensor_unwritten", "saber_hip_net_get_choice", "saber_hip_net_set_choice", "saber_hip_net_stage_blocks", "saber_hip_net_stage_head", "saber_hip_net_time_op_in_pass", "saber_hip_net_status", "saber_hip_net_inject_coop_error", "saber_hip_net_coop_fallbacks", "saber_hip_coop_fallbacks_total",
     "saber_hip_net_create", "saber_hip_net_add_tensor", "saber_hip_net_add_conv", "saber_hip_net_add_fc",
     "saber_hip_net_add_quantize", "saber_hip_net_add_dequantize", "saber_hip_net_add_transpose_in_f32", "saber_hip_net_add_eltwise_i8",
     "saber_hip_net_add_eltwise_f32", "saber_hip_net_add_pool_i8", "saber_hip_net_add_pool_f32",
@@ -126,6 +127,8 @@
     lib.saber_hip_conv2d_stage_run.argtypes = [P, P, P, C.POINTER(P), C.POINTER(P), P]
     lib.saber_hip_conv2d_stage_create_tail.argtypes = [C.POINTER(P), I, P, C.POINTER(P)]
     lib.saber_hip_conv2d_stage_run_tail.argtypes = [P, P, P, C.POINTER(P), C.POINTER(P), P, P]
+    lib.saber_hip_conv2d_stage_create_head.argtypes = [C.POINTER(P), I, P, P, P, C.POINTER(P)]
+    lib.saber_hip_conv2d_stage_run_head.argtypes = [P, P, P, C.POINTER(P), C.POINTER(P), P, P]
     lib.saber_hip_conv2d_stem_pair_create.argtypes = [P, P, P, C.POINTER(P)]
     lib.saber_hip_conv2d_stem_pair_destroy.argtypes = [P]
     lib.saber_hip_conv2d_stem_pair_destroy.restype = None
@@ -155,6 +158,7 @@
     lib.saber_hip_fc_destroy.argtypes = [P]
     lib.saber_hip_net_optimize.argtypes = [P, I]
     lib.saber_hip_net_stage_blocks.argtypes = [P, I]
+    lib.saber_hip_net_stage_head.argtypes = [P, I]
     lib.saber_hip_net_status.argtypes = [P]
     lib.saber_hip_net_inject_coop_error.argtypes = [P]
     lib.saber_hip_net_coop_fallbacks.argtypes = [P]
diff --git a/anakin_amd/saber.py b/anakin_amd/saber.py
--- a/anakin_amd/saber.py
+++ b/anakin_amd/saber.py
@@ -295,12 +295,16 @@
 
 class SaberChainStage:
 
-    def __init__(self, chains, tail=None):
+    def __init__(self, chains, tail=None, head=None):
         self.chains = list(chains)
         self.tail = tail
+        self.head = head
         arr = (C.c_void_p * len(chains))(*[c.h for c in chains])
         self.h = C.c_void_p()
-        if tail is None:
+        if head is not None:
+            L.check(L.load().saber_hip_conv2d_stage_create_head(arr, len(chains), tail.h if tail is not None else None, head[0].h, head[1].h,
+                                                                C.byref(self.h)))
+        elif tail is None:
             L.check(L.load().saber_hip_conv2d_stage_create(arr, len(chains), C.byref(self.h)))
         else:
             L.check(L.load().saber_hip_conv2d_stage_create_tail(arr, len(chains), tail.h, C.byref(self.h)))
@@ -313,6 +317,12 @@
             L.check(L.load().saber_hip_conv2d_stage_run(self.h, _p(x), _p(res), a, b, _stream()))
         else:
             L.check(L.load().saber_hip_conv2d_stage_run_tail(self.h, _p(x), _p(res), a, b, _p(y_tail), _stream()))
+
+    def dispatch_head(self, x_head, y_head_b, y1s, y2s, y_tail=None):
+        n = len(self.chains)
+        a = (C.c_void_p * n)(*[t.data_ptr() for t in y1s])
+        b = (C.c_void_p * n)(*[t.data_ptr() for t in y2s])
+        L.check(L.load().saber_hip_conv2d_stage_run_head(self.h, _p(x_head), _p(y_head_b), a, b, _p(y_tail) if y_tail is not None else None, _stream()))
 
     def __del__(self):
         try:
@@ -798,6 +808,25 @@
                 ch[i] = v - (1 << 32) if v >> 31 else v
         self.set_choices(ch)
 
+    def heads(self):
+        lib = L.load()
+        ch = self.choices()
+        out = []
+        for i, _, on in self.stages():
+            p = int(lib.saber_hip_net_stage_head(self.h, i))
+            if on and p >= 0 and (ch[p] >> 29) & 1:
+                out.append((p, i))
+        return out
+
+    def select_heads(self, on):
+        lib = L.load()
+        ch = self.choices()
+        for i, _, sel in self.stages():
+            p = int(lib.saber_hip_net_stage_head(self.h, i))
+            if sel and p >= 0:
+                ch[p] = (ch[p] | (1 << 29)) if on else (ch[p] & ~(1 << 29))
+        self.set_choices(ch)
+
     def time_ops(self, iters=20):
         out = (C.c_float * self.num_ops())()
         L.check(L.load().saber_hip_net_time_ops(self.h, _stream(), iters, out))
diff --git a/include/saber_hip.h b/include/saber_hip.h
--- a/include/saber_hip.h
+++ b/include/saber_hip.h
@@ -101,6 +101,11 @@
                                saber_hip_stream_t stream);
 int saber_hip_conv2d_stage_create_tail(saber_hip_chain_t* const* chains, int n, saber_hip_chain_t* tail, saber_hip_chain_stage_t** out);
 int saber_hip_conv2d_stage_run_tail(saber_hip_chain_stage_t* stage, const void* x, const void* res, void* const* y1, void* const* y2,
+                                    void* y_tail, saber_hip_stream_t stream);
+
+int saber_hip_conv2d_stage_create_head(saber_hip_chain_t* const* chains, int n, saber_hip_chain_t* tail, const saber_hip_conv_t* head_a,
+                                       const saber_hip_conv_t* head_b, saber_hip_chain_stage_t** out);
+int saber_hip_conv2d_stage_run_head(saber_hip_chain_stage_t* stage, const void* x_head, void* y_head_b, void* const* y1, void* const* y2,
                                     void* y_tail, saber_hip_stream_t stream);
 
 typedef struct saber_hip_stem_pair saber_hip_stem_pair_t;
@@ -231,6 +236,7 @@
 int saber_hip_net_status(saber_hip_net_t* net);
 int saber_hip_net_inject_coop_error(saber_hip_net_t* net);
 int saber_hip_net_stage_blocks(const saber_hip_net_t* net, int index);
+int saber_hip_net_stage_head(const saber_hip_net_t* net, int index);
 int saber_hip_net_num_launches(const saber_hip_net_t* net);
 int saber_hip_net_tensor_unwritten(const saber_hip_net_t* net, int id);
 int saber_hip_net_add_softmax(saber_hip_net_t* net, int rows, int cols, int in_id, int out_id);
```
